# cgisky1980/Qwen3-TTS-Rust

Measured on AMD Instinct MI355X. Metric: audio_sec_per_s, higher is better.
Workload: dtype bf16

## Files before the change

include/q3tts.h:

```cpp
#ifndef Q3TTS_H
#define Q3TTS_H

#include <stdint.h>

#ifdef __cplusplus
extern "C" {
#endif

#define Q3TTS_OK 0
#define Q3TTS_ERR_INVALID (-1)
#define Q3TTS_ERR_DEVICE (-2)
#define Q3TTS_ERR_OOM (-3)
#define Q3TTS_ERR_IO (-4)
#define Q3TTS_ERR_STATE (-5)
#define Q3TTS_ERR_UNSUPPORTED (-6)

#define Q3TTS_MAX_UPSAMPLE 4
#define Q3TTS_MAX_DEC_BLOCKS 8


typedef struct q3tts_model_config {
    int32_t t_n_layer, t_d_model, t_n_head, t_n_kv_head, t_head_dim, t_d_ffn, t_vocab;
    float t_rope_theta;
    int32_t t_mrope_sections[4];
// ... 164 lines not shown
int32_t q3tts_node_size(const q3tts_node* n);
q3tts_engine* q3tts_node_engine(q3tts_node* n, int32_t rank);
int32_t q3tts_node_shard(int32_t n_total, int32_t world, int32_t rank, int32_t* idx, int32_t cap);

typedef struct q3tts_timings {
    float prefill_ms, decode_ms, vocoder_ms, total_ms;
    float frame_step_ms;
    float probe_kernel_ms;
    int64_t frame_steps;
    int64_t algo_bytes_per_step;
    int64_t algo_flops_per_step;
    float mean_live_slots;
    float mean_rows;
    int64_t probe_count;
    float probe_empty_ms;
    float mean_ctx_tokens;
} q3tts_timings;
int q3tts_get_timings(const q3tts_engine* e, q3tts_timings* out);

int32_t q3tts_mel_frames(int64_t n_samples);
int q3tts_mel(q3tts_engine* e, const float* audio, int64_t n_samples, float* out, int32_t cap_frames, int32_t* n_frames);

typedef struct q3tts_clone_config {
    int32_t mel_dim;
    int32_t se_channels[5];
    int32_t se_kernels[5];
    int32_t se_dilations[5];
    int32_t se_attn_channels;
    int32_t se_res2net_scale;
    int32_t se_se_channels;
    int32_t se_dim;
    int32_t ae_filters;
    int32_t ae_kernel, ae_res_kernel, ae_last_kernel;
    int32_t ae_n_ratios; int32_t ae_ratios[4];
    int32_t ae_hidden;
    int32_t ae_n_layer, ae_n_head, ae_head_dim, ae_d_ffn, ae_window;
    float ae_rope_theta, ae_ln_eps, ae_layer_scale;
    int32_t ae_down_stride;
    int32_t ae_vq_dim;
    int32_t ae_n_codebooks, ae_codebook_size;
} q3tts_clone_config;
void q3tts_clone_default_config(q3tts_clone_config* cfg);
int q3tts_clone_init(q3tts_engine* e, const q3tts_clone_config* cfg);
int32_t q3tts_clone_audio_frames(const q3tts_engine* e, int64_t n_samples);
int q3tts_clone_audio_encode(q3tts_engine* e, const float* audio, int64_t n_samples, int64_t* codes, int32_t cap_frames,
                             int32_t* n_frames);
int q3tts_clone_speaker_encode(q3tts_engine* e, const float* audio, int64_t n_samples, float* spk_emb);
int q3tts_k_speaker_from_mel(q3tts_engine* e, const float* mel, int32_t n_frames, float* spk_emb);
int q3tts_k_audio_latent(q3tts_engine* e, const float* audio, int64_t n_samples, float* latent, int32_t cap_frames,
                         int32_t* n_frames);

typedef struct q3tts_tokenizer q3tts_tokenizer;
int q3tts_tokenizer_load(const char* tokenizer_json_path, q3tts_tokenizer** out, char* err, int32_t err_cap);
void q3tts_tokenizer_free(q3tts_tokenizer* t);
int32_t q3tts_tokenizer_vocab_size(const q3tts_tokenizer* t);
int q3tts_tokenizer_encode(const q3tts_tokenizer* t, const char* utf8, int64_t n_bytes, uint32_t* ids, int32_t cap,
                           int32_t* n_ids, char* err, int32_t err_cap);
int q3tts_tokenizer_decode(const q3tts_tokenizer* t, const uint32_t* ids, int32_t n, char* out, int64_t cap, int64_t* n_bytes,
                           char* err, int32_t err_cap);

int q3tts_k_gemm_exact(int32_t device, const float* x, int32_t B, int32_t K, const uint16_t* w_bf16, int32_t N,
                       const float* norm_w , float eps, const float* bias ,
                       int32_t epilogue , float* y, uint64_t* argmax_keys,
                       int32_t iters, float* mean_kernel_ms);
int q3tts_k_attention(int32_t device, const float* qkv , int32_t n_rows, int32_t pos0,
                      int32_t n_head, int32_t n_kv_head, int32_t head_dim, const float* q_norm_w, const float* k_norm_w,
                      float eps, float rope_theta, const int32_t* mrope_sections, float* out );
int q3tts_k_attention_decode(int32_t device, const float* qkv, int32_t n_slots, const int32_t* lens, int32_t n_ctx, int32_t n_head,
                             int32_t n_kv_head, int32_t head_dim, const float* q_norm_w, const float* k_norm_w, float eps, float rope_theta,
                             const int32_t* mrope_sections, int32_t policy, float* out_f32, uint16_t* out_bf16);
int q3tts_k_attention_runs(int32_t device, const float* qkv, int32_t n_runs, const int32_t* run_n, const int32_t* run_pos0, int32_t n_ctx,
                           int32_t n_head, int32_t n_kv_head, int32_t head_dim, const float* q_norm_w, const float* k_norm_w, float eps,
                           float rope_theta, const int32_t* mrope_sections, int32_t policy, int32_t out_form, void* out, float* out_scale,
                           uint16_t* k_cache, uint16_t* v_cache);
int q3tts_k_attention_decode_ex(int32_t device, const float* qkv, int32_t n_slots, const int32_t* lens, int32_t n_ctx, int32_t n_head,
                                int32_t n_kv_head, int32_t head_dim, const float* q_norm_w, const float* k_norm_w, float eps,
                                float rope_theta, const int32_t* mrope_sections, int32_t policy, int32_t row_indexed, int32_t out_form,
                                void* out, float* out_scale, uint16_t* k_cache, uint16_t* v_cache);
int q3tts_k_attention_pair(int32_t device, const float* qkv, int32_t n_slots, int32_t n_ctx, int32_t n_head, int32_t n_kv_head,
                           int32_t head_dim, const float* q_norm_w, const float* k_norm_w, float eps, float rope_theta,
                           const int32_t* mrope_sections, int32_t out_form, void* out, float* out_scale, uint16_t* k_cache, uint16_t* v_cache);
int q3tts_k_attend_pick(int32_t fused, int32_t gqa_ratio, int32_t n_ctx, int32_t n_seg, int32_t seg_max_n, int32_t seg_max_t,
                        int32_t n_kv_head, int32_t* kernel);
int q3tts_k_sample(int32_t device, const float* logits, int32_t n, int32_t ld, int32_t limit, float temperature,
                   int32_t top_k, float top_p, const float* r_uniform, int32_t* out_ids);
int q3tts_k_talker_prefill(q3tts_engine* e, const float* embd, int32_t n_tok, float* hidden_out, float* logits_out);
int q3tts_k_talker_prefill_prefix(q3tts_engine* e, const q3tts_prefix* prefix, const float* embd, int32_t n_tok, float* hidden_out,
                                  float* logits_out);
int q3tts_k_vocoder(q3tts_engine* e, const int32_t* codes, int32_t n_frames, int32_t chunk_frames, float* pcm_out,
                    int32_t* n_samples_out);
int q3tts_k_vocoder_latent(q3tts_engine* e, const int32_t* codes, int32_t n_frames, int32_t chunk_frames, float* out);
typedef struct q3tts_voc_tap {
    char name[32];
    int32_t dtype, layout, hist_rows, rows, channels, reserved;
    uint64_t offset;
} q3tts_voc_tap;
int q3tts_k_vocoder_taps(q3tts_engine* e, const int32_t* codes, int32_t n_frames, int32_t chunk_frames, int32_t tap_call, void* buf,
                         uint64_t buf_bytes, q3tts_voc_tap* recs, int32_t rec_cap, int32_t* n_recs);
int q3tts_k_vocoder_bench(q3tts_engine* e, int32_t n_slots, int32_t chunks, float* ms_per_chunk);
int q3tts_k_gguf_read(const char* path, const char* tensor, float* out, int64_t cap, int64_t* nelem, int64_t* dims4, int32_t* ggml_type);
int q3tts_k_gguf_meta(const char* path, const char* key, int32_t* value_type, int32_t* elem_type, int64_t* count, double* values,
                      int64_t values_cap, char* str, int64_t str_cap, int64_t* str_bytes);
int q3tts_k_probe(q3tts_engine* e, int32_t enable);
int q3tts_k_mfma_bf16(int32_t device, const uint16_t* a, const uint16_t* b, const float* c, float* d, int32_t n_cases, int32_t chain);
int q3tts_k_bgemm(int32_t device, const uint16_t* xb, int32_t B, int32_t K, const uint16_t* w_bf16, int32_t N, const float* ssp, int32_t ntiles,
                  int32_t d_norm, float eps, int32_t epilogue, const float* nw_next, float* y, uint16_t* yb, float* ssp_out, uint64_t* keys,
                  int32_t iters, float* mean_kernel_ms);
int q3tts_k_bgemm_policy(int32_t big);
int q3tts_k_attend_policy(int32_t decode, int32_t prefill);
int q3tts_k_pred_variant(q3tts_engine* e, int32_t force);
int q3tts_k_text_ready(int32_t n_text, int32_t closed, int32_t n_frames);
int q3tts_k_bgemm_pick(int32_t B, int32_t K, int32_t N, int32_t epilogue, int32_t w_once, int32_t q8, int32_t* out5);
int q3tts_k_bgemm_q8(int32_t device, const uint16_t* xb, int32_t B, int32_t K, const int8_t* q, const uint16_t* d_f16, int32_t N, const float* ssp,
                     int32_t ntiles, int32_t d_norm, float eps, int32_t epilogue, const float* nw_next, float* y, uint16_t* yb, float* ssp_out,
                     uint64_t* keys, int32_t iters, float* mean_kernel_ms);
int q3tts_k_bgemm_q8a8(int32_t device, const int8_t* aq, const float* ad, int32_t B, int32_t K, const int8_t* q, const uint16_t* d_f16, int32_t N,
                       const float* ssp, int32_t ntiles, int32_t d_norm, float eps, int32_t epilogue, const float* nw_next, float* y, int8_t* yq,
                       float* yd, float* ssp_out, int32_t iters, float* mean_kernel_ms);
int q3tts_k_bgemm_q8a8_argmax(int32_t device, const int8_t* aq, const float* ad, int32_t B, int32_t K, const int8_t* q, const uint16_t* d_f16, int32_t N,
                              const float* ssp, int32_t ntiles, int32_t d_norm, float eps, int32_t* ids_out);
int q3tts_k_bgemm_voc(int32_t device, const uint16_t* xb, int32_t B, int32_t K, const uint16_t* w_bf16, int32_t N, int32_t epilogue, const float* bias,
                      int32_t bias_n, const float* col_scale, int32_t seg_rows, int32_t gap_rows, float* y, uint16_t* yb, int32_t want_yb);
int q3tts_k_project(int32_t device, const float* x, int32_t rows, int32_t n_in, const float* w, const float* bias, int32_t n_out, const float* nw,
                    float* y, uint16_t* xb, float* ssp);
int q3tts_k_norm_inputs(int32_t device, const float* x, int32_t rows, int32_t d, const float* nw, uint16_t* xb, float* ssp);
int q3tts_k_alloc_upload(q3tts_engine* e, int64_t bytes, int64_t* mismatches);
int q3tts_k_pcm_pack(int32_t device, const float* src, int32_t rows, int64_t stride, const int32_t* ent_row, const int32_t* ent_first,
                     const int32_t* ent_count, const int64_t* ent_dst, int32_t n_ent, int32_t format, void* out, int64_t out_n);
int q3tts_k_resample_table(int32_t rate_in, int32_t rate_out, int32_t* L, int32_t* M, int32_t* H, float* tab, int64_t cap, int64_t* n);
int q3tts_k_pcm_resample(int32_t device, const float* src, int32_t rows, int64_t stride, const int32_t* row_len, const int32_t* row_final,
                         const int32_t* ent_row, const int32_t* ent_first, const int32_t* ent_count, const int64_t* ent_dst, int32_t n_ent,
                         int32_t rate_in, int32_t rate_out, int32_t format, void* out, int64_t out_n, int32_t iters, float* mean_ms);
int q3tts_k_rng_f32(uint64_t seed, int32_t n, float* out);

#ifdef __cplusplus
}
#endif
#endif
```

qwen3-tts-rust_amd/csrc/q3_attend.hip:

```cpp
#include "q3_kernels.h"

__device__ __forceinline__ uint2 pack_bf16x4(float a, float b, float c, float d) {
    return make_uint2((uint32_t)q3_bf16(a) | ((uint32_t)q3_bf16(b) << 16), (uint32_t)q3_bf16(c) | ((uint32_t)q3_bf16(d) << 16));
}
__device__ __forceinline__ uint16_t* k_cache_elem(uint16_t* khead, int pos, int lane) {
    const int blk = pos >> 6, kl = pos & 63, c = lane >> 1, e0 = 4 * (lane & 1);
    return khead + ((size_t)(blk * (Q3_ATT_HD >> 3) + c) * 64 + kl) * 8 + e0;
}
__device__ __forceinline__ float prep_rinv(const float4 x4, float eps, int hd) {
    float acc = 0.0f;
    acc = fmaf(x4.x, x4.x, acc); acc = fmaf(x4.y, x4.y, acc); acc = fmaf(x4.z, x4.z, acc); acc = fmaf(x4.w, x4.w, acc);
    acc = wave_sum(acc);
    return 1.0f / sqrtf(acc / (float)hd + eps);
}
__device__ __forceinline__ void prep_norm(const float4 x4, float rinv, const float4 w4, float y[4]) {
    y[0] = (x4.x * rinv) * w4.x; y[1] = (x4.y * rinv) * w4.y; y[2] = (x4.z * rinv) * w4.z; y[3] = (x4.w * rinv) * w4.w;
}
__device__ __forceinline__ void prep_rope(const float y[4], const float4 c4, const float4 s4, int hl, int lane, float o[4]) {
    const float cc[4] = {c4.x, c4.y, c4.z, c4.w}, ss[4] = {s4.x, s4.y, s4.z, s4.w};
#pragma unroll
    for (int e = 0; e < 4; ++e) {
        const float other = __shfl_xor(y[e], hl);
        o[e] = (lane < hl) ? fmaf(-other, ss[e], y[e] * cc[e])
                           : fmaf(other, ss[e], y[e] * cc[e]);
// ... 312 lines not shown
#pragma unroll
        for (int u = 0; u < 4; ++u) vv[tr][u] = *(const uint4*)(vb + (size_t)min(64 * tr + 4 * sw + kg + 16 * u, T - 1) * hd + dl * 8);
    ml0 = wave_max(ml0); ml1 = wave_max(ml1);
    if (lane == 0) { mw[sw] = ml0; mw[4 + sw] = ml1; }
    Q3_LDS_BARRIER();
    const float m0 = fmaxf(fmaxf(mw[0], mw[1]), fmaxf(mw[2], mw[3])), m1 = fmaxf(fmaxf(mw[4], mw[5]), fmaxf(mw[6], mw[7]));
    float ls0 = 0.0f, ls1 = 0.0f;
    for (int blk = sw; blk * 64 < T; blk += 4) {
        const int t = blk * 64 + lane;
        if (t < T) {
            const float e0 = q3_expf(p0[t] - m0), e1 = q3_expf(p1[t] - m1);
            p0[t] = e0; p1[t] = e1; ls0 += e0; ls1 += e1;
        }
    }
    ls0 = wave_sum(ls0); ls1 = wave_sum(ls1);
    if (lane == 0) { lw[sw] = ls0; lw[4 + sw] = ls1; }
    Q3_LDS_BARRIER();
    Q3_STAMP(a, 2);
    float o0[8], o1[8];
#pragma unroll
    for (int e = 0; e < 8; ++e) { o0[e] = 0.0f; o1[e] = 0.0f; }
    const uint4 vn = *(const uint4*)(vnew + 4 * dl);
#pragma unroll
    for (int tr = 0; tr < 4; ++tr) {
        const int t0 = 64 * tr + 4 * sw + kg;
        if (64 * tr >= T) break;
#pragma unroll
        for (int u = 0; u < 4; ++u) {
            const int t = t0 + 16 * u;
            if (t < T) {
                const float pa = p0[t], pb = p1[t];
                const uint4 w = (t == pos) ? vn : vv[tr][u];
                att_pv8x2(pa, pb, w, o0, o1);
            }
        }
    }
    for (int t0 = 256 + 4 * sw + kg; t0 < T; t0 += 64) {
        uint4 vl[4];
#pragma unroll
        for (int u = 0; u < 4; ++u) vl[u] = *(const uint4*)(vb + (size_t)min(t0 + 16 * u, T - 1) * hd + dl * 8);
#pragma unroll
        for (int u = 0; u < 4; ++u) {
            const int t = t0 + 16 * u;
            if (t < T) {
                const float pa = p0[t], pb = p1[t];
                const uint4 w = (t == pos) ? vn : vl[u];
                att_pv8x2(pa, pb, w, o0, o1);
            }
        }
    }
#pragma unroll
    for (int e = 0; e < 8; ++e) {
        o0[e] = o0[e] + __shfl_xor(o0[e], 16); o0[e] = o0[e] + __shfl_xor(o0[e], 32);
        o1[e] = o1[e] + __shfl_xor(o1[e], 16); o1[e] = o1[e] + __shfl_xor(o1[e], 32);
    }
    if (kg == 0) {
        *(float4*)(ow + (0 * 4 + sw) * hd + dl * 8) = (float4){o0[0], o0[1], o0[2], o0[3]}; *(float4*)(ow + (0 * 4 + sw) * hd + dl * 8 + 4) = (float4){o0[4], o0[5], o0[6], o0[7]};
        *(float4*)(ow + (1 * 4 + sw) * hd + dl * 8) = (float4){o1[0], o1[1], o1[2], o1[3]}; *(float4*)(ow + (1 * 4 + sw) * hd + dl * 8 + 4) = (float4){o1[4], o1[5], o1[6], o1[7]};
    }
    Q3_LDS_BARRIER();
    Q3_STAMP(a, 3);
    if (tid < 128) {
        const int h2 = tid >> 6, d0 = 2 * (tid & 63);
        const float l = ((lw[h2 * 4] + lw[h2 * 4 + 1]) + lw[h2 * 4 + 2]) + lw[h2 * 4 + 3];
        float ov[2];
#pragma unroll
        for (int q = 0; q < 2; ++q) {
            const int d = d0 + q;
            const float r0 = ow[(h2 * 4 + 0) * hd + d], r1 = ow[(h2 * 4 + 1) * hd + d], r2 = ow[(h2 * 4 + 2) * hd + d], r3 = ow[(h2 * 4 + 3) * hd + d];
            ov[q] = (((r0 + r1) + r2) + r3) / l;
        }
        const int hq = g * 2 + h2;
        if (a.out_bf16 == 2) q3_q8_out2x16(ov[0], ov[1], row, hq * hd + d0, (a.Hq * hd) >> 6, a.out_rt16, (int8_t*)a.out, a.out_scale);
        else if (a.out_bf16) *(uint32_t*)((uint16_t*)a.out + q3_atile_off(row, hq * hd + d0, (a.Hq * hd) >> 5)) = (uint32_t)q3_bf16(ov[0]) | ((uint32_t)q3_bf16(ov[1]) << 16);
        else *(float2*)(a.out + (size_t)row * a.ldo + (size_t)hq * hd + d0) = make_float2(ov[0], ov[1]);
    }
#ifdef Q3_STAMPS
    Q3_STAMP(a, 4);
    asm volatile("s_waitcnt vmcnt(0)" ::: "memory");
    Q3_STAMP(a, 5);
#endif
}

template <int R>
__global__ __launch_bounds__((R + 1) * 64) void k_attend_small(Q3Attend a) {
    __shared__ __attribute__((aligned(16))) float qh[R][Q3_ATT_HD];
    __shared__ __attribute__((aligned(16))) uint32_t knew[64];
    __shared__ __attribute__((aligned(16))) uint32_t vnew[64];
    const int g = blockIdx.x, row = blockIdx.y, wv = threadIdx.x >> 6, lane = threadIdx.x & 63;
    Q3_STAMP(a, 0);
    int pos, slot;
    q3_row_map(row, a.row_pos, a.row_slot, a.slot_mod, a.pos_const, &pos, &slot);
    if (pos < 0) return;
    constexpr int hd = Q3_ATT_HD, half = hd >> 1, nl = hd >> 2;
    const int T = pos + 1;
    const Q3QkPrep& pr = a.prep;
    const size_t hb = ((size_t)slot * a.Hkv + g) * a.n_ctx;
    const uint16_t* kb = a.kc + hb * hd;
    const uint16_t* vb = a.vc + hb * hd;
    const float* rowp = a.qkv + (size_t)row * a.ld;
    const float* csp = pr.cs + (size_t)pos * half + 4 * (lane & 15);
    const float* snp = pr.sn + (size_t)pos * half + 4 * (lane & 15);
    if (wv == R) {
        const bool isk = lane < nl;
        const float4 x4 = isk ? ((const float4*)(rowp + (size_t)(a.Hq + g) * hd))[lane] : ((const float4*)(rowp + (size_t)(a.Hq + a.Hkv + g) * hd))[lane - nl];
        float4 w4 = (float4){0.f, 0.f, 0.f, 0.f}, c4 = (float4){1.f, 1.f, 1.f, 1.f}, s4 = (float4){0.f, 0.f, 0.f, 0.f};
        if (isk) { w4 = ((const float4*)pr.knw)[lane]; c4 = *(const float4*)csp; s4 = *(const float4*)snp; }
        const float4 v = isk ? x4 : (float4){0.f, 0.f, 0.f, 0.f};
        float o[4];
        prep_arith(v, w4, c4, s4, pr.eps, lane, o);
        if (isk) {
            const uint2 kk = pack_bf16x4(o[0], o[1], o[2], o[3]);
            *(uint2*)k_cache_elem(pr.kc + hb * hd, pos, lane) = kk;
            *(uint2*)(knew + 2 * lane) = kk;
        } else {
            const int j = lane - nl;
            const uint2 vk = pack_bf16x4(x4.x, x4.y, x4.z, x4.w);
            *(uint2*)(pr.vc + (hb + pos) * hd + 4 * j) = vk;
            *(uint2*)(vnew + 2 * j) = vk;
        }
        Q3_STAMP(a, 1);
        __syncthreads();
        return;
    }
    const int hq = g * R + wv;
    uint4 kv[16];
    uint32_t vv[16];
#pragma unroll
    for (int c = 0; c < 16; ++c) kv[c] = lane < pos ? ((const uint4*)kb)[c * 64 + lane] : make_uint4(0, 0, 0, 0);
#pragma unroll
    for (int u = 0; u < 16; ++u) vv[u] = u < pos ? *(const uint32_t*)(vb + (size_t)u * hd + 2 * lane) : 0u;
    float4 x4 = (float4){0.f, 0.f, 0.f, 0.f}, w4 = x4, c4 = (float4){1.f, 1.f, 1.f, 1.f}, s4 = x4;
    if (lane < nl) { x4 = ((const float4*)(rowp + (size_t)hq * hd))[lane]; w4 = ((const float4*)pr.qnw)[lane]; c4 = *(const float4*)csp; s4 = *(const float4*)snp; }
    {
        float y[4];
        prep_norm(x4, prep_rinv(x4, pr.eps, hd), w4, y);
        const float cc[4] = {c4.x, c4.y, c4.z, c4.w}, ss[4] = {s4.x, s4.y, s4.z, s4.w};
        float o[4];
#pragma unroll
        for (int e = 0; e < 4; ++e) {
            const float other = __shfl_xor(y[e], 16);
            o[e] = (lane < 16) ? fmaf(-other, ss[e], y[e] * cc[e]) : fmaf(other, ss[e], y[e] * cc[e]);
        }
        if (lane < nl) *(float4*)(qh[wv] + 4 * lane) = (float4){o[0], o[1], o[2], o[3]};
    }
    Q3_STAMP(a, 1);
    __syncthreads();
    Q3_STAMP(a, 2);
    if (lane == pos) {
#pragma unroll
        for (int c = 0; c < 16; ++c) kv[c] = *(const uint4*)(knew + 4 * c);
    }
    const float* q = qh[wv];
    float sc = 0.0f;
#pragma unroll
    for (int c = 0; c < 16; ++c)
        sc = att_dot8(*(const float4*)(q + c * 8), *(const float4*)(q + c * 8 + 4), kv[c], sc);
    sc = sc * (1.0f / sqrtf((float)hd));
    const float m = wave_max(lane < T ? sc : -INFINITY);
    const float e = lane < T ? q3_expf(sc - m) : 0.0f;
    float l = wave_sum(e);
    l = ((l + 0.0f) + 0.0f) + 0.0f;
#ifdef Q3_STAMPS
    asm volatile("" :: "v"(l)); Q3_STAMP(a, 3);
#endif
    float o0[16], o1[16];
#pragma unroll
    for (int u = 0; u < 16; ++u) { o0[u] = 0.0f; o1[u] = 0.0f; }
    const uint32_t vn = vnew[lane];
#pragma unroll
    for (int c = 0; c < 4; ++c) {
        if (16 * c >= T) break;
#pragma unroll
        for (int u = 0; u < 16; ++u) {
            const int t = 16 * c + u;
            if (t >= T) break;
            uint32_t w;
            if (t == pos) w = vn;
            else if (c == 0) w = vv[u];
            else w = *(const uint32_t*)(vb + (size_t)t * hd + 2 * lane);
            const float pt = __uint_as_float(__builtin_amdgcn_readlane(__float_as_uint(e), t));
            o0[u] = fmaf(pt, q3_u2f(w << 16), o0[u]);
            o1[u] = fmaf(pt, q3_u2f(w & 0xffff0000u), o1[u]);
        }
    }
    float r0[4], r1[4];
#pragma unroll
    for (int w = 0; w < 4; ++w) {
        r0[w] = (o0[4 * w] + o0[4 * w + 1]) + (o0[4 * w + 2] + o0[4 * w + 3]);
        r1[w] = (o1[4 * w] + o1[4 * w + 1]) + (o1[4 * w + 2] + o1[4 * w + 3]);
    }
    const float ov0 = (((r0[0] + r0[1]) + r0[2]) + r0[3]) / l, ov1 = (((r1[0] + r1[1]) + r1[2]) + r1[3]) / l;
    const int d0 = 2 * lane;
    att_out2(a, row, hq, d0, ov0, ov1);
#ifdef Q3_STAMPS
    Q3_STAMP(a, 4);
    asm volatile("s_waitcnt vmcnt(0)" ::: "memory");
    Q3_STAMP(a, 5);
#endif
}

__global__ __launch_bounds__(256) void k_attend_pair(Q3Attend a) {
    __shared__ __attribute__((aligned(16))) float kh[2][128], vh[2][128], qh[2][2][128], ps[2][2][64];
    const int g = blockIdx.x, b = blockIdx.y, wave = threadIdx.x >> 6, lane = threadIdx.x & 63;
    const int rr = wave >> 1, hh = wave & 1, R = 2, hd = 128;
    const int row = rr * a.slot_mod + b, slot = b, pos = rr;
    const Q3QkPrep& pr = a.prep;
    const size_t hb = ((size_t)slot * a.Hkv + g) * a.n_ctx;
    const float* rowp = a.qkv + (size_t)row * a.ld;
    const int half = hd >> 1, nl = hd >> 2;
    float qo[4], o4[4];
    prep_head(rowp + (size_t)(g * R + hh) * hd, pr.qnw, pr.eps, pr.cs + (size_t)pos * half, pr.sn + (size_t)pos * half, hd, lane, qo);
    if (lane < nl) *(float4*)(qh[rr][hh] + 4 * lane) = (float4){qo[0], qo[1], qo[2], qo[3]};
    if (hh == 0) {
        prep_head(rowp + (size_t)(a.Hq + g) * hd, pr.knw, pr.eps, pr.cs + (size_t)pos * half, pr.sn + (size_t)pos * half, hd, lane, o4);
        if (lane < nl) {
// ... 144 lines not shown
                const float ov = ((rsw[0][e] + rsw[1][e]) + rsw[2][e]) + rsw[3][e];
                const int d = dl * 8 + e, col = (g * 2 + hh) * hd + d;
                if (a.out_bf16) ((uint16_t*)a.out)[q3_atile_off(row, col, (a.Hq * hd) >> 5)] = q3_bf16(ov / l);
                else a.out[(size_t)row * a.ldo + col] = ov / l;
            }
        }
        asm volatile("s_waitcnt lgkmcnt(0)" ::: "memory");
    }
}

static int g_att_decode = 0, g_att_prefill = 0;
static std::once_flag g_att_once;
static void att_policy_init() {
    std::call_once(g_att_once, []() {
        const char* ev = getenv("Q3TTS_ATT_OLD"); g_att_decode = (ev && atoi(ev)) ? 1 : 0;
        ev = getenv("Q3TTS_ATT_PREFILL_OLD"); g_att_prefill = (ev && atoi(ev)) ? 1 : 0;
    });
}
void q3_attend_policy(int decode, int prefill) { att_policy_init(); g_att_decode = decode; g_att_prefill = prefill; }
void q3_attend_policy_get(int* decode, int* prefill) { att_policy_init(); *decode = g_att_decode; *prefill = g_att_prefill; }

static hipError_t att_allow_lds(const void* kernel, size_t lds) { return hipFuncSetAttribute(kernel, hipFuncAttributeMaxDynamicSharedMemorySize, (int)lds); }

int q3_attend_pick(const Q3Attend& a) {
    att_policy_init();
    if (a.hd != Q3_ATT_HD || a.Hkv <= 0 || a.Hq % a.Hkv) return Q3_ATT_REFUSED;
    const int R = a.Hq / a.Hkv;
    if ((R != 1 && R != 2 && R != 4) || (a.fused && R == 1) || (a.fused == 2 && R != 2)) return Q3_ATT_REFUSED;
    if (a.fused == 2) return Q3_ATT_PAIR;
    if (a.fused && a.n_ctx <= 64 && R == 2) return Q3_ATT_SMALL2;
    if (a.fused && R == 2 && g_att_decode == 0) return Q3_ATT_GQA2;
    if (!a.fused && R == 2 && a.seg && a.seg_max_n <= 128 && a.seg_max_t <= 256 && g_att_prefill != 1 &&
        (a.n_seg * a.Hkv >= 128 || g_att_prefill == 2)) return Q3_ATT_PREFILL;
    if (a.fused) return R == 2 ? Q3_ATT_F2 : Q3_ATT_F4;
    return R == 1 ? Q3_ATT_N1 : (R == 2 ? Q3_ATT_N2 : Q3_ATT_N4);
}

int q3_launch_attend(const Q3Attend& a, hipStream_t s) {
    const int pick = q3_attend_pick(a);
    if (pick == Q3_ATT_REFUSED) return 1;
    const int R = a.Hq / a.Hkv;
    const dim3 grid(a.Hkv, a.rows);
    if (pick == Q3_ATT_PAIR) {
        hipLaunchKernelGGL(k_attend_pair, dim3(a.Hkv, a.slot_mod), dim3(256), 0, s, a);
        return 0;
    }
    if (pick == Q3_ATT_SMALL2) {
        hipLaunchKernelGGL((k_attend_small<2>), grid, dim3(192), 0, s, a);
        return 0;
    }
    if (pick == Q3_ATT_GQA2) {
        const size_t lds2 = ((size_t)2 * a.n_ctx + 2 * Q3_ATT_HD + 8 * Q3_ATT_HD + 16 + 128) * sizeof(float);
        static Q3PerDevice pd2;
        if (lds2 > 65536 && !pd2.ensure(lds2, [&]() { return att_allow_lds((const void*)k_attend_gqa2, lds2); })) return 1;
        hipLaunchKernelGGL(k_attend_gqa2, grid, dim3(256), lds2, s, a);
        return 0;
    }
    if (pick == Q3_ATT_PREFILL) {
        const int nblk = (a.seg_max_t + 63) / 64;
        const int pw = a.seg_max_t > 128 ? (a.seg_max_t + 63) & ~63 : 128;
        const size_t lds3 = (size_t)nblk * 16384 + (size_t)a.seg_max_t * 256 + (size_t)8 * (pw + 128) * sizeof(float);
        static Q3PerDevice pd3;
        if (lds3 > 65536 && !pd3.ensure(lds3, [&]() { return att_allow_lds((const void*)k_attend_prefill, lds3); })) return 1;
        hipLaunchKernelGGL(k_attend_prefill, dim3(a.Hkv, a.n_seg), dim3(512), lds3, s, a);
        return 0;
    }
    const size_t lds = att_lds(R, a.n_ctx).bytes;
    static Q3PerDevice pd;
    if (lds > 65536 && !pd.ensure(lds, [&]() {
            hipError_t e = hipSuccess;
            for (const void* k : {(const void*)k_attend<2, true>, (const void*)k_attend<4, true>, (const void*)k_attend<1, false>,
                                  (const void*)k_attend<2, false>, (const void*)k_attend<4, false>})
                if (e == hipSuccess) e = att_allow_lds(k, lds);
            return e;
        })) return 1;
    if (pick == Q3_ATT_F2) hipLaunchKernelGGL((k_attend<2, true>), grid, dim3(512), lds, s, a);
    else if (pick == Q3_ATT_F4) hipLaunchKernelGGL((k_attend<4, true>), grid, dim3(1024), lds, s, a);
    else if (pick == Q3_ATT_N1) hipLaunchKernelGGL((k_attend<1, false>), grid, dim3(256), lds, s, a);
    else if (pick == Q3_ATT_N2) hipLaunchKernelGGL((k_attend<2, false>), grid, dim3(512), lds, s, a);
    else hipLaunchKernelGGL((k_attend<4, false>), grid, dim3(1024), lds, s, a);
    return 0;
}

__global__ __launch_bounds__(256) void k_kv_prefix(Q3KvPrefix a) {
    const int j = blockIdx.y, isv = blockIdx.x & 1, lg = blockIdx.x >> 1, l = lg / a.Hkv, g = lg - l * a.Hkv;
    const int P = a.P[j], np = (P + 63) & ~63;
    const size_t src = ((size_t)l * a.Hkv + g) * np * a.hd;
    const size_t dst = (size_t)l * a.layer_stride + ((size_t)a.slot[j] * a.Hkv + g) * a.n_ctx * a.hd;
    const int n16 = (isv ? P : np) * (a.hd >> 3);
    const uint4* sp = (const uint4*)((isv ? a.pv[j] : a.pk[j]) + src);
    uint4* dp = (uint4*)((isv ? a.vc : a.kc) + dst);
    for (int i = threadIdx.x; i < n16; i += 256) dp[i] = sp[i];
}
void q3_launch_kv_prefix(const Q3KvPrefix& a, hipStream_t s) {
    if (a.n <= 0) return;
    hipLaunchKernelGGL(k_kv_prefix, dim3(a.L * 2 * a.Hkv, a.n), dim3(256), 0, s, a);
}
```

qwen3-tts-rust_amd/csrc/q3_engine.h:

```cpp
#pragma once
#include <algorithm>
#include <cstddef>
#include <atomic>
#include <mutex>
#include <string>
#include <vector>

#include "../../include/q3tts.h"
#include "q3_kernels.h"

static_assert(sizeof(q3tts_request) == 80 && offsetof(q3tts_request, text_stream) == 12 && offsetof(q3tts_request, prompt) == 16 &&
              offsetof(q3tts_request, text_open) == 44 && offsetof(q3tts_request, seed) == 48 && offsetof(q3tts_request, prefix) == 72, "q3tts_request layout");

struct Q3Voc;
struct Q3Mel;
struct Q3Clone;

struct Q3Tfm {
    int L = 0, d = 0, Hq = 0, Hkv = 0, hd = 0, F = 0, nq = 0, nkv = 0, nqkv = 0, head_n = 0;
    std::vector<float*> attn_norm, ffn_norm, qn, kn;
    std::vector<uint4*> wqkv, wo, wgu, wd;
    float* out_norm = nullptr;
    uint4* head = nullptr;
    std::vector<uint16_t*> sqkv, so, sgu, sd; uint16_t* shead = nullptr; bool q8 = false;
    bool a8 = false;
    uint16_t *kc = nullptr, *vc = nullptr;
    size_t layer_stride = 0;
    int n_ctx = 0, n_slots = 0;
    float *cs = nullptr, *sn = nullptr;
    size_t weight_bytes = 0;
};

struct Q3Scratch {
    float* qkv = nullptr;
    uint16_t *att = nullptr, *h = nullptr;
    float *asc_att = nullptr, *asc_h = nullptr; int rt16 = 0;
    int rows = 0;
};

struct Q3Rows {
    float* x = nullptr;
    uint16_t* xb = nullptr;
    float* ssp = nullptr;
    float* ascale = nullptr; int rt16 = 0;
};

struct Q3Lane {
    int nb = 0;
    hipStream_t stream = nullptr;
    Q3Rows T, P;
    float *logits = nullptr, *logits_tmp = nullptr, *fb = nullptr;
    unsigned long long* keys = nullptr;
    int *row_pos_t = nullptr, *slot_id = nullptr, *perm = nullptr;
    Q3Scratch sc;
    float* plogits = nullptr;
    std::vector<hipGraph_t> graphs;
    std::vector<hipGraphExec_t> execs;
    std::vector<hipGraph_t> graphs_s;
    std::vector<hipGraphExec_t> execs_s;
    std::vector<hipGraph_t> graphs_t[2];
    std::vector<hipGraphExec_t> execs_t[2];
    hipEvent_t ev_begin = nullptr, ev_end = nullptr;
};

struct q3tts_engine {
    q3tts_engine_config cfg;
    std::string err;
    hipStream_t stream = nullptr, vstream = nullptr;
    std::vector<void*> allocs;
    Q3Tfm T, P;
    float* text = nullptr;
    std::vector<float*> codec;
    const float** codec_dev = nullptr;
    std::vector<float*> pproj;
    float* proj_w = nullptr;
    float* proj_b = nullptr;
    float* tts_pad = nullptr;
    float* marker_row = nullptr;
    int B = 0;
    std::vector<int> buckets; int cur_bucket = -1;
    std::vector<int> row_of_slot, slot_of_row;
    Q3Slot* slots = nullptr;
    Q3Slot* slots_host = nullptr;
    int* codes = nullptr;
    float* rng = nullptr;
    Q3Lane lane;
    Q3Scratch sc_pre;
    Q3Rows pf;
    int *pf_pos = nullptr, *pf_slot = nullptr;
    int* pf_seg = nullptr;
    Q3PromptRow* prow_dev = nullptr; int prow_cap = 0;
    float* spk_dev = nullptr; int* refcodes_dev = nullptr;
    float temperature = 0.7f; int top_k = 40; float top_p = 0.9f; int has_seed = 0; uint64_t seed = 0;
    int max_steps = 512;
    float p_temperature = 0.0f; int p_top_k = 0; float p_top_p = 1.0f; float rep_penalty = 1.0f;
    int pred_force = 0, pred_variant = 0;
    int streams_open = 0;
    int* ts_ids = nullptr; int* ts_cnt = nullptr; int2* ts_cur = nullptr;
    std::vector<char> ts_slot; int ts_variant = 0, ts_used = 0;
    float* prng = nullptr;
    uint32_t* seen = nullptr; int seen_words = 0;
    hipEvent_t ev0 = nullptr, ev1 = nullptr, ev2 = nullptr, ev3 = nullptr;
    std::vector<hipEvent_t> fin_ev;
    q3tts_timings tm{};
    Q3Voc* voc = nullptr;
    Q3Mel* mel = nullptr;
    Q3Clone* clone = nullptr;
    int probe = 0, probe_kind = 0;
    std::vector<hipEvent_t> probe_ev;
    int probe_i = 0;
    double probe_ms = 0, probe_empty_ms = 0; long long probe_cnt = 0, probe_empty_cnt = 0, row_steps = 0;
    int dev_pcm_on = 0; float* dev_pcm = nullptr; int dev_pcm_n = 0; size_t dev_pcm_stride = 0;
    int out_rate = 0; Q3Resamp rs_out{}; std::vector<Q3Resamp> rs_cache;
    float* rs_stage = nullptr; size_t rs_stage_stride = 0, rs_stage_cap = 0;
    double hp_launch = 0, hp_sync = 0;
    float *park_logits = nullptr, *park_x = nullptr;
    float* first_chunk_host = nullptr;
    std::atomic<q3tts_session*> session{nullptr};
    std::mutex err_mu;
};

struct q3tts_prefix {
    q3tts_engine* e = nullptr;
    int P = 0, np = 0;
    uint16_t *k = nullptr, *v = nullptr;
};

int q3_set_err(q3tts_engine* e, int code, const std::string& msg);
int q3_refuse_in_session(q3tts_engine* e);
#define Q3_NOT_IN_SESSION(e) do { if ((e) && (e)->session.load()) return q3_refuse_in_session(e); } while (0)
#define Q3_HIP(e, call)                                                                                         \
    do {                                                                                                        \
        hipError_t err__ = (call);                                                                              \
        if (err__ != hipSuccess)                                                                                \
            return q3_set_err((e), Q3TTS_ERR_DEVICE, std::string(#call) + ": " + hipGetErrorString(err__));     \
    } while (0)

int q3_dev_alloc_zeroed(q3tts_engine* e, void** p, size_t bytes);

template <class T>
int q3_dalloc(q3tts_engine* e, T** p, size_t n) {
    void* q = nullptr;
    const int rc = q3_dev_alloc_zeroed(e, &q, n * sizeof(T) + 64);
    if (rc != Q3TTS_OK) return rc;
    e->allocs.push_back(q);
    *p = (T*)q;
    return Q3TTS_OK;
}

class Q3Gguf;
struct Q3TfmShape {
    int grp;
    int L, d, Hq, Hkv, hd, F, head_n;
    float theta; const int* sections;
    int n_ctx, n_slots;
};
int q3_tfm_init(q3tts_engine* e, Q3Tfm& t, const Q3TfmShape& sh, const Q3Gguf* g, const char* file, int q8mode);
int q3_assets_init(q3tts_engine* e, const std::string& wdir);

struct Q3LayerRun {
    int rows;
    const int *row_pos, *row_slot;
    bool one_row_per_slot;
    hipEvent_t* probe;
    int slot_mod, pos_const;
    const int* seg; int n_seg, seg_max_n, seg_max_t;
};
int q3_run_layers(q3tts_engine* e, Q3Tfm& t, const Q3Rows& r, const Q3LayerRun& a, Q3Scratch& sc, hipStream_t s);
int q3_record_frame(q3tts_engine* e, Q3Lane& L, hipStream_t s, int B);
int q3_capture_frames(q3tts_engine* e, std::vector<hipGraph_t>& graphs, std::vector<hipGraphExec_t>& execs);
Q3BGemm q3_gemm_head(const Q3Tfm& t, int q, int N, const Q3Rows& r, int row0, int rows, float eps, int once, float* y);
int q3_launch_gemm(q3tts_engine* e, const Q3Tfm& t, const Q3BGemm& g, hipStream_t s, hipEvent_t* probe = nullptr, int kind = -1);

void q3_rope_tables(int n_pos, int hd, float theta, const int* sections, std::vector<float>& cs, std::vector<float>& sn);

void q3_stdrng_f32(uint64_t seed, int n, float* out);

void q3_mel_destroy(q3tts_engine* e);
int q3_mel_run(q3tts_engine* e, const float* audio, int64_t n_samples, int32_t* n_frames, float** out_dev);
void q3_clone_destroy(q3tts_engine* e);
int q3_voc_create(q3tts_engine* e);
void q3_voc_destroy(q3tts_engine* e);
int q3_voc_reset(q3tts_engine* e, int slot);
int q3_voc_decode(q3tts_engine* e, int slot, int f0, int nf, int is_last, hipStream_t s);
int q3_voc_decode_batch(q3tts_engine* e, const int* slots, const int* real, int ns, int nf, hipStream_t s, int beside_decoder);
void q3_voc_mark_last(q3tts_engine* e, int slot);
float* q3_voc_pcm(q3tts_engine* e, int slot);
int q3_voc_samples(q3tts_engine* e, int slot);
int q3_voc_samples_per_frame(const q3tts_engine* e);
size_t q3_voc_pcm_stride(const q3tts_engine* e);

int q3_resample_get(q3tts_engine* e, int rate_in, int rate_out, Q3Resamp* out);
int q3_resample_slot(q3tts_engine* e, int b, long long first_out, int count, int n_valid, bool is_final, hipStream_t s);

enum { BOS_TOKEN = 151672, EOS_TOKEN = 151673 };

int q3_plan_rows(q3tts_engine* e, const std::vector<int>& live);
int q3_admit_many(q3tts_engine* e, const int* slots, const q3tts_request* const* reqs, int count, int* rc);
int q3_run_chunk(q3tts_engine* e, int CH);
int q3_text_rows_set(q3tts_engine* e, int b, const int32_t* T, int from, int n, int n_frames);
int q3_park_rows(q3tts_engine* e, int b, bool save);
void q3_text_trailing(const q3tts_request* r, std::vector<int32_t>& T);
int q3_pred_force_variant(q3tts_engine* e, int force);
int q3_voc_dispatch(q3tts_engine* e, const char* live, const char* want, int* voc_frames, bool more, bool* first);
double q3_now_ms();
```

qwen3-tts-rust_amd/csrc/q3_engine.hip:

```cpp
#include "q3_engine.h"
#include "q3_gguf.h"

#include <chrono>
#include <cmath>
#include <cstdio>
#include <cstdlib>
#include <cstring>

static thread_local std::string g_err;

int q3_set_err(q3tts_engine* e, int code, const std::string& msg) {
    if (e) { std::lock_guard<std::mutex> lk(e->err_mu); e->err = msg; }
    g_err = msg;
    return code;
}
extern "C" const char* q3tts_last_error(const q3tts_engine* e) {
    if (!e) return g_err.c_str();
    if (!e->session.load()) return e->err.c_str();
    static thread_local std::string copy;
    std::lock_guard<std::mutex> lk(const_cast<q3tts_engine*>(e)->err_mu);
    copy = e->err;
    return copy.c_str();
}
int q3_refuse_in_session(q3tts_engine* e) {
// ... 49 lines not shown
    if (c.talker_q8_0 == 2) REQ(m.t_vocab % 32 == 0 && ((m.t_n_head + 2 * m.t_n_kv_head) * m.t_head_dim) % 32 == 0 && m.t_d_ffn % 64 == 0);
    REQ(c.predictor_q8_0 >= 0 && c.predictor_q8_0 <= 2);
    if (c.predictor_q8_0 == 2) {
        REQ(m.p_d_model % 512 == 0); REQ(m.p_d_ffn % 512 == 0); REQ((m.p_n_head * m.p_head_dim) % 512 == 0);
        REQ(m.codebook_size % 32 == 0); REQ(((m.p_n_head + 2 * m.p_n_kv_head) * m.p_head_dim) % 32 == 0); REQ(m.p_d_ffn % 64 == 0);
    }
#undef REQ
    return Q3TTS_OK;
}

int q3_dev_alloc_zeroed(q3tts_engine* e, void** p, size_t bytes) {
    void* q = nullptr;
    hipError_t err = hipMalloc(&q, bytes);
    if (err != hipSuccess) return q3_set_err(e, Q3TTS_ERR_OOM, std::string("hipMalloc: ") + hipGetErrorString(err));
    err = hipMemsetAsync(q, 0, bytes, e->stream);
    if (err == hipSuccess) err = hipStreamSynchronize(e->stream);
    if (err != hipSuccess) { hipFree(q); return q3_set_err(e, Q3TTS_ERR_DEVICE, std::string("hipMemset: ") + hipGetErrorString(err)); }
    *p = q;
    return Q3TTS_OK;
}
#define TRY(x) do { int rc__ = (x); if (rc__ != Q3TTS_OK) return rc__; } while (0)

static int alloc_scratch(q3tts_engine* e, Q3Scratch& sc, int rows, int nqkv, int nq, int F) {
    sc.rows = rows;
    const size_t r16 = ((size_t)rows + 15) & ~(size_t)15;
    TRY(q3_dalloc(e, &sc.qkv, (size_t)rows * nqkv)); TRY(q3_dalloc(e, &sc.att, r16 * nq)); TRY(q3_dalloc(e, &sc.h, r16 * F));
    sc.rt16 = (int)(r16 / 16);
    if (e->T.a8 || e->P.a8) { TRY(q3_dalloc(e, &sc.asc_att, r16 * (nq / 32))); TRY(q3_dalloc(e, &sc.asc_h, r16 * (F / 32))); }
    return Q3TTS_OK;
}

static int alloc_rows(q3tts_engine* e, Q3Rows& r, size_t rows, int d, bool scales) {
    const size_t r16 = (rows + 15) & ~(size_t)15;
    TRY(q3_dalloc(e, &r.x, rows * d)); TRY(q3_dalloc(e, &r.xb, r16 * d)); TRY(q3_dalloc(e, &r.ssp, rows * (d / 16)));
    r.rt16 = (int)(r16 / 16);
    if (scales) TRY(q3_dalloc(e, &r.ascale, r16 * (d / 32)));
    return Q3TTS_OK;
}

extern "C" int q3tts_engine_create(const q3tts_engine_config* cfg, q3tts_engine** out) {
    if (!cfg || !out) return q3_set_err(nullptr, Q3TTS_ERR_INVALID, "null argument");
    std::string why;
    if (validate(*cfg, why) != Q3TTS_OK) return q3_set_err(nullptr, Q3TTS_ERR_INVALID, why);
    if (cfg->predictor_q8_0 == 1)
        return q3_set_err(nullptr, Q3TTS_ERR_UNSUPPORTED, "predictor_q8_0 = 1 (Q8_0 weights x bf16 activations) is not implemented for the Predictor: use 0 (bf16) or 2 (Q8_0 x Q8_0)");
    int ndev = 0;
    if (hipGetDeviceCount(&ndev) != hipSuccess || ndev <= 0)
        return q3_set_err(nullptr, Q3TTS_ERR_DEVICE, "no HIP device: libq3tts has no CPU fallback");
    if (cfg->device < 0 || cfg->device >= ndev) return q3_set_err(nullptr, Q3TTS_ERR_INVALID, "device ordinal out of range");
    q3tts_engine* e = new q3tts_engine();
    e->cfg = *cfg; e->cfg.weights_path = nullptr;
    e->max_steps = cfg->max_steps_cap < 512 ? cfg->max_steps_cap : 512;
    auto fail = [&](int rc) { std::string m = e->err; q3tts_engine_destroy(e); g_err = m; return rc; };
#define TRYC(x) do { int rc__ = (x); if (rc__ != Q3TTS_OK) return fail(rc__); } while (0)
#define HIPC(call) do { hipError_t er__ = (call); if (er__ != hipSuccess) { q3_set_err(e, Q3TTS_ERR_DEVICE, std::string(#call) + ": " + hipGetErrorString(er__)); return fail(Q3TTS_ERR_DEVICE); } } while (0)
    HIPC(hipSetDevice(cfg->device));
    q3_bgemm_prepare();
    if (cfg->talker_q8_0 == 2 || cfg->predictor_q8_0 == 2) q3_bgemm8_prepare();
    HIPC(hipStreamCreateWithFlags(&e->stream, hipStreamNonBlocking));
    if (getenv("Q3TTS_VOC_SERIAL") && atoi(getenv("Q3TTS_VOC_SERIAL"))) e->vstream = e->stream;
    else if (getenv("Q3TTS_VOC_CUMASK")) {
        uint32_t w = (uint32_t)strtoul(getenv("Q3TTS_VOC_CUMASK"), nullptr, 16), mask[8];
        for (auto& x : mask) x = w;
        HIPC(hipExtStreamCreateWithCUMask(&e->vstream, 8, mask));
    } else HIPC(hipStreamCreateWithFlags(&e->vstream, hipStreamNonBlocking));
    HIPC(hipEventCreate(&e->ev0)); HIPC(hipEventCreate(&e->ev1)); HIPC(hipEventCreate(&e->ev2)); HIPC(hipEventCreate(&e->ev3));
    e->fin_ev.resize(cfg->max_batch, nullptr);
    for (auto& ev : e->fin_ev) HIPC(hipEventCreateWithFlags(&ev, hipEventDisableTiming));
    const q3tts_model_config& m = e->cfg.model;
    const int B = cfg->max_batch;
    e->B = B;
    hipStream_t s = e->stream;
    const std::string wdir = cfg->weights_path ? cfg->weights_path : "";
    Q3Gguf gt, gp;
    std::string er;
    if (!wdir.empty() && (gt.open(wdir + "/qwen3_tts_talker.gguf", er) || gp.open(wdir + "/qwen3_tts_predictor.gguf", er))) { q3_set_err(e, Q3TTS_ERR_INVALID, er); return fail(Q3TTS_ERR_INVALID); }
    TRYC(q3_tfm_init(e, e->T, {.grp = Q3G_TALKER, .L = m.t_n_layer, .d = m.t_d_model, .Hq = m.t_n_head, .Hkv = m.t_n_kv_head, .hd = m.t_head_dim, .F = m.t_d_ffn,
                               .head_n = m.t_vocab, .theta = m.t_rope_theta, .sections = m.t_mrope_sections, .n_ctx = cfg->n_ctx, .n_slots = B},
                     wdir.empty() ? nullptr : &gt, "qwen3_tts_talker.gguf", cfg->talker_q8_0));
    TRYC(q3_tfm_init(e, e->P, {.grp = Q3G_PRED, .L = m.p_n_layer, .d = m.p_d_model, .Hq = m.p_n_head, .Hkv = m.p_n_kv_head, .hd = m.p_head_dim, .F = m.p_d_ffn,
                               .head_n = (m.n_codebooks - 1) * m.codebook_size, .theta = m.p_rope_theta, .sections = nullptr, .n_ctx = 64, .n_slots = B},
                     wdir.empty() ? nullptr : &gp, "qwen3_tts_predictor.gguf", cfg->predictor_q8_0));
    TRYC(q3_assets_init(e, wdir));
    TRYC(q3_dalloc(e, &e->slots, (size_t)B));
    HIPC(hipHostMalloc((void**)&e->slots_host, sizeof(Q3Slot) * 2 * B, hipHostMallocDefault));
    memset(e->slots_host, 0, sizeof(Q3Slot) * 2 * B);
    TRYC(q3_dalloc(e, &e->codes, (size_t)B * cfg->max_steps_cap * m.n_codebooks)); TRYC(q3_dalloc(e, &e->rng, (size_t)B * cfg->max_steps_cap));
    TRYC(q3_dalloc(e, &e->prng, (size_t)B * cfg->max_steps_cap * (m.n_codebooks - 1)));
    e->seen_words = (m.sample_limit + 31) / 32;
    TRYC(q3_dalloc(e, &e->seen, (size_t)B * e->seen_words));
    TRYC(q3_dalloc(e, &e->ts_ids, (size_t)B * cfg->max_steps_cap)); TRYC(q3_dalloc(e, &e->ts_cnt, (size_t)B)); TRYC(q3_dalloc(e, &e->ts_cur, (size_t)B));
    TRYC(q3_dalloc(e, &e->park_logits, (size_t)B * m.t_vocab)); TRYC(q3_dalloc(e, &e->park_x, (size_t)B * m.t_d_model));
    e->ts_slot.assign(B, 0);
    {
        const int nb = B;
        const int nqkv_max = std::max(e->T.nqkv, e->P.nqkv), nq_max = std::max(e->T.nq, e->P.nq), F_max = std::max(e->T.F, e->P.F);
        Q3Lane& L = e->lane;
        L.nb = nb;
        HIPC(hipStreamCreateWithFlags(&L.stream, hipStreamNonBlocking));
        HIPC(hipEventCreate(&L.ev_begin)); HIPC(hipEventCreate(&L.ev_end));
        TRYC(alloc_rows(e, L.T, (size_t)nb, m.t_d_model, e->T.a8)); TRYC(alloc_rows(e, L.P, (size_t)2 * nb, m.p_d_model, e->P.a8));
        TRYC(q3_dalloc(e, &L.logits, (size_t)nb * m.t_vocab)); TRYC(q3_dalloc(e, &L.logits_tmp, (size_t)nb * std::max(m.t_vocab, m.t_d_model)));
        TRYC(q3_dalloc(e, &L.fb, (size_t)nb * m.d_embed)); TRYC(q3_dalloc(e, &L.keys, (size_t)nb * (m.codebook_size / 16)));
        TRYC(q3_dalloc(e, &L.plogits, (size_t)nb * m.codebook_size));
        TRYC(q3_dalloc(e, &L.row_pos_t, (size_t)nb)); TRYC(q3_dalloc(e, &L.slot_id, (size_t)nb)); TRYC(q3_dalloc(e, &L.perm, (size_t)nb));
        std::vector<int> sid(nb), rp(nb, -1);
        for (int b = 0; b < nb; ++b) sid[b] = b;
        HIPC(hipMemcpyAsync(L.slot_id, sid.data(), nb * 4, hipMemcpyHostToDevice, s));
        HIPC(hipMemcpyAsync(L.row_pos_t, rp.data(), nb * 4, hipMemcpyHostToDevice, s));
        HIPC(hipStreamSynchronize(s));
        TRYC(alloc_scratch(e, L.sc, 2 * nb, nqkv_max, nq_max, F_max));
        for (int r = 1; r < nb && r < 16; r *= 2) e->buckets.push_back(r);
        for (int r = 16; r < nb; r += 16) e->buckets.push_back(r);
        e->buckets.push_back(nb);
        e->cur_bucket = (int)e->buckets.size() - 1;
        e->row_of_slot = sid; e->slot_of_row = sid;
    }
    TRYC(alloc_scratch(e, e->sc_pre, cfg->n_ctx, e->T.nqkv, e->T.nq, e->T.F));
    TRYC(alloc_rows(e, e->pf, (size_t)cfg->n_ctx, m.t_d_model, e->T.a8));
    TRYC(q3_dalloc(e, &e->pf_pos, (size_t)cfg->n_ctx)); TRYC(q3_dalloc(e, &e->pf_slot, (size_t)cfg->n_ctx)); TRYC(q3_dalloc(e, &e->pf_seg, (size_t)4 * cfg->max_batch));
    { std::vector<int> pp(cfg->n_ctx); for (int i = 0; i < cfg->n_ctx; ++i) pp[i] = i;
      HIPC(hipMemcpyAsync(e->pf_pos, pp.data(), pp.size() * 4, hipMemcpyHostToDevice, s)); HIPC(hipStreamSynchronize(s)); }
    e->prow_cap = cfg->n_ctx;
    TRYC(q3_dalloc(e, &e->prow_dev, (size_t)e->prow_cap)); TRYC(q3_dalloc(e, &e->spk_dev, (size_t)m.d_embed));
    TRYC(q3_dalloc(e, &e->refcodes_dev, (size_t)cfg->n_ctx * 16));
    {
        TRYC(q3_dalloc(e, &e->marker_row, (size_t)m.d_embed));
        const Q3PromptRow mr{1, m.tts_pad_id, 0, 0};
        HIPC(hipMemcpyAsync(e->prow_dev, &mr, sizeof(mr), hipMemcpyHostToDevice, s));
        HIPC(hipStreamSynchronize(s));
        q3_launch_prompt_rows(e->prow_dev, 1, e->text, m.text_vocab, e->codec_dev, m.codec0_rows, m.codecq_rows, m.n_codebooks, e->spk_dev, m.d_embed, e->marker_row, s);
        HIPC(hipStreamSynchronize(s));
    }
    if (cfg->with_vocoder) {
        TRYC(q3_voc_create(e));
        HIPC(hipHostMalloc((void**)&e->first_chunk_host, sizeof(float) * 4 * (size_t)q3_voc_samples_per_frame(e), hipHostMallocDefault));
    }
    HIPC(hipStreamSynchronize(s));
    if (!(getenv("Q3TTS_NO_GRAPH") && atoi(getenv("Q3TTS_NO_GRAPH")))) TRYC(q3_capture_frames(e, e->lane.graphs, e->lane.execs));
#undef TRYC
#undef HIPC
    *out = e;
    return Q3TTS_OK;
}

extern "C" void q3tts_engine_destroy(q3tts_engine* e) {
    if (!e) return;
    if (q3tts_session* ss = e->session.load()) q3tts_session_close(ss);
    hipSetDevice(e->cfg.device);
    if (e->stream) hipStreamSynchronize(e->stream);
    if (e->vstream) hipStreamSynchronize(e->vstream);
    if (e->voc) q3_voc_destroy(e);
    q3_mel_destroy(e);
    q3_clone_destroy(e);
    if (e->first_chunk_host) hipHostFree(e->first_chunk_host);
    {
        Q3Lane& L = e->lane;
        if (L.stream) hipStreamSynchronize(L.stream);
        for (auto ge : L.execs) if (ge) hipGraphExecDestroy(ge);
        for (auto gr : L.graphs) if (gr) hipGraphDestroy(gr);
        for (auto ge : L.execs_s) if (ge) hipGraphExecDestroy(ge);
        for (auto gr : L.graphs_s) if (gr) hipGraphDestroy(gr);
        for (int v = 0; v < 2; ++v) {
            for (auto ge : L.execs_t[v]) if (ge) hipGraphExecDestroy(ge);
            for (auto gr : L.graphs_t[v]) if (gr) hipGraphDestroy(gr);
        }
// ... 640 lines not shown
    e->probe_ms = 0; e->probe_cnt = 0; e->row_steps = 0; e->probe_empty_ms = 0; e->probe_empty_cnt = 0;
    hipStream_t s = e->stream;
    while (done < n) {
        bool admitted = false;
        {
            std::vector<int> as, ai; std::vector<const q3tts_request*> ar;
            for (int b = 0; b < B && next < n; ++b)
                if (run[b].req < 0) { TRY(drain(b)); as.push_back(b); ar.push_back(&reqs[next]); ai.push_back(next++); }
            {
                std::vector<int> live(as);
                for (int b = 0; b < B; ++b) if (run[b].req >= 0) live.push_back(b);
                TRY(plan_rows(e, live));
            }
            if (!as.empty()) {
                Q3_HIP(e, hipEventRecord(e->ev0, s));
                admitted = true;
                std::vector<int> rcs(as.size());
                TRY(admit_many(e, as.data(), ar.data(), (int)as.size(), rcs.data()));
                for (size_t i = 0; i < as.size(); ++i) {
                    if (rcs[i] != Q3TTS_OK) { outs[ai[i]].status = rcs[i]; ++done; }
                    else { run[as[i]] = SlotRun{}; run[as[i]].req = ai[i]; voc_frames[as[i]] = 0; }
                }
            }
        }
        if (admitted) { Q3_HIP(e, hipEventRecord(e->ev2, s)); }
        hp_lap(hp_admit);
        bool any = false;
        for (int b = 0; b < B; ++b) if (run[b].req >= 0) any = true;
        if (!any) break;
        float ms = 0;
        TRY(run_chunk(e, CH, &ms));
        hp_lap(hp_chunk);
        dec_ms += ms; steps += CH;
        if (admitted) { hipEventElapsedTime(&ms, e->ev0, e->ev2); pre_ms += ms; }
        for (int b = 0; b < B; ++b) if (run[b].req >= 0) { ctx_tokens += (long long)e->slots_host[b].cur_pos * CH; live_slot_steps += CH; }
        if (e->voc) {
            const double tv0 = now_ms();
            hipStream_t vs = e->vstream;
            for (int b = 0; b < B; ++b) { live[b] = run[b].req >= 0; want[b] = live[b] && reqs[run[b].req].want_pcm; }
            bool first = false;
            TRY(q3_voc_dispatch(e, live.data(), want.data(), voc_frames.data(), next < n, &first));
            if (first) {
                for (int b = 0; b < B; ++b)
                    if (run[b].req >= 0 && run[b].t_first == 0 && voc_frames[b] > 0) {
                        const int nsmp = std::min(voc_frames[b], 4) * spf;
                        Q3_HIP(e, hipMemcpyAsync(e->first_chunk_host, q3_voc_pcm(e, b), sizeof(float) * (size_t)nsmp, hipMemcpyDeviceToHost, vs));
                    }
                Q3_HIP(e, hipStreamSynchronize(vs));
                const double tn = now_ms();
                for (int b = 0; b < B; ++b) if (run[b].req >= 0 && run[b].t_first == 0 && voc_frames[b] > 0) run[b].t_first = tn;
            }
            voc_ms += now_ms() - tv0;
        }
        hp_lap(hp_voc);
        for (int j = 0; j < B; ++j)
            if (pending[j] >= 0 && hipEventQuery(e->fin_ev[j]) == hipSuccess) TRY(drain(j));
        for (int b = 0; b < B; ++b) {
            if (run[b].req < 0 || e->slots_host[b].active) continue;
            for (int j = 0; j < B; ++j)
                if (pending[j] >= 0 && hipEventQuery(e->fin_ev[j]) == hipSuccess) TRY(drain(j));
            TRY(finalize(e, b, &reqs[run[b].req], &outs[run[b].req], run[b], t0, true, e->fin_ev[b], run[b].req));
            pending[b] = run[b].req;
            run[b].req = -1; ++done;
            e->ts_slot[b] = 0;
        }
        hp_lap(hp_fin);
    }
    for (int b = 0; b < B; ++b) TRY(drain(b));
    hp_lap(hp_tail);
    if (host_prof) {
        fprintf(stderr, "q3tts_generate_batch host wall (ms): admit + plan %.1f | chunks (launch + wait) %.1f = launch %.1f + wait %.1f, device events %.1f over %lld steps | vocoder issue %.1f | finalize %.1f | tail (last results) %.1f | total %.1f\n",
                hp_admit, hp_chunk, e->hp_launch, e->hp_sync, dec_ms, steps, hp_voc, hp_fin, hp_tail, now_ms() - t0);
        e->hp_launch = e->hp_sync = 0;
    }
    e->tm.prefill_ms = (float)pre_ms; e->tm.decode_ms = (float)dec_ms; e->tm.vocoder_ms = (float)voc_ms;
    e->tm.total_ms = (float)(now_ms() - t0); e->tm.frame_steps = steps; e->tm.frame_step_ms = steps ? (float)(dec_ms / steps) : 0.0f;
    {
        const q3tts_model_config& m = e->cfg.model;
        const long long wt = (long long)e->T.weight_bytes;
        const double bpw_p = e->P.q8 ? 1.0625 : 2.0;
        const long long wp_layers = (long long)e->P.weight_bytes - (long long)(bpw_p * (double)((size_t)e->P.head_n * m.p_d_model));
        const long long head1 = (long long)(bpw_p * (double)((size_t)m.codebook_size * m.p_d_model)), pj = 2ll * m.p_d_model * m.d_embed;
        const long long kv_per_tok = 2ll * m.t_n_layer * 2 * m.t_n_kv_head * m.t_head_dim;
        const long long fixed = wt + (m.n_codebooks - 1) * (wp_layers + head1) + pj;
        e->tm.algo_bytes_per_step = fixed + (steps ? kv_per_tok * (ctx_tokens / steps) : 0);
        e->tm.mean_live_slots = steps ? (float)((double)live_slot_steps / (double)steps) : 0.0f;
        e->tm.algo_flops_per_step = (long long)((double)fixed * (double)e->tm.mean_live_slots);
        e->tm.mean_rows = steps ? (float)((double)e->row_steps / (double)steps) : 0.0f;
        e->tm.mean_ctx_tokens = steps ? (float)((double)ctx_tokens / (double)steps) : 0.0f;
        e->tm.probe_kernel_ms = e->probe_cnt ? (float)(e->probe_ms / (double)e->probe_cnt) : 0.0f;
        e->tm.probe_count = e->probe_cnt;
        e->tm.probe_empty_ms = e->probe_empty_cnt ? (float)(e->probe_empty_ms / (double)e->probe_empty_cnt) : 0.0f;
    }
    return Q3TTS_OK;
}

int q3_plan_rows(q3tts_engine* e, const std::vector<int>& live) { return plan_rows(e, live); }
int q3_admit_many(q3tts_engine* e, const int* slots, const q3tts_request* const* reqs, int count, int* rc) { return admit_many(e, slots, reqs, count, rc); }
int q3_run_chunk(q3tts_engine* e, int CH) { return run_chunk(e, CH, nullptr); }
double q3_now_ms() { return now_ms(); }

extern "C" int q3tts_generate(q3tts_engine* e, const q3tts_request* req, q3tts_result* out) {
    int rc = q3tts_generate_batch(e, req, 1, out);
    if (rc != Q3TTS_OK) return rc;
    return out->status;
}

extern "C" void q3tts_result_free(q3tts_result* r) {
    if (!r) return;
    free(r->codes);
    pin_free(r->pcm);
    r->codes = nullptr; r->pcm = nullptr;
}

extern "C" int q3tts_get_timings(const q3tts_engine* e, q3tts_timings* out) {
    if (!e || !out) return Q3TTS_ERR_INVALID;
    *out = e->tm;
    return Q3TTS_OK;
}

struct q3tts_stream {
    q3tts_engine* e; q3tts_request req; int voc_frames = 0; bool finished = false; bool final_sent = false;
    std::vector<float> chunk; double t0 = 0, t_first = 0;
    long long delivered = 0;
};

static int stream_emit(q3tts_stream* st, int before, int after, bool fin, const float** chunk, int32_t* n_samples) {
    q3tts_engine* e = st->e;
    hipStream_t s = e->stream;
    const float* from = q3_voc_pcm(e, 0) + before;
    int c = after - before;
    if (e->out_rate) {
        const Q3Resamp& r = e->rs_out;
        c = (int)((fin ? q3_resample_N(after, r.L, r.M) : q3_resample_D(after, r.L, r.M, r.H)) - st->delivered);
        TRY(q3_resample_slot(e, 0, st->delivered, c, after, fin, s));
        from = e->rs_stage;
        st->delivered += std::max(c, 0);
    }
    st->chunk.resize((size_t)std::max(1, c));
    if (c > 0) Q3_HIP(e, hipMemcpyAsync(st->chunk.data(), from, sizeof(float) * (size_t)c, hipMemcpyDeviceToHost, s));
    Q3_HIP(e, hipStreamSynchronize(s));
    *chunk = st->chunk.data(); *n_samples = std::max(c, 0);
    return Q3TTS_OK;
}

extern "C" int q3tts_stream_begin(q3tts_engine* e, const q3tts_request* req, q3tts_stream** out) {
    if (!e || !req || !out) return q3_set_err(e, Q3TTS_ERR_INVALID, "null argument");
    Q3_NOT_IN_SESSION(e);
    if (!e->voc) return q3_set_err(e, Q3TTS_ERR_STATE, "streaming needs with_vocoder = 1");
    if (req->text_open == 1) return q3_set_err(e, Q3TTS_ERR_INVALID, "text_open = 1 is for sessions (q3tts_session_append_text): a stream takes closed text and never waits");
    Q3_HIP(e, hipSetDevice(e->cfg.device));
    std::fill(e->ts_slot.begin(), e->ts_slot.end(), 0);
    q3tts_stream* st = new q3tts_stream();
    st->e = e; st->req = *req; st->t0 = now_ms();
    int rc = plan_rows(e, std::vector<int>{0});
    if (rc == Q3TTS_OK) rc = admit(e, 0, req);
    if (rc != Q3TTS_OK) { delete st; return rc; }
    ++e->streams_open;
    *out = st;
    return Q3TTS_OK;
}

extern "C" int q3tts_stream_poll(q3tts_stream* st, const float** chunk, int32_t* n_samples, int32_t* is_final) {
    if (!st || !chunk || !n_samples || !is_final) return q3_set_err(nullptr, Q3TTS_ERR_INVALID, "null argument");
    q3tts_engine* e = st->e;
    *chunk = nullptr; *n_samples = 0; *is_final = 0;
    if (st->final_sent) { *is_final = 1; return Q3TTS_OK; }
    hipStream_t s = e->stream;
    const int spf = q3_voc_samples_per_frame(e);
// ... 55 lines not shown
```

qwen3-tts-rust_amd/csrc/q3_hooks.hip:

```cpp
#include "q3_engine.h"

#include <cstdio>
#include <cstring>

#define TRY(x) do { int rc__ = (x); if (rc__ != Q3TTS_OK) return rc__; } while (0)
#define HK(call) do { hipError_t er__ = (call); if (er__ != hipSuccess) return q3_set_err(nullptr, Q3TTS_ERR_DEVICE, std::string(#call) + ": " + hipGetErrorString(er__)); } while (0)

struct DevBuf {
    void* p = nullptr;
    ~DevBuf() { if (p) hipFree(p); }
    template <class T> operator T*() const { return (T*)p; }
    int put(const void* host, size_t bytes) {
        if (hipMalloc(&p, bytes + 64) != hipSuccess || hipMemset(p, 0, bytes + 64) != hipSuccess) return q3_set_err(nullptr, Q3TTS_ERR_OOM, "hipMalloc");
        if (host) HK(hipMemcpy(p, host, bytes, hipMemcpyHostToDevice));
        return Q3TTS_OK;
    }
    int alloc(size_t bytes) { return put(nullptr, bytes); }
    int get(void* host, size_t bytes) const { HK(hipMemcpy(host, p, bytes, hipMemcpyDeviceToHost)); return Q3TTS_OK; }
};

template <class F>
static int time_launches(int iters, F launch, float* mean_ms) {
    if (iters <= 0 || !mean_ms) return Q3TTS_OK;
    hipEvent_t a, b; HK(hipEventCreate(&a)); HK(hipEventCreate(&b));
// ... 286 lines not shown
        if (q3_launch_qk_prep(qp, nullptr)) return q3_set_err(nullptr, Q3TTS_ERR_INVALID, "attention runs hook: the q/k prep launch was refused");
    }
    Q3QkPrep qp = h.prep(drun, (int)n_run, eps); qp.row_pos = drp; qp.row_slot = drs;
    if (q3_launch_qk_prep(qp, nullptr)) return q3_set_err(nullptr, Q3TTS_ERR_INVALID, "attention runs hook: the q/k prep launch was refused");
    Q3Attend at = h.attend(drun, (int)n_run); at.row_pos = drp; at.row_slot = drs;
    at.seg = dseg; at.n_seg = n_runs; at.seg_max_n = seg_max_n; at.seg_max_t = seg_max_t;
    TRY(att_hook_launch("attention runs hook", at, -1, policy));
    TRY(h.read_out(out, out_scale));
    return h.read_cache(k_cache, v_cache);
}

extern "C" int q3tts_k_attention_decode_ex(int32_t device, const float* qkv, int32_t n_slots, const int32_t* lens, int32_t n_ctx, int32_t Hq, int32_t Hkv,
                                           int32_t hd, const float* qnw, const float* knw, float eps, float theta, const int32_t* sections, int32_t policy,
                                           int32_t row_indexed, int32_t out_form, void* out, float* out_scale, uint16_t* k_cache, uint16_t* v_cache) {
    if (const char* why = AttHook::check(qkv, n_slots, n_ctx, Hq, Hkv, hd, qnw, knw, out_form, out, out_scale))
        return q3_set_err(nullptr, Q3TTS_ERR_INVALID, std::string("attention decode_ex hook: ") + why);
    if (!lens || Hq / Hkv < 2 || policy < -1 || policy > 1 || row_indexed < 0 || row_indexed > 1)
        return q3_set_err(nullptr, Q3TTS_ERR_INVALID, "attention decode_ex hook: lens, a GQA ratio of 2 or 4, decode policy -1 .. 1, row_indexed 0 / 1");
    long long total = 0;
    for (int s = 0; s < n_slots; ++s) {
        if (lens[s] < 1 || lens[s] > n_ctx) return q3_set_err(nullptr, Q3TTS_ERR_INVALID, "attention decode_ex hook: a length outside 1 .. n_ctx");
        if (row_indexed && lens[s] != lens[0]) return q3_set_err(nullptr, Q3TTS_ERR_INVALID, "attention decode_ex hook: row-indexed addressing needs equal lengths");
        total += lens[s];
    }
    HK(hipSetDevice(device));
    AttHook h;
    TRY(h.init(n_slots, n_ctx, Hq, Hkv, qnw, knw, theta, sections, out_form, n_slots));
    const int ld = h.ld, npre = (int)(total - n_slots);
    std::vector<float> pre((size_t)std::max(npre, 1) * ld), last((size_t)n_slots * ld);
    std::vector<int> pp, ps, dp(n_slots), ds(n_slots);
    {
        size_t src = 0, ip = 0;
        for (int s = 0; s < n_slots; ++s) {
            for (int r = 0; r < lens[s] - 1; ++r, ++src, ++ip) { memcpy(&pre[ip * ld], qkv + src * ld, (size_t)ld * 4); pp.push_back(r); ps.push_back(s); }
            memcpy(&last[(size_t)s * ld], qkv + src * ld, (size_t)ld * 4); ++src;
            dp[s] = lens[s] - 1; ds[s] = s;
        }
    }
    DevBuf dpre, dlast, dpp, dps, ddp, dds;
    TRY(dpre.put(pre.data(), pre.size() * 4)); TRY(dlast.put(last.data(), last.size() * 4));
    TRY(dpp.put(pp.data(), pp.size() * 4)); TRY(dps.put(ps.data(), ps.size() * 4)); TRY(ddp.put(dp.data(), n_slots * 4)); TRY(dds.put(ds.data(), n_slots * 4));
    if (npre) {
        Q3QkPrep qp = h.prep(dpre, npre, eps); qp.row_pos = dpp; qp.row_slot = dps;
        if (q3_launch_qk_prep(qp, nullptr)) return q3_set_err(nullptr, Q3TTS_ERR_INVALID, "attention decode_ex hook: the q/k prep launch was refused");
    }
    Q3QkPrep dq = h.prep(dlast, n_slots, eps);
    Q3Attend at = h.attend(dlast, n_slots);
    if (row_indexed) { dq.slot_mod = at.slot_mod = n_slots; dq.pos_const = at.pos_const = lens[0] - 1; }
    else { dq.row_pos = at.row_pos = ddp; dq.row_slot = at.row_slot = dds; }
    at.fused = 1; at.prep = dq;
    TRY(att_hook_launch("attention decode_ex hook", at, policy, -1));
    TRY(h.read_out(out, out_scale));
    return h.read_cache(k_cache, v_cache);
}

extern "C" int q3tts_k_attention_pair(int32_t device, const float* qkv, int32_t n_slots, int32_t n_ctx, int32_t Hq, int32_t Hkv, int32_t hd, const float* qnw,
                                      const float* knw, float eps, float theta, const int32_t* sections, int32_t out_form, void* out, float* out_scale,
                                      uint16_t* k_cache, uint16_t* v_cache) {
    if (const char* why = AttHook::check(qkv, n_slots, n_ctx, Hq, Hkv, hd, qnw, knw, out_form, out, out_scale))
        return q3_set_err(nullptr, Q3TTS_ERR_INVALID, std::string("attention pair hook: ") + why);
    if (Hq / Hkv != 2) return q3_set_err(nullptr, Q3TTS_ERR_INVALID, "attention pair hook: the GQA ratio must be 2");
    HK(hipSetDevice(device));
    AttHook h;
    TRY(h.init(n_slots, n_ctx, Hq, Hkv, qnw, knw, theta, sections, out_form, 2 * n_slots));
    DevBuf drows;
    TRY(drows.put(qkv, (size_t)2 * n_slots * h.ld * 4));
    Q3QkPrep qp = h.prep(drows, 2 * n_slots, eps); qp.slot_mod = n_slots; qp.pos_const = 0;
    Q3Attend at = h.attend(drows, 2 * n_slots); at.slot_mod = n_slots; at.pos_const = 0;
    at.fused = 2; at.prep = qp;
    TRY(att_hook_launch("attention pair hook", at, -1, -1));
    TRY(h.read_out(out, out_scale));
    return h.read_cache(k_cache, v_cache);
}

extern "C" int q3tts_k_attend_pick(int32_t fused, int32_t gqa_ratio, int32_t n_ctx, int32_t n_seg, int32_t seg_max_n, int32_t seg_max_t, int32_t n_kv_head,
                                   int32_t* kernel) {
    if (!kernel || fused < 0 || fused > 2 || gqa_ratio <= 0 || gqa_ratio > 64 || n_ctx <= 0 || n_seg < 0 || seg_max_n < 0 || seg_max_t < 0 || n_kv_head <= 0 ||
        n_kv_head > 4096)
        return q3_set_err(nullptr, Q3TTS_ERR_INVALID, "attend pick: bad shape");
    Q3Attend a{}; a.hd = Q3_ATT_HD; a.Hkv = n_kv_head; a.Hq = n_kv_head * gqa_ratio; a.fused = fused; a.n_ctx = n_ctx;
    if (n_seg > 0) { a.seg = (const int*)16; a.n_seg = n_seg; a.seg_max_n = seg_max_n; a.seg_max_t = seg_max_t; }
    *kernel = q3_attend_pick(a);
    return Q3TTS_OK;
}

extern "C" int q3tts_k_sample(int32_t device, const float* logits, int32_t n, int32_t ld, int32_t limit, float temperature, int32_t top_k,
                              float top_p, const float* r, int32_t* out) {
    if (!logits || !out || n <= 0 || limit <= 0 || limit > 4096 || limit > ld) return q3_set_err(nullptr, Q3TTS_ERR_INVALID, "sample hook: bad shape");
    HK(hipSetDevice(device));
    DevBuf dl, dr, dout;
    TRY(dl.put(logits, (size_t)n * ld * 4)); TRY(dr.put(r, (size_t)n * 4)); TRY(dout.alloc((size_t)n * 4));
    q3_launch_sample_rows(dl, n, ld, limit, temperature, top_k, top_p, r ? (const float*)dr.p : nullptr, dout, nullptr);
    HK(hipDeviceSynchronize());
    return dout.get(out, (size_t)n * 4);
}

static int bgemm_hook(const char* name, int device, const uint16_t* xb, int B, int K, const void* w, bool q8, int N, const float* ssp, int ntiles, int d_norm,
                      float eps, int epi, const float* nw_next, float* y, uint16_t* yb, float* ssp_out, uint64_t* keys, int iters, float* mean_ms) {
    HK(hipSetDevice(device));
    const int F = N / 2, nt = N / 16;
    DevBuf dx, dw, dwt, dsc, ds, dn, dy, dyb, dso, dk;
    { const std::vector<uint16_t> xt = atile_host(xb, B, K); TRY(dx.put(xt.data(), xt.size() * 2)); }
    TRY(dw.put(w, q8 ? (size_t)N * (K / 32) * 34 : (size_t)N * K * 2)); TRY(dwt.alloc(q8 ? (size_t)N * K : (size_t)N * K * 2));
    if (q8) TRY(dsc.alloc((size_t)N * (K / 32) * 2));
    TRY(ds.put(ntiles > 0 ? ssp : nullptr, (size_t)B * std::max(ntiles, 1) * 4)); TRY(dn.put(nw_next, (size_t)N * 4));
    TRY(dy.put(epi == Q3_EPI_RESID ? y : nullptr, (size_t)B * N * 4)); TRY(dyb.alloc(pad16(B) * N * 2)); TRY(dso.alloc((size_t)B * nt * 4)); TRY(dk.alloc((size_t)B * nt * 8));
    tile_weight(dw, dwt, q8 ? &dsc : nullptr, N, K, epi == Q3_EPI_SWIGLU);
    Q3BGemm g{}; g.a = dx; g.a_row0 = 0; g.B = B; g.w = dwt; g.K = K; g.N = N;
    if (q8) g.wscale = dsc;
    if (ssp) g.ssp = ds;
    g.ld_ssp = ntiles; g.ntiles = ntiles; g.d_norm = d_norm; g.eps = eps; g.epi = epi;
    g.y = dy; g.ldy = N; g.yb = dyb;
    if (nw_next) g.nw_next = dn;
    g.ssp_out = dso; g.ld_ssp_out = nt; g.keys = dk; g.key_stride = nt;
    if (q3_launch_bgemm(g, nullptr)) return q3_set_err(nullptr, Q3TTS_ERR_INVALID, std::string(name) + ": shape");
    HK(hipDeviceSynchronize());
    if (epi == Q3_EPI_STORE || epi == Q3_EPI_RESID) TRY(dy.get(y, (size_t)B * N * 4));
    if (epi == Q3_EPI_SWIGLU) TRY(untile_host(dyb, B, F, yb));
    if (epi == Q3_EPI_RESID && nw_next) { TRY(untile_host(dyb, B, N, yb)); TRY(dso.get(ssp_out, (size_t)B * nt * 4)); }
    if (epi == Q3_EPI_ARGMAX) {
        std::vector<uint64_t> parts((size_t)B * nt);
        TRY(dk.get(parts.data(), parts.size() * 8));
        for (int b = 0; b < B; ++b) { uint64_t m = 0; for (int t = 0; t < nt; ++t) m = std::max(m, parts[(size_t)b * nt + t]); keys[b] = m; }
    }
    if (epi == Q3_EPI_RESID) { g.epi = Q3_EPI_STORE; g.nw_next = nullptr; }
    return time_launches(iters, [&] { q3_launch_bgemm(g, nullptr); }, mean_ms);
}

extern "C" int q3tts_k_bgemm(int32_t device, const uint16_t* xb, int32_t B, int32_t K, const uint16_t* w, int32_t N, const float* ssp, int32_t ntiles,
                             int32_t d_norm, float eps, int32_t epi, const float* nw_next, float* y, uint16_t* yb, float* ssp_out, uint64_t* keys,
                             int32_t iters, float* mean_ms) {
    if (!xb || !w || B <= 0 || K % 256 || K < 256 || N % 16 || epi < 0 || epi > 3) return q3_set_err(nullptr, Q3TTS_ERR_INVALID, "bgemm hook: K % 256 == 0, N % 16 == 0");
    if (epi == Q3_EPI_SWIGLU && (N % 64 || !yb)) return q3_set_err(nullptr, Q3TTS_ERR_INVALID, "bgemm hook: swiglu needs N % 64 == 0 and yb");
    if (epi == Q3_EPI_RESID && nw_next && N % 32) return q3_set_err(nullptr, Q3TTS_ERR_INVALID, "bgemm hook: norm outputs need N % 32 == 0");
    if ((epi == Q3_EPI_STORE || epi == Q3_EPI_RESID) && !y) return q3_set_err(nullptr, Q3TTS_ERR_INVALID, "bgemm hook: y missing");
    if (epi == Q3_EPI_ARGMAX && !keys) return q3_set_err(nullptr, Q3TTS_ERR_INVALID, "bgemm hook: keys missing");
    if (epi == Q3_EPI_RESID && nw_next && (!yb || !ssp_out)) return q3_set_err(nullptr, Q3TTS_ERR_INVALID, "bgemm hook: norm outputs missing");
    return bgemm_hook("bgemm", device, xb, B, K, w, false, N, ssp, ntiles, d_norm, eps, epi, nw_next, y, yb, ssp_out, keys, iters, mean_ms);
}

extern "C" int q3tts_k_bgemm_q8(int32_t device, const uint16_t* xb, int32_t B, int32_t K, const int8_t* q, const uint16_t* d_f16, int32_t N, const float* ssp,
                                int32_t ntiles, int32_t d_norm, float eps, int32_t epi, const float* nw_next, float* y, uint16_t* yb, float* ssp_out,
                                uint64_t* keys, int32_t iters, float* mean_ms) {
    if (!xb || !q || !d_f16 || B <= 0 || K % 512 || K < 512 || N % 16 || epi < 0 || epi > 3) return q3_set_err(nullptr, Q3TTS_ERR_INVALID, "bgemm_q8 hook: K % 512 == 0, N % 16 == 0");
    if (epi == Q3_EPI_SWIGLU && (N % 64 || !yb)) return q3_set_err(nullptr, Q3TTS_ERR_INVALID, "bgemm_q8 hook: swiglu needs N % 64 == 0 and yb");
    if (epi == Q3_EPI_RESID && nw_next && (N % 32 || !yb || !ssp_out)) return q3_set_err(nullptr, Q3TTS_ERR_INVALID, "bgemm_q8 hook: norm outputs");
    if ((epi == Q3_EPI_STORE || epi == Q3_EPI_RESID) && !y) return q3_set_err(nullptr, Q3TTS_ERR_INVALID, "bgemm_q8 hook: y missing");
    if (epi == Q3_EPI_ARGMAX && !keys) return q3_set_err(nullptr, Q3TTS_ERR_INVALID, "bgemm_q8 hook: keys missing");
    const std::vector<uint8_t> blocks = pack_q8_0(q, d_f16, N, K);
    return bgemm_hook("bgemm_q8", device, xb, B, K, blocks.data(), true, N, ssp, ntiles, d_norm, eps, epi, nw_next, y, yb, ssp_out, keys, iters, mean_ms);
}

extern "C" int q3tts_k_bgemm_q8a8(int32_t device, const int8_t* aq, const float* ad, int32_t B, int32_t K, const int8_t* q, const uint16_t* d_f16, int32_t N,
                                  const float* ssp, int32_t ntiles, int32_t d_norm, float eps, int32_t epi, const float* nw_next, float* y, int8_t* yq, float* yd,
                                  float* ssp_out, int32_t iters, float* mean_ms) {
    if (!aq || !ad || !q || !d_f16 || B <= 0 || K % 512 || K < 512 || N % 32 || epi < 0 || epi > 2) return q3_set_err(nullptr, Q3TTS_ERR_INVALID, "bgemm_q8a8 hook: K % 512 == 0, N % 32 == 0, epilogue 0..2");
    if (epi == Q3_EPI_SWIGLU && (N % 128 || !yq || !yd)) return q3_set_err(nullptr, Q3TTS_ERR_INVALID, "bgemm_q8a8 hook: swiglu needs N % 128 == 0, yq, yd");
    if (epi == Q3_EPI_RESID && (N % 64 || !nw_next || !yq || !yd || !ssp_out || !y)) return q3_set_err(nullptr, Q3TTS_ERR_INVALID, "bgemm_q8a8 hook: residual needs N % 64 == 0, nw_next, y, yq, yd, ssp_out");
    if (epi == Q3_EPI_STORE && !y) return q3_set_err(nullptr, Q3TTS_ERR_INVALID, "bgemm_q8a8 hook: y missing");
    HK(hipSetDevice(device));
    const int F = N / 2, kb = K / 32, Nout = epi == Q3_EPI_SWIGLU ? F : N;
    const size_t B16 = pad16(B); const int rt16 = (int)(B16 / 16);
    const std::vector<uint8_t> blocks = pack_q8_0(q, d_f16, N, K);
    std::vector<int8_t> at(B16 * K, 0); std::vector<float> ast((size_t)kb * B16, 0.0f);
    for (int r = 0; r < B; ++r) {
        for (int k = 0; k < K; ++k) at[q3_q8_off(r, k, K >> 6)] = aq[(size_t)r * K + k];
// ... 340 lines not shown
```

qwen3-tts-rust_amd/csrc/q3_kernels.h:

```cpp
#pragma once
#include "q3_common.h"

enum { Q3_EPI_STORE = 0, Q3_EPI_RESID = 1, Q3_EPI_SWIGLU = 2, Q3_EPI_ARGMAX = 3, Q3_EPI_GELU = 4 };

#ifdef Q3_STAMPS
#define Q3_STAMP_FIELD unsigned long long* dbg;
#define Q3_STAMP(p, i) do { if ((p).dbg && threadIdx.x == 0) (p).dbg[((size_t)blockIdx.x + (size_t)gridDim.x * blockIdx.y) * 8 + (i)] = __builtin_amdgcn_s_memrealtime(); } while (0)
#else
#define Q3_STAMP_FIELD
#define Q3_STAMP(p, i) do { } while (0)
#endif

#include <mutex>
#include <type_traits>
#include <vector>
struct Q3PerDevice {
    std::mutex mu; size_t have[64] = {0};
    template <class F> bool ensure(size_t want, F set_attr) {
        int dev = 0; if (hipGetDevice(&dev) != hipSuccess) dev = 0;
        std::lock_guard<std::mutex> lk(mu);
        if (have[dev & 63] >= want) return true;
        if constexpr (std::is_void_v<decltype(set_attr())>) set_attr();
        else if (set_attr() != hipSuccess) return false;
        have[dev & 63] = want;
// ... 87 lines not shown
    sq = sq + __shfl_xor(sq, 1); sq = sq + __shfl_xor(sq, 2); sq = sq + __shfl_xor(sq, 4); sq = sq + __shfl_xor(sq, 8);
    if (tile_leader) *ssp_tile = sq;
}
#endif

#ifdef __HIPCC__
__device__ __forceinline__ void q3_q8_out32(float v, int row, int k, int kpairs, int rt16, int8_t* q, float* sc) {
    float amax = fabsf(v);
#pragma unroll
    for (int m = 1; m <= 16; m <<= 1) amax = fmaxf(amax, __shfl_xor(amax, m));
    const float d = amax / 127.0f, id = d != 0.0f ? 1.0f / d : 0.0f;
    q[q3_q8_off(row, k, kpairs)] = (int8_t)(int)roundf(v * id);
    if ((k & 31) == 0) sc[q3_q8_scale_idx(row, k >> 5, rt16)] = q3_q8_sig11(d);
}
__device__ __forceinline__ void q3_norm_out_q8(float v, float nwv, int row, int k, int kpairs, int rt16, int8_t* q, float* sc, float* ssp_tile, bool tile_leader) {
    q3_q8_out32(v * nwv, row, k, kpairs, rt16, q, sc);
    float sq = v * v;
    sq = sq + __shfl_xor(sq, 1); sq = sq + __shfl_xor(sq, 2); sq = sq + __shfl_xor(sq, 4); sq = sq + __shfl_xor(sq, 8);
    if (tile_leader) *ssp_tile = sq;
}
__device__ __forceinline__ void q3_q8_out2x16(float v0, float v1, int row, int k0, int kpairs, int rt16, int8_t* q, float* sc) {
    float amax = fmaxf(fabsf(v0), fabsf(v1));
#pragma unroll
    for (int m = 1; m <= 8; m <<= 1) amax = fmaxf(amax, __shfl_xor(amax, m));
    const float d = amax / 127.0f, id = d != 0.0f ? 1.0f / d : 0.0f;
    q[q3_q8_off(row, k0, kpairs)] = (int8_t)(int)roundf(v0 * id);
    q[q3_q8_off(row, k0 + 1, kpairs)] = (int8_t)(int)roundf(v1 * id);
    if ((k0 & 31) == 0) sc[q3_q8_scale_idx(row, k0 >> 5, rt16)] = q3_q8_sig11(d);
}
__device__ __forceinline__ void q3_q8_out8x4(const float* v, int row, int k0, int kpairs, int rt16, int8_t* q, float* sc, bool store) {
    float amax = 0.0f;
#pragma unroll
    for (int i = 0; i < 8; ++i) amax = fmaxf(amax, fabsf(v[i]));
    amax = fmaxf(amax, __shfl_xor(amax, 1)); amax = fmaxf(amax, __shfl_xor(amax, 2));
    const float d = amax / 127.0f, id = d != 0.0f ? 1.0f / d : 0.0f;
    if (store) {
#pragma unroll
        for (int i = 0; i < 8; ++i) q[q3_q8_off(row, k0 + i, kpairs)] = (int8_t)(int)roundf(v[i] * id);
        if ((k0 & 31) == 0) sc[q3_q8_scale_idx(row, k0 >> 5, rt16)] = q3_q8_sig11(d);
    }
}
#endif

struct Q3Fill {
    uint4* dst; int N, K;
    int mode;
    int row0, rows;
    uint32_t tid_a, tid_b;
    const uint16_t* src_a; const uint16_t* src_b;
    uint64_t seed; float scale;
    uint16_t* dst_scale; const uint8_t* src8_a; const uint8_t* src8_b;
};
void q3_launch_fill_tiled(const Q3Fill& f, hipStream_t s);
void q3_launch_fill_tiled_q8(const Q3Fill& f, hipStream_t s);
void q3_launch_fill_f32(float* dst, size_t n, uint64_t seed, uint32_t tid, float base, float scale, int round_bf16, hipStream_t s);

constexpr int Q3_ATT_HD = 128;
struct Q3QkPrep {
    float* qkv; int ld; int rows;
    int Hq, Hkv, hd;
    const float* qnw; const float* knw; float eps;
    const float* cs; const float* sn;
    uint16_t* kc; uint16_t* vc; int n_ctx;
    const int* row_pos; const int* row_slot;
    int slot_mod, pos_const;
};
int q3_launch_qk_prep(const Q3QkPrep& a, hipStream_t s);

struct Q3Attend {
    const float* qkv; int ld; int rows;
    float* out; int ldo;
    int out_bf16;
    float* out_scale; int out_rt16;
    int Hq, Hkv, hd;
    const uint16_t* kc; const uint16_t* vc; int n_ctx;
    const int* row_pos; const int* row_slot;
    int slot_mod, pos_const;
    int fused;
    Q3QkPrep prep;
    const int* seg; int n_seg; int seg_max_n; int seg_max_t;
    Q3_STAMP_FIELD
};
int q3_launch_attend(const Q3Attend& a, hipStream_t s);
enum { Q3_ATT_REFUSED = -1, Q3_ATT_N1 = 0, Q3_ATT_N2 = 1, Q3_ATT_N4 = 2,
       Q3_ATT_F2 = 3, Q3_ATT_F4 = 4,
       Q3_ATT_GQA2 = 5, Q3_ATT_SMALL2 = 6, Q3_ATT_PAIR = 7, Q3_ATT_PREFILL = 8 };
int q3_attend_pick(const Q3Attend& a);
#define Q3_KVP_MAX 64
struct Q3KvPrefix {
    uint16_t* kc; uint16_t* vc; size_t layer_stride; int n_ctx;
    int L, Hkv, hd, n;
    const uint16_t* pk[Q3_KVP_MAX]; const uint16_t* pv[Q3_KVP_MAX]; int P[Q3_KVP_MAX]; int slot[Q3_KVP_MAX];
};
void q3_launch_kv_prefix(const Q3KvPrefix& a, hipStream_t s);
void q3_attend_policy(int decode, int prefill);
void q3_attend_policy_get(int* decode, int* prefill);

struct Q3Sample {
    float* logits; int ld; int limit; int eos;
    Q3Slot* slots; int B;
    const int* row_slot;
    const float* rng;
    int* codes; int max_steps_cap; int ncb;
    uint32_t* seen; int seen_words;
};
void q3_launch_sample(const Q3Sample& a, hipStream_t s);
void q3_launch_sample_rows(const float* logits, int n, int ld, int limit, float temperature, int top_k, float top_p,
                           const float* r, int* out, hipStream_t s);

struct Q3PredInput {
    const float* xT; const float* out_norm; float eps; int d;
    const float* codec0; int codec0_rows;
    const float* pproj0; const float* proj_b; int dp;
    const Q3Slot* slots; const int* row_slot; float* X; float* px; float* fb; int B;
    const float* nw; uint16_t* xb; float* ssp;
    float* xscale; int x_rt16;
};
void q3_launch_pred_input(const Q3PredInput& a, hipStream_t s);
int q3_launch_sample_input(const Q3Sample& a, const Q3PredInput& p, const Q3Project& pj, hipStream_t s);

struct Q3PredNext {
    const unsigned long long* keys; int n_key_parts; int q; int ncb;
    const float* codec_q; int rows_q; int d;
    Q3Slot* slots; const int* row_slot; int B;
    int* codes; int max_steps_cap;
    float* fb; const float* tts_pad; float* xT; int* row_pos_t;
    const float* pproj_q; const float* proj_b; int dp; float* px;
    const float* nw; uint16_t* xb; float* ssp;
    float* xscale; int x_rt16;
    const float* plogits; int cbs; const float* prng; int prng_stride;
    Q3_STAMP_FIELD
};
int q3_launch_pred_next(const Q3PredNext& a, hipStream_t s, bool sample = false);
int q3_pred_next_prepare();
struct Q3TextRows {
    const float* text; int text_vocab;
    const int* ids; const int* cnt; int2* cur; int cap;
};
int q3_launch_pred_last_text(const Q3PredNext& a, const Q3TextRows& t, hipStream_t s, bool sample);

struct Q3PromptRow { int32_t kindA, idA, kindB, idB; };
void q3_launch_prompt_rows(const Q3PromptRow* rows, int n, const float* text, int text_vocab, const float* const* codec,
                           int codec0_rows, int codecq_rows, int ncb, const float* spk, int d, float* out, hipStream_t s);
void q3_launch_prompt_ref_frames(const int* codes, int n_frames, const float* marker, const float* const* codec,
                                 int codec0_rows, int codecq_rows, int ncb, int d, float* out, hipStream_t s);

void q3_launch_copy_rows(float* dst, int ldd, const float* src, int lds, int rows, int cols, hipStream_t s);

void q3_launch_gather_rows(float* dst, const float* src, const int* perm, int rows, int cols, hipStream_t s);
void q3_launch_rmsnorm_rows(const float* x, int ldx, const float* w, float eps, int d, int rows, float* out, int ldo, hipStream_t s);

#define Q3_PCM_MAX_ENT 64
struct Q3PcmEnt { int32_t row, first, count, pad; long long dst_off; };
struct Q3PcmPack { Q3PcmEnt e[Q3_PCM_MAX_ENT]; };
void q3_launch_pcm_pack(const float* src, size_t stride, const Q3PcmPack& ents, int n_ent, int max_count, int i16, void* dst, hipStream_t s);
__device__ __forceinline__ void q3_pcm_put(float* d, float v) { *d = v; }
__device__ __forceinline__ void q3_pcm_put(int16_t* d, float v) {
    v = v * 32767.0f;
    v = fminf(fmaxf(v, -32768.0f), 32767.0f);
    *d = (int16_t)(int)truncf(v);
}

#define Q3_RESAMPLE_MAX_COEF 32768
#define Q3_RESAMPLE_LDS_BYTES 65536
struct Q3Resamp { int32_t rate_in, rate_out, L, M, H, T; const float* tab; };
struct Q3PcmSrc { int32_t len[Q3_PCM_MAX_ENT]; unsigned long long final_mask; };
int q3_resample_plan(int rate_in, int rate_out, int* L, int* M, int* H, int* T);
int q3_resample_table(int rate_in, int rate_out, int* L, int* M, int* H, std::vector<float>& tab);
std::vector<float> q3_resample_device_layout(const std::vector<float>& tab, int L, int M, int T);
long long q3_resample_N(long long n, int L, int M);
long long q3_resample_D(long long n, int L, int M, int H);
int q3_launch_pcm_resample(const float* src, size_t stride, const Q3PcmPack& ents, const Q3PcmSrc& rows, int n_ent, int max_count, const Q3Resamp& rs,
                           int i16, void* dst, hipStream_t s);
```

qwen3-tts-rust_amd/csrc/q3_kernels.hip:

```cpp
#include "q3_kernels.h"


__global__ void k_fill_tiled(Q3Fill f, int nb0, int nb_count) {
    const size_t gid = (size_t)blockIdx.x * blockDim.x + threadIdx.x;
    const int kblocks = f.K >> 5;
    const size_t total = (size_t)nb_count * kblocks * 64;
    if (gid >= total) return;
    const int lane = (int)(gid & 63);
    const size_t t = gid >> 6;
    const int kb = (int)(t % kblocks), nb = nb0 + (int)(t / kblocks);
    const int n = nb * 16 + (lane & 15), k0 = kb * 32 + (lane >> 4) * 4;
    uint32_t tid; int lr; const uint16_t* src;
    if (f.mode == 0) { tid = f.tid_a; lr = n - f.row0; src = f.src_a; }
    else {
        const int tile = n >> 4, c = n & 15;
        if (c < 8) { tid = f.tid_a; lr = tile * 8 + c; src = f.src_a; }
        else { tid = f.tid_b; lr = tile * 8 + c - 8; src = f.src_b; }
    }
    uint16_t h[8];
#pragma unroll
    for (int e = 0; e < 8; ++e) {
        const size_t idx = (size_t)lr * f.K + k0 + (e >> 2) * 16 + (e & 3);
        h[e] = src ? src[idx] : q3_bf16(q3_synth(f.seed, tid, idx, f.scale));
    }
// ... 468 lines not shown
    const float* e = a.codec_q + (size_t)(ok ? code : 0) * d;
    const int frame = sl->n_frames;
    if (tid == 0) a.codes[((size_t)slot * a.max_steps_cap + frame) * a.ncb + a.q] = code;
    constexpr int NI = 8, NP = 4;
    const float* pr = ok ? a.pproj_q + (size_t)code * a.dp : a.proj_b;
    const bool trow = cur.x != 0;
    float pv[NP], wv[NP];
    if (!last) {
#pragma unroll
        for (int u = 0; u < NP; ++u) { const int i = min(tid + u * 256, a.dp - 1); pv[u] = pr[i]; wv[u] = a.nw[i]; }
    }
    for (int i0 = 0; i0 < d; i0 += NI * 256) {
        float ev[NI], fv[NI], tp[NI], nv[NI];
#pragma unroll
        for (int u = 0; u < NI; ++u) {
            const int i = min(i0 + tid + u * 256, d - 1);
            ev[u] = ok ? e[i] : 0.0f; fv[u] = a.fb[(size_t)b * d + i];
            if (last) {
                if constexpr (TEXT) tp[u] = trow ? text_elem(text_rows(tx...).text, text_rows(tx...).text_vocab, cur.y, i, d) : a.tts_pad[i];
                else tp[u] = a.tts_pad[i];
                nv[u] = a.nw[i];
            }
        }
#pragma unroll
        for (int u = 0; u < NI; ++u) {
            const int i = i0 + tid + u * 256;
            if (i >= d) continue;
            float f = fv[u] + ev[u];
            if (!last) a.fb[(size_t)b * d + i] = f;
            else {
                f = f + tp[u]; a.xT[(size_t)b * d + i] = f;
                if (a.xscale) q3_norm_out_q8(f, nv[u], b, i, d >> 6, a.x_rt16, (int8_t*)a.xb, a.xscale, a.ssp + (size_t)b * (d >> 4) + (i >> 4), (i & 15) == 0);
                else q3_norm_out(f, nv[u], a.xb + q3_atile_off(b, i, d >> 5), a.ssp + (size_t)b * (d >> 4) + (i >> 4), (i & 15) == 0);
            }
        }
    }
    if (!last) {
#pragma unroll
        for (int u = 0; u < NP; ++u) {
            const int i = tid + u * 256;
            if (i < a.dp) {
                a.px[(size_t)b * a.dp + i] = pv[u];
                if (a.xscale) q3_norm_out_q8(pv[u], wv[u], b, i, a.dp >> 6, a.x_rt16, (int8_t*)a.xb, a.xscale, a.ssp + (size_t)b * (a.dp >> 4) + (i >> 4), (i & 15) == 0);
                else q3_norm_out(pv[u], wv[u], a.xb + q3_atile_off(b, i, a.dp >> 5), a.ssp + (size_t)b * (a.dp >> 4) + (i >> 4), (i & 15) == 0);
            }
        }
        for (int i = tid + NP * 256; i < a.dp; i += 256) {
            const float v = pr[i];
            a.px[(size_t)b * a.dp + i] = v;
            if (a.xscale) q3_norm_out_q8(v, a.nw[i], b, i, a.dp >> 6, a.x_rt16, (int8_t*)a.xb, a.xscale, a.ssp + (size_t)b * (a.dp >> 4) + (i >> 4), (i & 15) == 0);
            else q3_norm_out(v, a.nw[i], a.xb + q3_atile_off(b, i, a.dp >> 5), a.ssp + (size_t)b * (a.dp >> 4) + (i >> 4), (i & 15) == 0);
        }
    }
    if (last) {
        __syncthreads();
        if (tid == 0) {
            a.row_pos_t[b] = sl->cur_pos; sl->cur_pos = sl->cur_pos + 1; sl->n_frames = frame + 1;
            if constexpr (TEXT) {
                const Q3TextRows& t = text_rows(tx...);
                t.cur[slot] = frame + 1 < tcnt ? make_int2(1, t.ids[(size_t)slot * t.cap + frame + 1]) : make_int2(0, 0);
            }
        }
    }
}
int q3_pred_next_prepare() {
    static std::mutex mu;
    static bool done[64] = {false};
    int dev = 0; if (hipGetDevice(&dev) != hipSuccess) dev = 0;
    std::lock_guard<std::mutex> lk(mu);
    if (done[dev & 63]) return 0;
    if (hipFuncSetAttribute((const void*)k_pred_next<true>, hipFuncAttributeMaxDynamicSharedMemorySize, SAMP_MAX * (int)sizeof(float)) != hipSuccess ||
        hipFuncSetAttribute((const void*)k_pred_next<true, Q3TextRows>, hipFuncAttributeMaxDynamicSharedMemorySize, SAMP_MAX * (int)sizeof(float)) != hipSuccess) {
        (void)hipGetLastError();
        return -1;
    }
    done[dev & 63] = true;
    return 0;
}
int q3_launch_pred_next(const Q3PredNext& a, hipStream_t s, bool sample) {
    if (!sample) { hipLaunchKernelGGL(k_pred_next<false>, dim3(a.B), dim3(256), 0, s, a); return 0; }
    if (a.cbs < 1 || a.cbs > SAMP_MAX || !a.plogits || !a.prng || a.q < 1) return -1;
    hipLaunchKernelGGL(k_pred_next<true>, dim3(a.B), dim3(256), (size_t)a.cbs * sizeof(float), s, a);
    return 0;
}
int q3_launch_pred_last_text(const Q3PredNext& a, const Q3TextRows& t, hipStream_t s, bool sample) {
    if (a.q != a.ncb - 1 || !t.ids || !t.cnt || !t.cur || t.cap < 1 || (t.text_vocab > 0 && !t.text)) return -1;
    if (!sample) { hipLaunchKernelGGL((k_pred_next<false, Q3TextRows>), dim3(a.B), dim3(256), 0, s, a, t); return 0; }
    if (a.cbs < 1 || a.cbs > SAMP_MAX || !a.plogits || !a.prng || a.q < 1) return -1;
    hipLaunchKernelGGL((k_pred_next<true, Q3TextRows>), dim3(a.B), dim3(256), (size_t)a.cbs * sizeof(float), s, a, t);
    return 0;
}

__device__ __forceinline__ float prompt_elem(int kind, int id, int i, const float* text, int text_vocab,
                                             const float* const* codec, int codec0_rows, int codecq_rows, int ncb,
                                             const float* spk, int d) {
    if (kind == 1) return text_elem(text, text_vocab, id, i, d);
    if (kind >= 2) {
        const int q = kind - 2;
        const int rows = q == 0 ? codec0_rows : codecq_rows;
        if (id < 0) id = 0;
        if (q < ncb && id < rows) return codec[q][(size_t)id * d + i];
        return 0.0f;
    }
    if (kind == -1) return spk[i];
    return 0.0f;
}
__global__ void k_prompt_rows(const Q3PromptRow* rows, const float* text, int text_vocab, const float* const* codec,
                              int codec0_rows, int codecq_rows, int ncb, const float* spk, int d, float* out) {
    const Q3PromptRow r = rows[blockIdx.x];
    for (int i = threadIdx.x; i < d; i += blockDim.x) {
        const float a = prompt_elem(r.kindA, r.idA, i, text, text_vocab, codec, codec0_rows, codecq_rows, ncb, spk, d);
        float v = a;
        if (r.kindB != 0) v = a + prompt_elem(r.kindB, r.idB, i, text, text_vocab, codec, codec0_rows, codecq_rows, ncb, spk, d);
        out[(size_t)blockIdx.x * d + i] = v;
    }
}
void q3_launch_prompt_rows(const Q3PromptRow* rows, int n, const float* text, int text_vocab, const float* const* codec,
                           int codec0_rows, int codecq_rows, int ncb, const float* spk, int d, float* out, hipStream_t s) {
    hipLaunchKernelGGL(k_prompt_rows, dim3(n), dim3(256), 0, s, rows, text, text_vocab, codec, codec0_rows, codecq_rows, ncb, spk, d, out);
}
__global__ void k_prompt_ref_frames(const int* codes, const float* marker, const float* const* codec, int codec0_rows,
                                    int codecq_rows, int ncb, int d, float* out) {
    const int f = blockIdx.x;
    for (int i = threadIdx.x; i < d; i += blockDim.x) {
        float sum = 0.0f;
        for (int q = 0; q < 16; ++q)
            sum += prompt_elem(2 + q, codes[f * 16 + q], i, nullptr, 0, codec, codec0_rows, codecq_rows, ncb, nullptr, d);
        out[(size_t)f * d + i] = marker[i] + sum;
    }
}
void q3_launch_prompt_ref_frames(const int* codes, int n_frames, const float* marker, const float* const* codec,
                                 int codec0_rows, int codecq_rows, int ncb, int d, float* out, hipStream_t s) {
    hipLaunchKernelGGL(k_prompt_ref_frames, dim3(n_frames), dim3(256), 0, s, codes, marker, codec, codec0_rows, codecq_rows, ncb, d, out);
}

__global__ void k_copy_rows(float* dst, int ldd, const float* src, int lds, int cols) {
    const int r = blockIdx.x;
    for (int i = threadIdx.x; i < cols; i += blockDim.x) dst[(size_t)r * ldd + i] = src[(size_t)r * lds + i];
}
__global__ void k_gather_rows(float* dst, const float* src, const int* perm, int cols) {
    const int r = blockIdx.y;
    const float* sp = src + (size_t)perm[r] * cols;
    for (int i = blockIdx.x * blockDim.x + threadIdx.x; i < cols; i += gridDim.x * blockDim.x) dst[(size_t)r * cols + i] = sp[i];
}
void q3_launch_gather_rows(float* dst, const float* src, const int* perm, int rows, int cols, hipStream_t s) {
    hipLaunchKernelGGL(k_gather_rows, dim3((cols + 255) / 256, rows), dim3(256), 0, s, dst, src, perm, cols);
}
void q3_launch_copy_rows(float* dst, int ldd, const float* src, int lds, int rows, int cols, hipStream_t s) {
    hipLaunchKernelGGL(k_copy_rows, dim3(rows), dim3(256), 0, s, dst, ldd, src, lds, cols);
}

template <int CPL>
__global__ __launch_bounds__(256) void k_rmsnorm_rows(const float* x, int ldx, const float* w, float eps, int d, int rows, float* out, int ldo) {
    const int r = blockIdx.x * 4 + (threadIdx.x >> 6), lane = threadIdx.x & 63;
    if (r >= rows) return;
    const float4* xr = (const float4*)(x + (size_t)r * ldx);
    float4* orow = (float4*)(out + (size_t)r * ldo);
    const float4* w4 = (const float4*)w;
    if constexpr (CPL > 0) {
        float4 v[CPL], g[CPL];
#pragma unroll
        for (int i = 0; i < CPL; ++i) { v[i] = xr[lane + 64 * i]; g[i] = w4[lane + 64 * i]; }
        float acc = 0.0f;
#pragma unroll
        for (int i = 0; i < CPL; ++i) { acc = fmaf(v[i].x, v[i].x, acc); acc = fmaf(v[i].y, v[i].y, acc); acc = fmaf(v[i].z, v[i].z, acc); acc = fmaf(v[i].w, v[i].w, acc); }
        acc = wave_sum(acc);
// ... 52 lines not shown
```

qwen3-tts-rust_amd/csrc/q3_layers.hip:

```cpp
#include "q3_engine.h"

static Q3BGemm gemm_w(const uint4* w, const uint16_t* wscale, int K, int N, int rows, int once) {
    Q3BGemm g{}; g.w_once = once; g.B = rows; g.w = w; g.wscale = wscale; g.K = K; g.N = N;
    return g;
}
static void a_rows(Q3BGemm& g, const Q3Tfm& t, const Q3Rows& r, float eps) {
    g.a = r.xb; g.ssp = r.ssp; g.ld_ssp = t.d / 16; g.ntiles = t.d / 16; g.d_norm = t.d; g.eps = eps;
    if (t.a8) { g.ascale = r.ascale; g.a_rt16 = r.rt16; }
}
static void a_scratch(Q3BGemm& g, const Q3Tfm& t, const Q3Scratch& sc, const uint16_t* a, const float* ascale) {
    g.a = a;
    if (t.a8) { g.ascale = ascale; g.a_rt16 = sc.rt16; }
}
static void y_rows(Q3BGemm& g, const Q3Tfm& t, const Q3Rows& r, const float* nw_next) {
    g.epi = Q3_EPI_RESID; g.y = r.x; g.ldy = t.d; g.yb = r.xb; g.nw_next = nw_next; g.ssp_out = r.ssp; g.ld_ssp_out = t.d / 16;
    if (t.a8) { g.yscale = r.ascale; g.y_rt16 = r.rt16; }
}
static Q3BGemm gemm_qkv(const Q3Tfm& t, int l, const Q3Rows& r, const Q3Scratch& sc, int rows, float eps, int once) {
    Q3BGemm g = gemm_w(t.wqkv[l], t.q8 ? t.sqkv[l] : nullptr, t.d, t.nqkv, rows, once);
    a_rows(g, t, r, eps);
    g.epi = Q3_EPI_STORE; g.y = sc.qkv; g.ldy = t.nqkv;
    return g;
}
static Q3BGemm gemm_o(const Q3Tfm& t, int l, const Q3Rows& r, const Q3Scratch& sc, int rows, int once) {
    Q3BGemm g = gemm_w(t.wo[l], t.q8 ? t.so[l] : nullptr, t.nq, t.d, rows, once);
    a_scratch(g, t, sc, sc.att, sc.asc_att);
    y_rows(g, t, r, t.ffn_norm[l]);
    return g;
}
static Q3BGemm gemm_gate_up(const Q3Tfm& t, int l, const Q3Rows& r, const Q3Scratch& sc, int rows, float eps, int once) {
    Q3BGemm g = gemm_w(t.wgu[l], t.q8 ? t.sgu[l] : nullptr, t.d, 2 * t.F, rows, once);
    a_rows(g, t, r, eps);
    g.epi = Q3_EPI_SWIGLU; g.yb = sc.h;
    if (t.a8) { g.yscale = sc.asc_h; g.y_rt16 = sc.rt16; }
    return g;
}
static Q3BGemm gemm_down(const Q3Tfm& t, int l, const Q3Rows& r, const Q3Scratch& sc, int rows, int once) {
    Q3BGemm g = gemm_w(t.wd[l], t.q8 ? t.sd[l] : nullptr, t.F, t.d, rows, once);
    a_scratch(g, t, sc, sc.h, sc.asc_h);
    y_rows(g, t, r, l + 1 < t.L ? t.attn_norm[l + 1] : t.out_norm);
    return g;
}
Q3BGemm q3_gemm_head(const Q3Tfm& t, int q, int N, const Q3Rows& r, int row0, int rows, float eps, int once, float* y) {
    const size_t tile_stride = (size_t)(N / 16) * (t.d / (t.q8 ? 64 : 32)) * 64, scale_stride = (size_t)N * (t.d / 32);
    Q3BGemm g = gemm_w(t.head + tile_stride * q, t.q8 ? t.shead + scale_stride * q : nullptr, t.d, N, rows, once);
    a_rows(g, t, r, eps);
    g.a_row0 = row0; g.ssp += (size_t)row0 * (t.d / 16);
    if (y) { g.epi = Q3_EPI_STORE; g.y = y; g.ldy = N; }
    return g;
}
template <class F>
static int probed(q3tts_engine* e, hipEvent_t* probe, int kind, hipStream_t s, F launch) {
    const bool on = probe && kind == e->probe_kind;
    if (on) hipEventRecord(probe[0], s);
    const int refused = launch() ? 1 : 0;
    if (on) hipEventRecord(probe[1], s);
    return refused;
}
int q3_launch_gemm(q3tts_engine* e, const Q3Tfm& t, const Q3BGemm& g, hipStream_t s, hipEvent_t* probe, int kind) {
    return probed(e, probe, kind, s, [&] { return (t.a8 ? q3_launch_bgemm8(g, s) : q3_launch_bgemm(g, s)) != 0; });
}

int q3_run_layers(q3tts_engine* e, Q3Tfm& t, const Q3Rows& r, const Q3LayerRun& a, Q3Scratch& sc, hipStream_t s) {
    const float eps = e->cfg.model.rms_eps;
    int bad = 0;
    const int once = &t == &e->T ? 1 : 0;
    for (int l = 0; l < t.L; ++l) {
        hipEvent_t* pe = l == 0 ? a.probe : nullptr;
        bad += q3_launch_gemm(e, t, gemm_qkv(t, l, r, sc, a.rows, eps, once), s, pe, 1);
        Q3QkPrep qp{}; qp.qkv = sc.qkv; qp.ld = t.nqkv; qp.rows = a.rows; qp.Hq = t.Hq; qp.Hkv = t.Hkv; qp.hd = t.hd;
        qp.qnw = t.qn[l]; qp.knw = t.kn[l]; qp.eps = eps; qp.cs = t.cs; qp.sn = t.sn;
        qp.kc = t.kc + l * t.layer_stride; qp.vc = t.vc + l * t.layer_stride; qp.n_ctx = t.n_ctx; qp.row_pos = a.row_pos; qp.row_slot = a.row_slot;
        qp.slot_mod = a.slot_mod; qp.pos_const = a.pos_const;
        const bool fused = a.one_row_per_slot && t.Hq / t.Hkv >= 2;
        const bool pair = !a.one_row_per_slot && a.slot_mod > 0 && a.rows == 2 * a.slot_mod && a.pos_const == 0 && t.Hq / t.Hkv == 2 && t.hd == 128;
        if (!fused && !pair) bad += q3_launch_qk_prep(qp, s) ? 1 : 0;
        Q3Attend at{}; at.qkv = sc.qkv; at.ld = t.nqkv; at.rows = a.rows; at.out = (float*)sc.att; at.ldo = t.nq; at.Hq = t.Hq; at.Hkv = t.Hkv; at.hd = t.hd;
        at.kc = qp.kc; at.vc = qp.vc; at.n_ctx = t.n_ctx; at.row_pos = a.row_pos; at.row_slot = a.row_slot;
        at.fused = pair ? 2 : (fused ? 1 : 0); at.prep = qp; at.out_bf16 = 1; at.slot_mod = a.slot_mod; at.pos_const = a.pos_const;
        if (t.a8) { at.out_bf16 = 2; at.out_scale = sc.asc_att; at.out_rt16 = sc.rt16; }
        if (!fused && !pair && a.n_seg > 0) { at.seg = a.seg; at.n_seg = a.n_seg; at.seg_max_n = a.seg_max_n; at.seg_max_t = a.seg_max_t; }
        bad += probed(e, pe, 2, s, [&] { return q3_launch_attend(at, s) != 0; });
        bad += q3_launch_gemm(e, t, gemm_o(t, l, r, sc, a.rows, once), s, pe, 3);
        bad += q3_launch_gemm(e, t, gemm_gate_up(t, l, r, sc, a.rows, eps, once), s, pe, 0);
        bad += q3_launch_gemm(e, t, gemm_down(t, l, r, sc, a.rows, once), s, pe, 4);
    }
    return bad;
}

int q3_record_frame(q3tts_engine* e, Q3Lane& L, hipStream_t s, int B) {
    int bad = 0;
    const q3tts_model_config& m = e->cfg.model;
    const int ncb = m.n_codebooks, cbs = m.codebook_size, dp = m.p_d_model, de = m.d_embed, cap = e->cfg.max_steps_cap;
    const float eps = m.rms_eps;
    Q3Slot* slots = e->slots;
    int* codes = e->codes;
    Q3Sample sa{}; sa.logits = L.logits; sa.ld = m.t_vocab; sa.limit = m.sample_limit; sa.eos = m.eos_code; sa.slots = slots; sa.B = B; sa.row_slot = L.slot_id;
    sa.rng = e->rng; sa.codes = codes; sa.max_steps_cap = cap; sa.ncb = ncb; sa.seen = e->seen; sa.seen_words = e->seen_words;
    const bool smp = e->pred_variant != 0;
    Q3PredInput pi{}; pi.xT = L.T.x; pi.out_norm = e->T.out_norm; pi.eps = eps; pi.d = de; pi.codec0 = e->codec[0]; pi.codec0_rows = m.codec0_rows;
    pi.slots = slots; pi.row_slot = L.slot_id; pi.X = nullptr; pi.fb = L.fb; pi.B = B; pi.pproj0 = e->pproj[0]; pi.proj_b = e->proj_b; pi.dp = dp; pi.px = L.P.x;
    pi.nw = e->P.attn_norm[0]; pi.xb = L.P.xb; pi.ssp = L.P.ssp;
    if (e->P.a8) { pi.xscale = L.P.ascale; pi.x_rt16 = L.P.rt16; }
    {
        Q3Project pj{}; pj.x = L.T.x; pj.ldx = de; pj.rows = B; pj.w = e->proj_w; pj.bias = e->proj_b; pj.n_in = de; pj.n_out = dp; pj.y = L.P.x; pj.ldy = dp;
        pj.nw = e->P.attn_norm[0]; pj.xb = L.P.xb; pj.ssp = L.P.ssp; pj.ld_ssp = dp / 16;
        pj.norm_w = e->T.out_norm; pj.eps = eps;
        if (e->P.a8) { pj.xscale = L.P.ascale; pj.x_rt16 = L.P.rt16; }
        bad += q3_launch_sample_input(sa, pi, pj, s) != 0;
    }
    auto pred_next = [&](int q) {
        Q3PredNext pn{}; pn.keys = L.keys; pn.n_key_parts = cbs / 16; pn.q = q; pn.ncb = ncb; pn.codec_q = e->codec[q]; pn.rows_q = m.codecq_rows; pn.d = de;
        pn.slots = slots; pn.row_slot = L.slot_id; pn.B = B; pn.codes = codes; pn.max_steps_cap = cap; pn.fb = L.fb;
        pn.tts_pad = e->tts_pad; pn.xT = L.T.x; pn.row_pos_t = L.row_pos_t; pn.pproj_q = e->pproj[q]; pn.proj_b = e->proj_b; pn.dp = dp; pn.px = L.P.x;
        const bool last = q == ncb - 1;
        pn.nw = last ? e->T.attn_norm[0] : e->P.attn_norm[0]; pn.xb = last ? L.T.xb : L.P.xb; pn.ssp = last ? L.T.ssp : L.P.ssp;
        if (last ? e->T.a8 : e->P.a8) { pn.xscale = last ? L.T.ascale : L.P.ascale; pn.x_rt16 = last ? L.T.rt16 : L.P.rt16; }
        if (smp) { pn.plogits = L.plogits; pn.cbs = cbs; pn.prng = e->prng; pn.prng_stride = cap * (ncb - 1); }
        if (last && e->ts_variant) {
            const Q3TextRows tr{e->text, m.text_vocab, e->ts_ids, e->ts_cnt, e->ts_cur, cap};
            bad += q3_launch_pred_last_text(pn, tr, s, smp) != 0;
        } else bad += q3_launch_pred_next(pn, s, smp) != 0;
    };
    for (int q = 0; q < ncb - 1; ++q) {
        const int rows = q == 0 ? 2 * B : B;
        if (q > 0) pred_next(q);
        hipEvent_t* pe = nullptr;
        if (e->probe == 1 && q == 1 && B == L.nb && e->probe_i + 2 <= 8) { pe = &e->probe_ev[e->probe_i]; e->probe_i += 2; }
        bad += q3_run_layers(e, e->P, L.P, {.rows = rows, .one_row_per_slot = q > 0, .probe = pe, .slot_mod = B, .pos_const = q == 0 ? 0 : q + 1}, L.sc, s);
        Q3BGemm g = q3_gemm_head(e->P, q, cbs, L.P, q == 0 ? B : 0, B, eps, 0, smp ? L.plogits : nullptr);
        if (!smp) { g.epi = Q3_EPI_ARGMAX; g.keys = L.keys; g.key_stride = cbs / 16; }
        bad += q3_launch_gemm(e, e->P, g, s);
    }
    pred_next(ncb - 1);
    hipEvent_t* pt = nullptr;
    if (e->probe == 2 && B == L.nb && e->probe_i + 2 <= 8) { pt = &e->probe_ev[e->probe_i]; e->probe_i += 2; }
    bad += q3_run_layers(e, e->T, L.T, {.rows = B, .row_pos = L.row_pos_t, .row_slot = L.slot_id, .one_row_per_slot = true, .probe = pt}, L.sc, s);
    bad += q3_launch_gemm(e, e->T, q3_gemm_head(e->T, 0, m.t_vocab, L.T, 0, B, eps, 1, L.logits), s);
    return bad;
}

int q3_capture_frames(q3tts_engine* e, std::vector<hipGraph_t>& graphs, std::vector<hipGraphExec_t>& execs) {
    Q3Lane& L = e->lane;
    graphs.resize(e->buckets.size(), nullptr); execs.resize(e->buckets.size(), nullptr);
    for (size_t bi = 0; bi < e->buckets.size(); ++bi) {
        Q3_HIP(e, hipStreamBeginCapture(L.stream, hipStreamCaptureModeThreadLocal));
        const int refused = q3_record_frame(e, L, L.stream, e->buckets[bi]);
        Q3_HIP(e, hipStreamEndCapture(L.stream, &graphs[bi]));
        if (refused) return q3_set_err(e, Q3TTS_ERR_INVALID, "frame step: " + std::to_string(refused) + " kernel launch(es) refused for this model shape");
        Q3_HIP(e, hipGraphInstantiate(&execs[bi], graphs[bi], nullptr, nullptr, 0));
        Q3_HIP(e, hipStreamSynchronize(L.stream));
    }
    return Q3TTS_OK;
}
```

qwen3-tts-rust_amd/csrc/q3_weights.hip:

```cpp
#include "q3_engine.h"
#include "q3_gguf.h"

#include <cmath>
#include <cstdio>

#define TRY(x) do { int rc__ = (x); if (rc__ != Q3TTS_OK) return rc__; } while (0)

void q3_rope_tables(int n_pos, int hd, float theta, const int* sections, std::vector<float>& cs, std::vector<float>& sn) {
    const int half = hd / 2;
    int s3 = half;
    if (sections) s3 = sections[0] + sections[1] + sections[2];
    cs.resize((size_t)n_pos * half); sn.resize((size_t)n_pos * half);
    for (int p = 0; p < n_pos; ++p)
        for (int i = 0; i < half; ++i) {
            const double inv = pow((double)theta, -2.0 * (double)i / (double)hd);
            const double ang = (i < s3) ? (double)p * inv : 0.0;
            cs[(size_t)p * half + i] = (float)cos(ang);
            sn[(size_t)p * half + i] = (float)sin(ang);
        }
}

struct GgSrc {
    q3tts_engine* e; const Q3Gguf* g; const char* file;
    std::vector<uint16_t> host; uint16_t* dev[2] = {nullptr, nullptr}; size_t dev_cap[2] = {0, 0};
// ... 172 lines not shown
        Q3Gguf g;
        if (g.open(gpath, err)) return q3_set_err(e, Q3TTS_ERR_INVALID, err);
        auto fetch = [&](const std::string& name, uint64_t ne0, bool required, std::vector<float>& out, size_t* nrows) -> int {
            const Q3GgufTensor* t = g.find(name);
            if (!t) return required ? q3_set_err(e, Q3TTS_ERR_INVALID, gpath + ": " + name + " (tensor) missing") : Q3TTS_OK;
            if (t->dims[0] != ne0 || t->dims.size() > 2) return q3_set_err(e, Q3TTS_ERR_INVALID, gpath + ": tensor '" + name + "' has the wrong row length");
            out.resize(t->nelem);
            if (q3_gguf_to_f32(*t, out.data(), err)) return q3_set_err(e, Q3TTS_ERR_INVALID, gpath + ": " + err);
            if (nrows) *nrows = t->dims.size() > 1 ? (size_t)t->dims[1] : 1;
            return Q3TTS_OK;
        };
        size_t pr = 0;
        TRY(fetch("proj.weight", d, true, pw, &pr));
        if (pr != (size_t)m.p_d_model) return q3_set_err(e, Q3TTS_ERR_INVALID, gpath + ": proj.weight does not have p_d_model rows");
        TRY(fetch("proj.bias", (uint64_t)m.p_d_model, true, pb, nullptr));
        TRY(fetch("text_embd", d, false, tabs[0], &rows[0]));
        for (int q = 0; q < m.n_codebooks; ++q) TRY(fetch("codec_embd." + std::to_string(q), d, true, tabs[1 + q], &rows[1 + q]));
    } else {
        auto fetch = [&](const std::string& file, bool required, std::vector<float>& out, size_t* nrows, size_t row_len) -> int {
            const std::string path = dir + "/" + file;
            if (!file_exists(path)) return required ? q3_set_err(e, Q3TTS_ERR_INVALID, "neither qwen3_assets.gguf nor " + file + " in " + dir) : Q3TTS_OK;
            std::vector<size_t> shape;
            if (q3_npy_load_f32(path, out, shape, err)) return q3_set_err(e, Q3TTS_ERR_INVALID, err);
            if (out.size() % row_len) return q3_set_err(e, Q3TTS_ERR_INVALID, path + ": size is not a multiple of the row length");
            if (nrows) *nrows = out.size() / row_len;
            return Q3TTS_OK;
        };
        size_t pr = 0, br = 0;
        TRY(fetch("proj_weight.npy", true, pw, &pr, d));
        TRY(fetch("proj_bias.npy", true, pb, &br, 1));
        if (pr != (size_t)m.p_d_model || br != (size_t)m.p_d_model) return q3_set_err(e, Q3TTS_ERR_INVALID, dir + ": projection shape does not match p_d_model");
        TRY(fetch("text_embedding_projected.npy", false, tabs[0], &rows[0], d));
        for (int q = 0; q < m.n_codebooks; ++q) TRY(fetch("codec_embedding_" + std::to_string(q) + ".npy", true, tabs[1 + q], &rows[1 + q], d));
    }
    for (int q = 2; q < m.n_codebooks; ++q)
        if (rows[1 + q] != rows[2]) return q3_set_err(e, Q3TTS_ERR_INVALID, dir + ": codec tables 1.." + std::to_string(m.n_codebooks - 1) + " differ in size");
    m.text_vocab = (int32_t)rows[0]; m.codec0_rows = (int32_t)rows[1];
    if (m.n_codebooks > 1) m.codecq_rows = (int32_t)rows[2];
    if (rows[0]) TRY(upload_table(e, &e->text, tabs[0].data(), tabs[0].size()));
    for (int q = 0; q < m.n_codebooks; ++q) TRY(upload_table(e, &e->codec[q], tabs[1 + q].data(), tabs[1 + q].size()));
    TRY(upload_proj(e, pw.data(), pb.data()));
    if ((size_t)m.tts_pad_id < rows[0]) e->tts_pad = e->text + (size_t)m.tts_pad_id * d;
    else TRY(q3_dalloc(e, &e->tts_pad, d));
    return Q3TTS_OK;
}
static int fill_assets_synthetic(q3tts_engine* e) {
    const q3tts_model_config& m = e->cfg.model;
    const uint64_t seed = e->cfg.synth_seed;
    const float es = 0.05f / Q3_IH4_STD, ps = 0.02f / Q3_IH4_STD;
    hipStream_t s = e->stream;
    TRY(q3_dalloc(e, &e->text, (size_t)m.text_vocab * m.d_embed));
    q3_launch_fill_f32(e->text, (size_t)m.text_vocab * m.d_embed, seed, Q3_TID(Q3G_ASSET, 0, Q3WA_TEXT), 0.0f, es, 1, s);
    for (int q = 0; q < m.n_codebooks; ++q) {
        const size_t rows = q == 0 ? m.codec0_rows : m.codecq_rows;
        TRY(q3_dalloc(e, &e->codec[q], rows * m.d_embed));
        q3_launch_fill_f32(e->codec[q], rows * m.d_embed, seed, Q3_TID(Q3G_ASSET, 1 + q, 0), 0.0f, es, 1, s);
    }
    TRY(q3_dalloc(e, &e->proj_w, (size_t)m.p_d_model * m.d_embed));
    q3_launch_fill_f32(e->proj_w, (size_t)m.p_d_model * m.d_embed, seed, Q3_TID(Q3G_ASSET, 0, Q3WA_PROJ_W), 0.0f, ps, 1, s);
    TRY(q3_dalloc(e, &e->proj_b, (size_t)m.p_d_model));
    q3_launch_fill_f32(e->proj_b, m.p_d_model, seed, Q3_TID(Q3G_ASSET, 0, Q3WA_PROJ_B), 0.0f, ps, 0, s);
    e->tts_pad = e->text + (size_t)m.tts_pad_id * m.d_embed;
    return Q3TTS_OK;
}

int q3_assets_init(q3tts_engine* e, const std::string& wdir) {
    const q3tts_model_config& m = e->cfg.model;
    hipStream_t s = e->stream;
    e->codec.assign(m.n_codebooks, nullptr);
    TRY(wdir.empty() ? fill_assets_synthetic(e) : load_assets_files(e, wdir));
    TRY(q3_dalloc(e, &e->codec_dev, 16));
    Q3_HIP(e, hipMemcpyAsync((void*)e->codec_dev, e->codec.data(), sizeof(float*) * m.n_codebooks, hipMemcpyHostToDevice, s));
    e->pproj.assign(m.n_codebooks, nullptr);
    for (int q = 0; q < m.n_codebooks; ++q) {
        const int rows = q == 0 ? m.codec0_rows : m.codecq_rows;
        TRY(q3_dalloc(e, &e->pproj[q], (size_t)rows * m.p_d_model));
        Q3Project pj{}; pj.x = e->codec[q]; pj.ldx = m.d_embed; pj.rows = rows; pj.w = e->proj_w; pj.bias = e->proj_b; pj.n_in = m.d_embed; pj.n_out = m.p_d_model;
        pj.y = e->pproj[q]; pj.ldy = m.p_d_model;
        q3_launch_project(pj, s);
    }
    Q3_HIP(e, hipStreamSynchronize(s));
    return Q3TTS_OK;
}
```

qwen3-tts-rust_amd/q3tts/_abi.py:

```python
import ctypes as C
import os

HERE = os.path.dirname(os.path.abspath(__file__))
PKG_ROOT = os.path.dirname(HERE)
REPO_ROOT = os.path.dirname(PKG_ROOT)
LIB_PATH = os.path.join(PKG_ROOT, "csrc", "libq3tts.so")

Q3TTS_MAX_UPSAMPLE = 4
Q3TTS_MAX_DEC_BLOCKS = 8


class ModelConfig(C.Structure):
    _fields_ = [
        ("t_n_layer", C.c_int32), ("t_d_model", C.c_int32), ("t_n_head", C.c_int32), ("t_n_kv_head", C.c_int32),
        ("t_head_dim", C.c_int32), ("t_d_ffn", C.c_int32), ("t_vocab", C.c_int32),
        ("t_rope_theta", C.c_float),
        ("t_mrope_sections", C.c_int32 * 4),
        ("p_n_layer", C.c_int32), ("p_d_model", C.c_int32), ("p_n_head", C.c_int32), ("p_n_kv_head", C.c_int32),
        ("p_head_dim", C.c_int32), ("p_d_ffn", C.c_int32),
        ("p_rope_theta", C.c_float),
        ("n_codebooks", C.c_int32), ("codebook_size", C.c_int32),
        ("rms_eps", C.c_float),
        ("d_embed", C.c_int32), ("text_vocab", C.c_int32), ("codec0_rows", C.c_int32), ("codecq_rows", C.c_int32),
        ("sample_limit", C.c_int32), ("eos_code", C.c_int32), ("tts_pad_id", C.c_int32),
# ... 45 lines not shown
        ("use_engine_sampler", C.c_int32),
        ("temperature", C.c_float), ("top_k", C.c_int32), ("top_p", C.c_float), ("has_seed", C.c_int32),
        ("text_open", C.c_int32),
        ("seed", C.c_uint64),
        ("max_steps", C.c_int32), ("min_frames", C.c_int32), ("force_eos_at", C.c_int32), ("want_pcm", C.c_int32),
        ("prefix", C.c_void_p),
    ]


class Result(C.Structure):
    _fields_ = [
        ("status", C.c_int32), ("n_frames", C.c_int32), ("hit_eos", C.c_int32),
        ("codes", C.POINTER(C.c_int32)), ("pcm", C.POINTER(C.c_float)),
        ("n_samples", C.c_int32), ("sample_rate", C.c_int32),
        ("first_chunk_ms", C.c_float), ("total_ms", C.c_float),
    ]


class VocTap(C.Structure):
    _fields_ = [
        ("name", C.c_char * 32), ("dtype", C.c_int32), ("layout", C.c_int32), ("hist_rows", C.c_int32), ("rows", C.c_int32),
        ("channels", C.c_int32), ("reserved", C.c_int32), ("offset", C.c_uint64),
    ]


class SessionEvent(C.Structure):
    _fields_ = [
        ("id", C.c_uint64), ("kind", C.c_int32), ("status", C.c_int32), ("pcm", C.c_void_p), ("n_samples", C.c_int32),
        ("is_final", C.c_int32), ("result", Result),
    ]


EV_NONE, EV_CHUNK, EV_DONE, EV_FAILED, EV_CANCELLED = 0, 1, 2, 3, 4
PCM_F32, PCM_I16 = 0, 1
SESSION_RING_DEPTH = 4


class Timings(C.Structure):
    _fields_ = [
        ("prefill_ms", C.c_float), ("decode_ms", C.c_float), ("vocoder_ms", C.c_float), ("total_ms", C.c_float),
        ("frame_step_ms", C.c_float), ("probe_kernel_ms", C.c_float),
        ("frame_steps", C.c_int64), ("algo_bytes_per_step", C.c_int64), ("algo_flops_per_step", C.c_int64),
        ("mean_live_slots", C.c_float), ("mean_rows", C.c_float), ("probe_count", C.c_int64), ("probe_empty_ms", C.c_float),
        ("mean_ctx_tokens", C.c_float),
    ]


class NodeTimings(C.Structure):
    _fields_ = [("generate_ms", C.c_float), ("gather_ms", C.c_float), ("total_ms", C.c_float), ("gathered_bytes", C.c_int64), ("n_devices", C.c_int32)]


class CloneConfig(C.Structure):
    _fields_ = [
        ("mel_dim", C.c_int32),
        ("se_channels", C.c_int32 * 5), ("se_kernels", C.c_int32 * 5), ("se_dilations", C.c_int32 * 5),
        ("se_attn_channels", C.c_int32), ("se_res2net_scale", C.c_int32), ("se_se_channels", C.c_int32), ("se_dim", C.c_int32),
        ("ae_filters", C.c_int32), ("ae_kernel", C.c_int32), ("ae_res_kernel", C.c_int32), ("ae_last_kernel", C.c_int32),
        ("ae_n_ratios", C.c_int32), ("ae_ratios", C.c_int32 * 4),
        ("ae_hidden", C.c_int32), ("ae_n_layer", C.c_int32), ("ae_n_head", C.c_int32), ("ae_head_dim", C.c_int32),
        ("ae_d_ffn", C.c_int32), ("ae_window", C.c_int32),
        ("ae_rope_theta", C.c_float), ("ae_ln_eps", C.c_float), ("ae_layer_scale", C.c_float),
        ("ae_down_stride", C.c_int32), ("ae_vq_dim", C.c_int32), ("ae_n_codebooks", C.c_int32), ("ae_codebook_size", C.c_int32),
    ]


SYMBOLS = [
    "q3tts_default_config", "q3tts_engine_create", "q3tts_engine_destroy", "q3tts_last_error", "q3tts_set_sampler",
    "q3tts_set_max_steps", "q3tts_build_prompt", "q3tts_free", "q3tts_generate", "q3tts_generate_batch",
    "q3tts_result_free", "q3tts_stream_begin", "q3tts_stream_poll", "q3tts_stream_end",
    "q3tts_get_timings", "q3tts_k_gemm_exact", "q3tts_k_attention", "q3tts_k_attention_decode", "q3tts_k_sample", "q3tts_k_talker_prefill",
    "q3tts_k_vocoder", "q3tts_k_vocoder_latent", "q3tts_k_vocoder_taps", "q3tts_k_vocoder_bench", "q3tts_set_device_pcm", "q3tts_get_device_pcm", "q3tts_k_rng_f32", "q3tts_k_probe", "q3tts_k_gguf_read", "q3tts_mel_frames", "q3tts_mel",
    "q3tts_clone_default_config", "q3tts_clone_init", "q3tts_clone_audio_frames", "q3tts_clone_audio_encode",
    "q3tts_clone_speaker_encode", "q3tts_k_speaker_from_mel", "q3tts_k_audio_latent",
    "q3tts_node_create", "q3tts_node_destroy", "q3tts_node_generate_batch", "q3tts_node_get_timings", "q3tts_node_last_error", "q3tts_node_size", "q3tts_node_engine", "q3tts_node_shard", "q3tts_k_bgemm_q8", "q3tts_k_bgemm_q8a8_argmax", "q3tts_k_bgemm_q8a8", "q3tts_k_alloc_upload", "q3tts_k_bgemm_policy", "q3tts_k_attend_policy", "q3tts_k_bgemm_pick", "q3tts_k_mfma_bf16", "q3tts_k_bgemm", "q3tts_k_bgemm_voc", "q3tts_k_project", "q3tts_k_norm_inputs", "q3tts_tokenizer_load", "q3tts_tokenizer_free", "q3tts_tokenizer_vocab_size", "q3tts_tokenizer_encode", "q3tts_tokenizer_decode",
    "q3tts_session_create", "q3tts_session_submit", "q3tts_session_cancel", "q3tts_session_next", "q3tts_session_close",
    "q3tts_session_last_error", "q3tts_k_pcm_pack",
    "q3tts_prefix_create", "q3tts_prefix_rows", "q3tts_prefix_destroy", "q3tts_k_talker_prefill_prefix",
    "q3tts_config_from_model_dir", "q3tts_k_gguf_meta",
    "q3tts_set_predictor_sampler", "q3tts_get_predictor_sampler", "q3tts_set_repetition_penalty", "q3tts_get_repetition_penalty",
    "q3tts_k_pred_variant",
    "q3tts_set_output_rate", "q3tts_get_output_rate", "q3tts_resample", "q3tts_k_resample_table", "q3tts_k_pcm_resample",
    "q3tts_session_append_text", "q3tts_k_text_ready",
    "q3tts_k_attention_runs", "q3tts_k_attention_decode_ex", "q3tts_k_attention_pair", "q3tts_k_attend_pick",
]


class Q3Error(RuntimeError):
    pass


_lib = None


def load_library(path=None):
    global _lib
    if _lib is not None and path is None:
        return _lib
    p = path or os.environ.get("Q3TTS_LIB") or LIB_PATH
    if not os.path.exists(p):
        raise Q3Error(
            f"{p} not found: build the HIP extension first (python -c 'import __graft_entry__ as g; g.build()'). "
            "There is no CPU fallback for the product path.")
    lib = C.CDLL(p)
    f32p, i32p, u32p = C.POINTER(C.c_float), C.POINTER(C.c_int32), C.POINTER(C.c_uint32)
    vp = C.c_void_p
    lib.q3tts_default_config.argtypes = [C.POINTER(EngineConfig)]
    lib.q3tts_default_config.restype = None
    lib.q3tts_engine_create.argtypes = [C.POINTER(EngineConfig), C.POINTER(vp)]
    lib.q3tts_engine_destroy.argtypes = [vp]
    lib.q3tts_engine_destroy.restype = None
    lib.q3tts_last_error.argtypes = [vp]
    lib.q3tts_last_error.restype = C.c_char_p
    lib.q3tts_set_sampler.argtypes = [vp, C.c_float, C.c_int32, C.c_float, C.c_int32, C.c_uint64]
    lib.q3tts_set_max_steps.argtypes = [vp, C.c_int32]
    lib.q3tts_set_predictor_sampler.argtypes = [vp, C.c_float, C.c_int32, C.c_float]
    lib.q3tts_get_predictor_sampler.argtypes = [vp, f32p, i32p, f32p]
    lib.q3tts_set_repetition_penalty.argtypes = [vp, C.c_float]
    lib.q3tts_get_repetition_penalty.argtypes = [vp, f32p]
    lib.q3tts_k_pred_variant.argtypes = [vp, C.c_int32]
    lib.q3tts_build_prompt.argtypes = [vp, C.POINTER(PromptDesc), C.POINTER(f32p), i32p]
    lib.q3tts_free.argtypes = [vp]
    lib.q3tts_free.restype = None
    lib.q3tts_generate.argtypes = [vp, C.POINTER(Request), C.POINTER(Result)]
    lib.q3tts_generate_batch.argtypes = [vp, C.POINTER(Request), C.c_int32, C.POINTER(Result)]
    lib.q3tts_result_free.argtypes = [C.POINTER(Result)]
    lib.q3tts_result_free.restype = None
    lib.q3tts_session_create.argtypes = [vp, C.c_int32, C.POINTER(vp)]
    lib.q3tts_session_submit.argtypes = [vp, C.POINTER(Request), C.POINTER(C.c_uint64)]
    lib.q3tts_session_cancel.argtypes = [vp, C.c_uint64]
    lib.q3tts_session_next.argtypes = [vp, C.c_int32, C.POINTER(SessionEvent)]
    lib.q3tts_session_close.argtypes = [vp]
    lib.q3tts_session_last_error.argtypes = [vp]
    lib.q3tts_session_last_error.restype = C.c_char_p
    lib.q3tts_session_append_text.argtypes = [vp, C.c_uint64, u32p, C.c_int32, C.c_int32]
    lib.q3tts_k_text_ready.argtypes = [C.c_int32, C.c_int32, C.c_int32]
    lib.q3tts_k_pcm_pack.argtypes = [C.c_int32, f32p, C.c_int32, C.c_int64, i32p, i32p, i32p, C.POINTER(C.c_int64), C.c_int32, C.c_int32, vp,
                                     C.c_int64]
    lib.q3tts_set_output_rate.argtypes = [vp, C.c_int32]
    lib.q3tts_get_output_rate.argtypes = [vp, i32p]
    lib.q3tts_resample.argtypes = [vp, f32p, C.c_int64, C.c_int32, C.c_int32, f32p, C.c_int64, C.POINTER(C.c_int64)]
    lib.q3tts_k_resample_table.argtypes = [C.c_int32, C.c_int32, i32p, i32p, i32p, f32p, C.c_int64, C.POINTER(C.c_int64)]
    lib.q3tts_k_pcm_resample.argtypes = [C.c_int32, f32p, C.c_int32, C.c_int64, i32p, i32p, i32p, i32p, i32p, C.POINTER(C.c_int64), C.c_int32,
                                         C.c_int32, C.c_int32, C.c_int32, vp, C.c_int64, C.c_int32, f32p]
    lib.q3tts_stream_begin.argtypes = [vp, C.POINTER(Request), C.POINTER(vp)]
    lib.q3tts_stream_poll.argtypes = [vp, C.POINTER(f32p), i32p, i32p]
    lib.q3tts_stream_end.argtypes = [vp, C.POINTER(Result)]
    lib.q3tts_get_timings.argtypes = [vp, C.POINTER(Timings)]
    lib.q3tts_k_gemm_exact.argtypes = [C.c_int32, f32p, C.c_int32, C.c_int32, C.POINTER(C.c_uint16), C.c_int32, f32p,
                                       C.c_float, f32p, C.c_int32, f32p, C.POINTER(C.c_uint64), C.c_int32, f32p]
    lib.q3tts_k_attention.argtypes = [C.c_int32, f32p, C.c_int32, C.c_int32, C.c_int32, C.c_int32, C.c_int32, f32p, f32p,
                                      C.c_float, C.c_float, i32p, f32p]
    lib.q3tts_k_attention_decode.argtypes = [C.c_int32, f32p, C.c_int32, i32p, C.c_int32, C.c_int32, C.c_int32, C.c_int32, f32p, f32p,
                                             C.c_float, C.c_float, i32p, C.c_int32, f32p, C.POINTER(C.c_uint16)]
    lib.q3tts_k_attention_runs.argtypes = [C.c_int32, f32p, C.c_int32, i32p, i32p, C.c_int32, C.c_int32, C.c_int32, C.c_int32, f32p, f32p, C.c_float,
                                           C.c_float, i32p, C.c_int32, C.c_int32, C.c_void_p, C.c_void_p, C.c_void_p, C.c_void_p]
    lib.q3tts_k_attention_decode_ex.argtypes = [C.c_int32, f32p, C.c_int32, i32p, C.c_int32, C.c_int32, C.c_int32, C.c_int32, f32p, f32p, C.c_float,
                                                C.c_float, i32p, C.c_int32, C.c_int32, C.c_int32, C.c_void_p, C.c_void_p, C.c_void_p, C.c_void_p]
    lib.q3tts_k_attention_pair.argtypes = [C.c_int32, f32p, C.c_int32, C.c_int32, C.c_int32, C.c_int32, C.c_int32, f32p, f32p, C.c_float, C.c_float,
                                           i32p, C.c_int32, C.c_void_p, C.c_void_p, C.c_void_p, C.c_void_p]
    lib.q3tts_k_attend_pick.argtypes = [C.c_int32, C.c_int32, C.c_int32, C.c_int32, C.c_int32, C.c_int32, C.c_int32, i32p]
    lib.q3tts_k_sample.argtypes = [C.c_int32, f32p, C.c_int32, C.c_int32, C.c_int32, C.c_float, C.c_int32, C.c_float,
                                   f32p, i32p]
    lib.q3tts_k_talker_prefill.argtypes = [vp, f32p, C.c_int32, f32p, f32p]
    lib.q3tts_k_talker_prefill_prefix.argtypes = [vp, vp, f32p, C.c_int32, f32p, f32p]
    lib.q3tts_prefix_create.argtypes = [vp, C.POINTER(PromptDesc), f32p, C.c_int32, C.POINTER(vp)]
    lib.q3tts_prefix_rows.argtypes = [vp]
    lib.q3tts_prefix_rows.restype = C.c_int32
    lib.q3tts_prefix_destroy.argtypes = [vp]
    lib.q3tts_k_vocoder.argtypes = [vp, i32p, C.c_int32, C.c_int32, f32p, i32p]
    lib.q3tts_k_vocoder_latent.argtypes = [vp, i32p, C.c_int32, C.c_int32, f32p]
    lib.q3tts_k_vocoder_taps.argtypes = [vp, i32p, C.c_int32, C.c_int32, C.c_int32, C.c_void_p, C.c_uint64, C.POINTER(VocTap), C.c_int32, i32p]
    lib.q3tts_k_vocoder_bench.argtypes = [vp, C.c_int32, C.c_int32, f32p]
    lib.q3tts_set_device_pcm.argtypes = [vp, C.c_int32]
    lib.q3tts_get_device_pcm.argtypes = [vp, C.POINTER(f32p), C.POINTER(C.c_int64), i32p]
    lib.q3tts_k_rng_f32.argtypes = [C.c_uint64, C.c_int32, f32p]
    lib.q3tts_k_probe.argtypes = [C.c_void_p, C.c_int32]
    lib.q3tts_mel_frames.argtypes = [C.c_int64]
    lib.q3tts_mel_frames.restype = C.c_int32
    lib.q3tts_mel.argtypes = [C.c_void_p, f32p, C.c_int64, f32p, C.c_int32, C.POINTER(C.c_int32)]
    lib.q3tts_k_gguf_read.argtypes = [C.c_char_p, C.c_char_p, f32p, C.c_int64, C.POINTER(C.c_int64), C.POINTER(C.c_int64), C.POINTER(C.c_int32)]
    lib.q3tts_k_gguf_meta.argtypes = [C.c_char_p, C.c_char_p, i32p, i32p, C.POINTER(C.c_int64), C.POINTER(C.c_double), C.c_int64, C.c_char_p, C.c_int64,
                                      C.POINTER(C.c_int64)]
    lib.q3tts_config_from_model_dir.argtypes = [C.c_char_p, C.c_char_p, C.POINTER(EngineConfig), C.c_char_p, C.c_int32, C.c_char_p, C.c_int32]
    lib.q3tts_clone_default_config.argtypes = [C.POINTER(CloneConfig)]
    lib.q3tts_clone_default_config.restype = None
    lib.q3tts_clone_init.argtypes = [vp, C.POINTER(CloneConfig)]
    lib.q3tts_clone_audio_frames.argtypes = [vp, C.c_int64]
    lib.q3tts_clone_audio_frames.restype = C.c_int32
    lib.q3tts_clone_audio_encode.argtypes = [vp, f32p, C.c_int64, C.POINTER(C.c_int64), C.c_int32, i32p]
    lib.q3tts_clone_speaker_encode.argtypes = [vp, f32p, C.c_int64, f32p]
    lib.q3tts_k_speaker_from_mel.argtypes = [vp, f32p, C.c_int32, f32p]
    lib.q3tts_k_audio_latent.argtypes = [vp, f32p, C.c_int64, f32p, C.c_int32, i32p]
    lib.q3tts_k_mfma_bf16.argtypes = [C.c_int32, C.c_void_p, C.c_void_p, C.c_void_p, C.c_void_p, C.c_int32, C.c_int32]
    lib.q3tts_k_bgemm.argtypes = [C.c_int32, C.c_void_p, C.c_int32, C.c_int32, C.c_void_p, C.c_int32, C.c_void_p, C.c_int32, C.c_int32, C.c_float,
                                  C.c_int32, C.c_void_p, C.c_void_p, C.c_void_p, C.c_void_p, C.c_void_p, C.c_int32, f32p]
    lib.q3tts_k_project.argtypes = [C.c_int32, C.c_void_p, C.c_int32, C.c_int32, C.c_void_p, C.c_void_p, C.c_int32, C.c_void_p, C.c_void_p, C.c_void_p, C.c_void_p]
    lib.q3tts_k_norm_inputs.argtypes = [C.c_int32, C.c_void_p, C.c_int32, C.c_int32, C.c_void_p, C.c_void_p, C.c_void_p]
    lib.q3tts_k_bgemm_voc.argtypes = [C.c_int32, C.c_void_p, C.c_int32, C.c_int32, C.c_void_p, C.c_int32, C.c_int32, C.c_void_p, C.c_int32, C.c_void_p,
                                      C.c_int32, C.c_int32, C.c_void_p, C.c_void_p, C.c_int32]
    lib.q3tts_node_create.argtypes = [C.POINTER(EngineConfig), i32p, C.c_int32, C.POINTER(vp)]
    lib.q3tts_node_destroy.argtypes = [vp]
    lib.q3tts_node_destroy.restype = None
    lib.q3tts_node_generate_batch.argtypes = [vp, C.POINTER(Request), C.c_int32, C.POINTER(Result), C.POINTER(C.POINTER(C.c_int16))]
    lib.q3tts_node_get_timings.argtypes = [vp, C.POINTER(NodeTimings)]
    lib.q3tts_node_last_error.argtypes = [vp]
    lib.q3tts_node_last_error.restype = C.c_char_p
    lib.q3tts_node_size.argtypes = [vp]
    lib.q3tts_node_size.restype = C.c_int32
    lib.q3tts_node_engine.argtypes = [vp, C.c_int32]
    lib.q3tts_node_engine.restype = vp
    lib.q3tts_node_shard.argtypes = [C.c_int32, C.c_int32, C.c_int32, i32p, C.c_int32]
    lib.q3tts_node_shard.restype = C.c_int32
    lib.q3tts_k_bgemm_q8.argtypes = [C.c_int32, C.c_void_p, C.c_int32, C.c_int32, C.c_void_p, C.c_void_p, C.c_int32, C.c_void_p, C.c_int32, C.c_int32, C.c_float,
                                     C.c_int32, C.c_void_p, C.c_void_p, C.c_void_p, C.c_void_p, C.c_void_p, C.c_int32, f32p]
    lib.q3tts_k_bgemm_q8a8_argmax.argtypes = [C.c_int32, C.c_void_p, C.c_void_p, C.c_int32, C.c_int32, C.c_void_p, C.c_void_p, C.c_int32, C.c_void_p, C.c_int32, C.c_int32, C.c_float, C.c_void_p]
    lib.q3tts_k_bgemm_q8a8_argmax.restype = C.c_int
    lib.q3tts_k_bgemm_q8a8.argtypes = [C.c_int32, C.c_void_p, C.c_void_p, C.c_int32, C.c_int32, C.c_void_p, C.c_void_p, C.c_int32, C.c_void_p, C.c_int32, C.c_int32, C.c_float,
                                       C.c_int32, C.c_void_p, C.c_void_p, C.c_void_p, C.c_void_p, C.c_void_p, C.c_int32, f32p]
    lib.q3tts_k_bgemm_policy.argtypes = [C.c_int32]
    lib.q3tts_k_attend_policy.argtypes = [C.c_int32, C.c_int32]
    lib.q3tts_k_bgemm_pick.argtypes = [C.c_int32, C.c_int32, C.c_int32, C.c_int32, C.c_int32, C.c_int32, i32p]
    lib.q3tts_k_alloc_upload.argtypes = [vp, C.c_int64, C.POINTER(C.c_int64)]
    lib.q3tts_tokenizer_load.argtypes = [C.c_char_p, C.POINTER(vp), C.c_char_p, C.c_int32]
    lib.q3tts_tokenizer_free.argtypes = [vp]
    lib.q3tts_tokenizer_free.restype = None
    lib.q3tts_tokenizer_vocab_size.argtypes = [vp]
    lib.q3tts_tokenizer_vocab_size.restype = C.c_int32
    lib.q3tts_tokenizer_encode.argtypes = [vp, C.c_char_p, C.c_int64, u32p, C.c_int32, i32p, C.c_char_p, C.c_int32]
    lib.q3tts_tokenizer_decode.argtypes = [vp, u32p, C.c_int32, C.c_char_p, C.c_int64, C.POINTER(C.c_int64), C.c_char_p, C.c_int32]
    if path is None:
        _lib = lib
    return lib


def default_config():
    cfg = EngineConfig()
    load_library().q3tts_default_config(C.byref(cfg))
    return cfg


def copy_config(cfg):
    c = EngineConfig.from_buffer_copy(cfg)
    c._source = cfg
# ... 96 lines not shown
```

qwen3-tts-rust_amd/q3tts/native.py:

```python
import ctypes as C
import math
import os
import weakref

import numpy as np

from . import _abi

f32p, i32p, u32p = C.POINTER(C.c_float), C.POINTER(C.c_int32), C.POINTER(C.c_uint32)


def _ptr(a, typ):
    return a.ctypes.data_as(typ)


_LANG_DEFAULT = object()


def make_prompt_desc(text_ids, spk_emb=None, lang_id=_LANG_DEFAULT, spk_id=-1, instruct_ids=None, ref_codes=None,
                     ref_text_ids=None, part="whole"):
    if part not in ("whole", "voice", "text"):
        raise ValueError(f"part must be 'whole', 'voice' or 'text', not {part!r}")
    if part == "voice" and text_ids is not None and len(text_ids) > 0:
        raise ValueError("a voice-only desc has no text: text_ids must be None or empty")
# ... 14 lines not shown
    t = np.ascontiguousarray([] if text_ids is None else text_ids, dtype=np.uint32)
    keep.append(t)
    d.text_ids, d.n_text = _ptr(t, u32p), len(t)
    if instruct_ids is not None:
        ins = np.ascontiguousarray(instruct_ids, dtype=np.uint32)
        keep.append(ins)
        d.instruct_ids, d.n_instruct = _ptr(ins, u32p), len(ins)
    d.lang_id, d.spk_id = (-1 if lang_id is None else lang_id), spk_id
    if spk_emb is not None:
        s = np.ascontiguousarray(spk_emb, dtype=np.float32)
        keep.append(s)
        d.spk_emb = _ptr(s, f32p)
    if ref_codes is not None:
        rc = np.ascontiguousarray(ref_codes, dtype=np.int32)
        keep.append(rc)
        d.ref_codes, d.n_ref_frames = _ptr(rc, i32p), rc.size // 16
        rt = np.ascontiguousarray(ref_text_ids if ref_text_ids is not None else [], dtype=np.uint32)
        keep.append(rt)
        d.ref_text_ids, d.n_ref_text = _ptr(rt, u32p), len(rt)
    return d, keep


class GenResult:
    def __init__(self, status, codes, pcm, hit_eos, first_chunk_ms, total_ms, sample_rate):
        self.status, self.codes, self.pcm, self.hit_eos = status, codes, pcm, hit_eos
        self.first_chunk_ms, self.total_ms, self.sample_rate = first_chunk_ms, total_ms, sample_rate

    @property
    def n_frames(self):
        return self.codes.shape[0]


class NativeEngine:

    def __init__(self, cfg):
        self.lib = _abi.load_library()
        self.cfg = cfg
        self.h = C.c_void_p()
        self._prefixes = weakref.WeakSet()
        rc = self.lib.q3tts_engine_create(C.byref(cfg), C.byref(self.h))
        if rc != 0:
            raise _abi.Q3Error(f"q3tts_engine_create failed ({rc}): {self.lib.q3tts_last_error(None).decode()}")

    def close(self):
        if getattr(self, "h", None):
            for x in list(getattr(self, "_prefixes", ())):
                x.close()
            self.lib.q3tts_engine_destroy(self.h)
            self.h = None

    def __del__(self):
        self.close()

    def _check(self, rc, what):
        if rc != 0:
            raise _abi.Q3Error(f"{what} failed ({rc}): {self.lib.q3tts_last_error(self.h).decode()}")

    def set_sampler(self, temperature, top_k, top_p, seed=None):
        self._check(self.lib.q3tts_set_sampler(self.h, temperature, top_k, top_p, 0 if seed is None else 1, seed or 0),
                    "q3tts_set_sampler")

    def set_max_steps(self, n):
        self._check(self.lib.q3tts_set_max_steps(self.h, n), "q3tts_set_max_steps")

    def set_predictor_sampler(self, temperature, top_k, top_p):
        self._check(self.lib.q3tts_set_predictor_sampler(self.h, temperature, top_k, top_p), "q3tts_set_predictor_sampler")

    def predictor_sampler(self):
        t, k, p = C.c_float(), C.c_int32(), C.c_float()
        self._check(self.lib.q3tts_get_predictor_sampler(self.h, C.byref(t), C.byref(k), C.byref(p)), "q3tts_get_predictor_sampler")
        return t.value, k.value, p.value

    def set_repetition_penalty(self, p):
        self._check(self.lib.q3tts_set_repetition_penalty(self.h, p), "q3tts_set_repetition_penalty")

    def repetition_penalty(self):
        p = C.c_float()
        self._check(self.lib.q3tts_get_repetition_penalty(self.h, C.byref(p)), "q3tts_get_repetition_penalty")
        return p.value

    def k_pred_variant(self, force):
        self._check(self.lib.q3tts_k_pred_variant(self.h, int(force)), "q3tts_k_pred_variant")

    def build_prompt(self, desc):
        out, n = f32p(), C.c_int32()
        self._check(self.lib.q3tts_build_prompt(self.h, C.byref(desc), C.byref(out), C.byref(n)), "q3tts_build_prompt")
        d = self.cfg.model.d_embed
        arr = np.ctypeslib.as_array(out, shape=(n.value, d)).copy()
        self.lib.q3tts_free(out)
        return arr

    def create_prefix(self, desc=None, embd=None):
        if (desc is None) == (embd is None):
            raise ValueError("create_prefix: give exactly one of desc or embd")
        h = C.c_void_p()
        if desc is not None:
            self._check(self.lib.q3tts_prefix_create(self.h, C.byref(desc), None, 0, C.byref(h)), "q3tts_prefix_create")
        else:
            e = np.ascontiguousarray(embd, dtype=np.float32)
            self._check(self.lib.q3tts_prefix_create(self.h, None, _ptr(e, f32p), e.shape[0], C.byref(h)), "q3tts_prefix_create")
        x = NativePrefix(self, h)
        self._prefixes.add(x)
        return x

    @staticmethod
    def make_request(embd=None, desc=None, temperature=0.0, top_k=40, top_p=0.9, seed=None, max_steps=0, min_frames=0,
                     force_eos_at=-1, want_pcm=0, use_engine_sampler=0, prefix=None, text_stream=False, text_open=False):
        r = _abi.Request()
        keep = []
        if prefix is not None:
            if not prefix.h:
                raise _abi.Q3Error("the prefix is closed")
            keep.append(prefix)
            r.prefix = prefix.h
        if embd is not None:
            e = np.ascontiguousarray(embd, dtype=np.float32)
            keep.append(e)
            r.prompt_embd, r.n_tok = _ptr(e, f32p), e.shape[0]
        if desc is not None:
            keep.append(desc)
            r.prompt = C.pointer(desc)
        r.use_engine_sampler = use_engine_sampler
        r.temperature, r.top_k, r.top_p = temperature, top_k, top_p
        r.has_seed, r.seed = (0, 0) if seed is None else (1, seed)
        r.max_steps, r.min_frames, r.force_eos_at, r.want_pcm = max_steps, min_frames, force_eos_at, want_pcm
        r.text_stream, r.text_open = int(bool(text_stream)), int(bool(text_open))
        return r, keep

    def _unpack(self, res):
        ncb = self.cfg.model.n_codebooks
        codes = np.ctypeslib.as_array(res.codes, shape=(res.n_frames, ncb)).copy() if res.n_frames > 0 else \
            np.zeros((0, ncb), dtype=np.int32)
        pcm = None
        if res.pcm:
            pcm = np.ctypeslib.as_array(res.pcm, shape=(res.n_samples,)).copy() if res.n_samples > 0 else \
                np.zeros(0, dtype=np.float32)
        out = GenResult(res.status, codes, pcm, bool(res.hit_eos), res.first_chunk_ms, res.total_ms, res.sample_rate)
        out.n_samples = int(res.n_samples)
        self.lib.q3tts_result_free(C.byref(res))
        return out

    def generate(self, **kw):
        r, keep = self.make_request(**kw)
        res = _abi.Result()
        self._check(self.lib.q3tts_generate(self.h, C.byref(r), C.byref(res)), "q3tts_generate")
        return self._unpack(res)

    def generate_batch(self, requests):
        n = len(requests)
        arr = (_abi.Request * n)()
        keep = []
        for i, kw in enumerate(requests):
            r, k = self.make_request(**kw)
            arr[i] = r
            keep.append(k)
        res = (_abi.Result * n)()
        self._check(self.lib.q3tts_generate_batch(self.h, arr, n, res), "q3tts_generate_batch")
        return [self._unpack(res[i]) for i in range(n)]

    def set_device_pcm(self, enable=True):
        self._check(self.lib.q3tts_set_device_pcm(self.h, 1 if enable else 0), "q3tts_set_device_pcm")

    def device_pcm(self):
        base, stride, n = f32p(), C.c_int64(0), C.c_int32(0)
        self._check(self.lib.q3tts_get_device_pcm(self.h, C.byref(base), C.byref(stride), C.byref(n)), "q3tts_get_device_pcm")
        return (C.cast(base, C.c_void_p).value or 0), int(stride.value), int(n.value)
# ... 489 lines not shown

ATTEND_KERNELS = ("k_attend<1, false>", "k_attend<2, false>", "k_attend<4, false>", "k_attend<2, true>", "k_attend<4, true>", "k_attend_gqa2",
                  "k_attend_small<2>", "k_attend_pair", "k_attend_prefill")


def k_attend_pick(fused, gqa_ratio, n_ctx, n_kv_head, n_seg=0, seg_max_n=0, seg_max_t=0):
    lib = _abi.load_library()
    k = C.c_int32(-2)
    rc = lib.q3tts_k_attend_pick(fused, gqa_ratio, n_ctx, n_seg, seg_max_n, seg_max_t, n_kv_head, C.byref(k))
    if rc != 0:
        raise _abi.Q3Error(f"q3tts_k_attend_pick failed ({rc}): {lib.q3tts_last_error(None).decode()}")
    return None if k.value < 0 else ATTEND_KERNELS[k.value]


def _att_hook_out(rows, nq, out_form, n_slots, n_kv_head, n_ctx, head_dim, want_cache):
    out = np.zeros((rows, nq), dtype=(np.float32, np.uint16, np.int8)[out_form] if 0 <= out_form <= 2 else np.float32)
    sc = np.zeros((rows, nq // 32), dtype=np.float32) if out_form == 2 else None
    kc = np.zeros((n_slots, n_kv_head, n_ctx, head_dim), dtype=np.uint16) if want_cache else None
    vc = np.zeros((n_slots, n_kv_head, n_ctx, head_dim), dtype=np.uint16) if want_cache else None
    return out, sc, kc, vc


def _att_hook_ret(out, sc, kc, vc):
    return dict(out=out, scale=sc, k_cache=kc, v_cache=vc)


def _dp(a):
    return None if a is None else a.ctypes.data


def k_attention_runs(qkv, runs, n_ctx, n_head, n_kv_head, head_dim, q_norm_w, k_norm_w, eps, rope_theta, sections, policy=-1, out_form=0,
                     want_cache=True, device=0):
    lib = _abi.load_library()
    qkv = np.ascontiguousarray(qkv, dtype=np.float32)
    p0 = np.ascontiguousarray([r[0] for r in runs], dtype=np.int32)
    nn = np.ascontiguousarray([r[1] for r in runs], dtype=np.int32)
    assert qkv.shape[0] == int(p0.sum() + nn.sum())
    qn = np.ascontiguousarray(q_norm_w, dtype=np.float32)
    kn = np.ascontiguousarray(k_norm_w, dtype=np.float32)
    sec = None if sections is None else np.ascontiguousarray(sections, dtype=np.int32)
    out, sc, kc, vc = _att_hook_out(max(int(nn.sum()), 1), n_head * head_dim, out_form, len(runs), n_kv_head, n_ctx, head_dim, want_cache)
    rc = lib.q3tts_k_attention_runs(device, _ptr(qkv, f32p), len(runs), _ptr(nn, i32p), _ptr(p0, i32p), n_ctx, n_head, n_kv_head, head_dim,
                                    _ptr(qn, f32p), _ptr(kn, f32p), eps, rope_theta, None if sec is None else _ptr(sec, i32p), policy, out_form,
                                    _dp(out), _dp(sc), _dp(kc), _dp(vc))
    if rc != 0:
        raise _abi.Q3Error(f"q3tts_k_attention_runs failed ({rc}): {lib.q3tts_last_error(None).decode()}")
    return _att_hook_ret(out, sc, kc, vc)


def k_attention_decode_ex(qkv, lens, n_ctx, n_head, n_kv_head, head_dim, q_norm_w, k_norm_w, eps, rope_theta, sections, policy=-1,
                          row_indexed=False, out_form=0, want_cache=True, device=0):
    lib = _abi.load_library()
    qkv = np.ascontiguousarray(qkv, dtype=np.float32)
    ln = np.ascontiguousarray(lens, dtype=np.int32)
    assert qkv.shape[0] == int(ln.sum())
    qn = np.ascontiguousarray(q_norm_w, dtype=np.float32)
    kn = np.ascontiguousarray(k_norm_w, dtype=np.float32)
    sec = None if sections is None else np.ascontiguousarray(sections, dtype=np.int32)
    out, sc, kc, vc = _att_hook_out(max(ln.size, 1), n_head * head_dim, out_form, ln.size, n_kv_head, n_ctx, head_dim, want_cache)
    rc = lib.q3tts_k_attention_decode_ex(device, _ptr(qkv, f32p), ln.size, _ptr(ln, i32p), n_ctx, n_head, n_kv_head, head_dim, _ptr(qn, f32p),
                                         _ptr(kn, f32p), eps, rope_theta, None if sec is None else _ptr(sec, i32p), policy,
                                         1 if row_indexed else 0, out_form, _dp(out), _dp(sc), _dp(kc), _dp(vc))
    if rc != 0:
        raise _abi.Q3Error(f"q3tts_k_attention_decode_ex failed ({rc}): {lib.q3tts_last_error(None).decode()}")
    return _att_hook_ret(out, sc, kc, vc)


def k_attention_pair(qkv, n_slots, n_ctx, n_head, n_kv_head, head_dim, q_norm_w, k_norm_w, eps, rope_theta, sections, out_form=0,
                     want_cache=True, device=0):
    lib = _abi.load_library()
    qkv = np.ascontiguousarray(qkv, dtype=np.float32)
    assert qkv.shape[0] == 2 * n_slots
    qn = np.ascontiguousarray(q_norm_w, dtype=np.float32)
    kn = np.ascontiguousarray(k_norm_w, dtype=np.float32)
    sec = None if sections is None else np.ascontiguousarray(sections, dtype=np.int32)
    out, sc, kc, vc = _att_hook_out(max(2 * n_slots, 1), n_head * head_dim, out_form, n_slots, n_kv_head, n_ctx, head_dim, want_cache)
    rc = lib.q3tts_k_attention_pair(device, _ptr(qkv, f32p), n_slots, n_ctx, n_head, n_kv_head, head_dim, _ptr(qn, f32p), _ptr(kn, f32p), eps,
                                    rope_theta, None if sec is None else _ptr(sec, i32p), out_form, _dp(out), _dp(sc), _dp(kc), _dp(vc))
    if rc != 0:
        raise _abi.Q3Error(f"q3tts_k_attention_pair failed ({rc}): {lib.q3tts_last_error(None).decode()}")
    return _att_hook_ret(out, sc, kc, vc)


def k_sample(logits, limit, temperature, top_k, top_p, r=None, device=0):
    lib = _abi.load_library()
    lg = np.ascontiguousarray(logits, dtype=np.float32)
    n, ld = lg.shape
    out = np.zeros(n, dtype=np.int32)
    rr = None if r is None else np.ascontiguousarray(r, dtype=np.float32)
    rc = lib.q3tts_k_sample(device, _ptr(lg, f32p), n, ld, limit, temperature, top_k, top_p, None if rr is None else _ptr(rr, f32p),
                            _ptr(out, i32p))
    if rc != 0:
        raise _abi.Q3Error(f"q3tts_k_sample failed ({rc}): {lib.q3tts_last_error(None).decode()}")
    return out


def k_gguf_read(path, tensor=""):
    lib = _abi.load_library()
    n = C.c_int64(0); dims = (C.c_int64 * 4)(); ty = C.c_int32(0)
    rc = lib.q3tts_k_gguf_read(os.fsencode(path), tensor.encode(), None, 0, C.byref(n), dims, C.byref(ty))
    if rc != 0:
        raise _abi.Q3Error(f"q3tts_k_gguf_read: {lib.q3tts_last_error(None).decode()} (status {rc})")
    out = np.zeros(n.value, dtype=np.float32)
    rc = lib.q3tts_k_gguf_read(os.fsencode(path), tensor.encode(), _ptr(out, f32p), n.value, C.byref(n), dims, C.byref(ty))
    if rc != 0:
        raise _abi.Q3Error(f"q3tts_k_gguf_read: {lib.q3tts_last_error(None).decode()} (status {rc})")
    shape = [int(d) for d in dims if d]
    if not str(path).endswith(".npy"):
        shape = shape[::-1]
    return out.reshape(shape), int(ty.value)


GGUF_VALUE_TYPES = ("u8", "i8", "u16", "i16", "u32", "i32", "f32", "bool", "str", "array", "u64", "i64", "f64")


def k_gguf_meta(path, key):
    lib = _abi.load_library()
    vt, et, n, nb = C.c_int32(0), C.c_int32(0), C.c_int64(0), C.c_int64(0)
    rc = lib.q3tts_k_gguf_meta(os.fsencode(path), key.encode(), C.byref(vt), C.byref(et), C.byref(n), None, 0, None, 0, C.byref(nb))
    if rc != 0:
        raise _abi.Q3Error(f"q3tts_k_gguf_meta: {lib.q3tts_last_error(None).decode()} (status {rc})")
    vals = (C.c_double * max(1, n.value))(); buf = C.create_string_buffer(max(1, nb.value))
    rc = lib.q3tts_k_gguf_meta(os.fsencode(path), key.encode(), C.byref(vt), C.byref(et), C.byref(n), vals, n.value, buf, nb.value, C.byref(nb))
    if rc != 0:
        raise _abi.Q3Error(f"q3tts_k_gguf_meta: {lib.q3tts_last_error(None).decode()} (status {rc})")
    tname, ename = GGUF_VALUE_TYPES[vt.value], GGUF_VALUE_TYPES[et.value]
    raw = buf.raw[:nb.value]
    if tname == "str":
        return tname, ename, raw
    if tname != "array":
        return tname, ename, vals[0]
    if ename != "str":
        return tname, ename, list(vals[:n.value])
    out, pos = [], 0
    for _ in range(n.value):
        ln = int.from_bytes(raw[pos:pos + 8], "little")
        out.append(raw[pos + 8:pos + 8 + ln])
        pos += 8 + ln
    return tname, ename, out


def config_from_model_dir(model_dir, quant=None, base=None):
    lib = _abi.load_library()
    cfg = _abi.copy_config(base) if base is not None else _abi.default_config()
    md = os.fsencode(model_dir)
    buf = C.create_string_buffer(len(md) + 16)
    err = C.create_string_buffer(1024)
    q = None if quant is None else str(quant).encode()
    rc = lib.q3tts_config_from_model_dir(md, q, C.byref(cfg), buf, len(buf), err, len(err))
    if rc != 0:
        raise _abi.Q3Error(f"q3tts_config_from_model_dir failed ({rc}): {err.value.decode('utf-8', 'replace')}")
    cfg._path_buf = buf
    return cfg


def k_pcm_pack(src, entries, out_n, fmt=0, device=0):
    lib = _abi.load_library()
    src = np.ascontiguousarray(src, dtype=np.float32)
    rows, stride = src.shape
    e = np.asarray(entries, dtype=np.int64).reshape(-1, 4)
    er, ef, ec = (np.ascontiguousarray(e[:, i], dtype=np.int32) for i in range(3))
    ed = np.ascontiguousarray(e[:, 3], dtype=np.int64)
    out = np.zeros(max(int(out_n), 1), dtype=np.int16 if fmt else np.float32)
    rc = lib.q3tts_k_pcm_pack(device, _ptr(src, f32p), rows, stride, _ptr(er, i32p), _ptr(ef, i32p), _ptr(ec, i32p),
                              ed.ctypes.data_as(C.POINTER(C.c_int64)), len(e), fmt, out.ctypes.data, int(out_n))
    if rc != 0:
# ... 112 lines not shown
```

Measured before the change: 658.4.

## Precompute predictor layer-0 QKV table per codebook and gather it in attention

At init, the predictor's layer-0 QKV projection is computed for every possible codec code of each codebook and stored as a device table. During decode, the attention kernel reads the sampled code's argmax and gathers that table row in place of the layer-0 QKV GEMM input. The extra block in the same kernel also does the embedding accumulation and projection copy for the next step. This removes a per-step GEMM in exchange for a large device table (capped by an env var), more init work and a more complex kernel.

```diff
diff --git a/include/q3tts.h b/include/q3tts.h
--- a/include/q3tts.h
+++ b/include/q3tts.h
@@ -270,6 +270,24 @@
                            const int32_t* mrope_sections, int32_t out_form, void* out, float* out_scale, uint16_t* k_cache, uint16_t* v_cache);
 int q3tts_k_attend_pick(int32_t fused, int32_t gqa_ratio, int32_t n_ctx, int32_t n_seg, int32_t seg_max_n, int32_t seg_max_t,
                         int32_t n_kv_head, int32_t* kernel);
+int q3tts_k_pred_table_row(q3tts_engine* e, int32_t q, int32_t code, float* out);
+typedef struct q3tts_k_pred_step {
+    int32_t n_rows, q, n_codebooks, n_key_parts, rows_q, d_embed, d_proj, max_steps_cap;
+    const uint64_t* keys;
+    const int32_t* active;
+    const int32_t* n_frames;
+    const float* codec_q;
+    const float* pproj_q;
+    const float* proj_b;
+    float* fb;
+    float* px;
+    int32_t* codes;
+} q3tts_k_pred_step;
+int q3tts_k_pred_next(int32_t device, q3tts_k_pred_step* st, const float* norm_w, uint16_t* xb, float* ssp);
+int q3tts_k_attention_gather(int32_t device, q3tts_k_pred_step* st, const float* table, const float* qkv, int32_t len, int32_t n_ctx,
+                             int32_t n_head, int32_t n_kv_head, int32_t head_dim, const float* q_norm_w, const float* k_norm_w, float eps,
+                             float rope_theta, const int32_t* mrope_sections, int32_t out_form, void* out, float* out_scale,
+                             uint16_t* k_cache, uint16_t* v_cache);
 int q3tts_k_sample(int32_t device, const float* logits, int32_t n, int32_t ld, int32_t limit, float temperature,
                    int32_t top_k, float top_p, const float* r_uniform, int32_t* out_ids);
 int q3tts_k_talker_prefill(q3tts_engine* e, const float* embd, int32_t n_tok, float* hidden_out, float* logits_out);
diff --git a/qwen3-tts-rust_amd/csrc/q3_attend.hip b/qwen3-tts-rust_amd/csrc/q3_attend.hip
--- a/qwen3-tts-rust_amd/csrc/q3_attend.hip
+++ b/qwen3-tts-rust_amd/csrc/q3_attend.hip
@@ -418,12 +418,51 @@
 #endif
 }
 
-template <int R>
-__global__ __launch_bounds__((R + 1) * 64) void k_attend_small(Q3Attend a) {
+__device__ __forceinline__ const Q3AttGather& att_gather(const Q3AttGather& t) { return t; }
+__device__ __forceinline__ void att_keys_load(const Q3AttGather& t, int row, int lane, unsigned long long kk[2]) {
+    const unsigned long long* kr = t.keys + (size_t)row * t.n_key_parts;
+    kk[0] = kr[min(lane, t.n_key_parts - 1)];
+    kk[1] = kr[min(lane + 64, t.n_key_parts - 1)];
+}
+__device__ __forceinline__ int att_keys_code(const Q3AttGather& t, int row, int lane, const unsigned long long kk[2]) {
+    unsigned long long k = kk[1] > kk[0] ? kk[1] : kk[0];
+    for (int p = lane + 128; p < t.n_key_parts; p += 64) { const unsigned long long o = t.keys[(size_t)row * t.n_key_parts + p]; k = o > k ? o : k; }
+#pragma unroll
+    for (int m = 32; m >= 1; m >>= 1) { const unsigned long long o = __shfl_xor(k, m); k = o > k ? o : k; }
+    return __builtin_amdgcn_readfirstlane(q3_argmax_idx(k));
+}
+__device__ __forceinline__ bool att_code_ok(const Q3AttGather& t, int code) { return code >= 0 && code < t.tab_rows; }
+template <int NT>
+__device__ __forceinline__ void att_gather_book(const Q3AttGather& t, int b, int tid) {
+    unsigned long long kk[2];
+    att_keys_load(t, b, tid & 63, kk);
+    const int slot = t.row_slot[b];
+    const Q3Slot* sl = t.slots + slot;
+    const int active = sl->active, frame = sl->n_frames;
+    const int code = att_keys_code(t, b, tid & 63, kk);
+    if (!active) return;
+    const bool ok = att_code_ok(t, code);
+    if (tid == 0) t.codes[((size_t)slot * t.max_steps_cap + frame) * t.ncb + t.q] = code;
+    const float4* e = (const float4*)(t.codec_q + (size_t)(ok ? code : 0) * t.d);
+    const float4* pr = (const float4*)(ok ? t.pproj_q + (size_t)code * t.dp : t.proj_b);
+    float4* fb = (float4*)(t.fb + (size_t)b * t.d);
+    float4* px = (float4*)(t.px + (size_t)b * t.dp);
+    for (int i = tid; i < (t.d >> 2); i += NT) {
+        const float4 f = fb[i], ev = ok ? e[i] : (float4){0.f, 0.f, 0.f, 0.f};
+        fb[i] = (float4){f.x + ev.x, f.y + ev.y, f.z + ev.z, f.w + ev.w};
+    }
+    for (int i = tid; i < (t.dp >> 2); i += NT) px[i] = pr[i];
+}
+template <int R, class... TX>
+__global__ __launch_bounds__((R + 1) * 64) void k_attend_small(Q3Attend a, TX... tx) {
+    constexpr bool GATHER = sizeof...(TX) != 0;
     __shared__ __attribute__((aligned(16))) float qh[R][Q3_ATT_HD];
     __shared__ __attribute__((aligned(16))) uint32_t knew[64];
     __shared__ __attribute__((aligned(16))) uint32_t vnew[64];
     const int g = blockIdx.x, row = blockIdx.y, wv = threadIdx.x >> 6, lane = threadIdx.x & 63;
+    if constexpr (GATHER) {
+        if (g == a.Hkv) { att_gather_book<(R + 1) * 64>(att_gather(tx...), row, threadIdx.x); return; }
+    }
     Q3_STAMP(a, 0);
     int pos, slot;
     q3_row_map(row, a.row_pos, a.row_slot, a.slot_mod, a.pos_const, &pos, &slot);
@@ -437,11 +476,22 @@
     const float* rowp = a.qkv + (size_t)row * a.ld;
     const float* csp = pr.cs + (size_t)pos * half + 4 * (lane & 15);
     const float* snp = pr.sn + (size_t)pos * half + 4 * (lane & 15);
+    unsigned long long kk[2] = {0ull, 0ull};
+    if constexpr (GATHER) att_keys_load(att_gather(tx...), row, lane, kk);
     if (wv == R) {
         const bool isk = lane < nl;
+        float4 w4 = (float4){0.f, 0.f, 0.f, 0.f}, c4 = (float4){1.f, 1.f, 1.f, 1.f}, s4 = (float4){0.f, 0.f, 0.f, 0.f};
+        if constexpr (GATHER) {
+            if (isk) { w4 = ((const float4*)pr.knw)[lane]; c4 = *(const float4*)csp; s4 = *(const float4*)snp; }
+            const Q3AttGather& t = att_gather(tx...);
+            __builtin_amdgcn_sched_barrier(0);
+            const int code = att_keys_code(t, row, lane, kk);
+            rowp = t.tab + (size_t)(att_code_ok(t, code) ? code : t.tab_rows) * a.ld;
+        }
         const float4 x4 = isk ? ((const float4*)(rowp + (size_t)(a.Hq + g) * hd))[lane] : ((const float4*)(rowp + (size_t)(a.Hq + a.Hkv + g) * hd))[lane - nl];
-        float4 w4 = (float4){0.f, 0.f, 0.f, 0.f}, c4 = (float4){1.f, 1.f, 1.f, 1.f}, s4 = (float4){0.f, 0.f, 0.f, 0.f};
-        if (isk) { w4 = ((const float4*)pr.knw)[lane]; c4 = *(const float4*)csp; s4 = *(const float4*)snp; }
+        if constexpr (!GATHER) {
+            if (isk) { w4 = ((const float4*)pr.knw)[lane]; c4 = *(const float4*)csp; s4 = *(const float4*)snp; }
+        }
         const float4 v = isk ? x4 : (float4){0.f, 0.f, 0.f, 0.f};
         float o[4];
         prep_arith(v, w4, c4, s4, pr.eps, lane, o);
@@ -467,7 +517,16 @@
 #pragma unroll
     for (int u = 0; u < 16; ++u) vv[u] = u < pos ? *(const uint32_t*)(vb + (size_t)u * hd + 2 * lane) : 0u;
     float4 x4 = (float4){0.f, 0.f, 0.f, 0.f}, w4 = x4, c4 = (float4){1.f, 1.f, 1.f, 1.f}, s4 = x4;
+    if constexpr (GATHER) {
+        if (lane < nl) { w4 = ((const float4*)pr.qnw)[lane]; c4 = *(const float4*)csp; s4 = *(const float4*)snp; }
+        const Q3AttGather& t = att_gather(tx...);
+        __builtin_amdgcn_sched_barrier(0);
+        const int code = att_keys_code(t, row, lane, kk);
+        rowp = t.tab + (size_t)(att_code_ok(t, code) ? code : t.tab_rows) * a.ld;
+        if (lane < nl) x4 = ((const float4*)(rowp + (size_t)hq * hd))[lane];
+    } else {
     if (lane < nl) { x4 = ((const float4*)(rowp + (size_t)hq * hd))[lane]; w4 = ((const float4*)pr.qnw)[lane]; c4 = *(const float4*)csp; s4 = *(const float4*)snp; }
+    }
     {
         float y[4];
         prep_norm(x4, prep_rinv(x4, pr.eps, hd), w4, y);
@@ -778,6 +837,17 @@
     return 0;
 }
 
+int q3_launch_attend_gather(const Q3Attend& a, const Q3AttGather& t, hipStream_t s) {
+    if (q3_attend_pick(a) != Q3_ATT_SMALL2 || a.rows < 1) return 1;
+    if (!t.tab || t.tab_rows < 1 || !t.keys || t.n_key_parts < 1 || t.q < 1 || t.q >= t.ncb || !t.codec_q || !t.slots || !t.row_slot || !t.codes ||
+        t.max_steps_cap < 1 || !t.fb || !t.pproj_q || !t.proj_b || !t.px || t.d < 4 || (t.d & 3) || t.dp < 4 || (t.dp & 3)) return 1;
+#ifdef Q3_STAMPS
+    if (a.dbg) return 1;
+#endif
+    hipLaunchKernelGGL((k_attend_small<2, Q3AttGather>), dim3(a.Hkv + 1, a.rows), dim3(192), 0, s, a, t);
+    return 0;
+}
+
 __global__ __launch_bounds__(256) void k_kv_prefix(Q3KvPrefix a) {
     const int j = blockIdx.y, isv = blockIdx.x & 1, lg = blockIdx.x >> 1, l = lg / a.Hkv, g = lg - l * a.Hkv;
     const int P = a.P[j], np = (P + 63) & ~63;
diff --git a/qwen3-tts-rust_amd/csrc/q3_engine.h b/qwen3-tts-rust_amd/csrc/q3_engine.h
--- a/qwen3-tts-rust_amd/csrc/q3_engine.h
+++ b/qwen3-tts-rust_amd/csrc/q3_engine.h
@@ -75,6 +75,7 @@
     std::vector<float*> pproj;
     float* proj_w = nullptr;
     float* proj_b = nullptr;
+    float* qkv0 = nullptr;
     float* tts_pad = nullptr;
     float* marker_row = nullptr;
     int B = 0;
@@ -157,6 +158,10 @@
 };
 int q3_tfm_init(q3tts_engine* e, Q3Tfm& t, const Q3TfmShape& sh, const Q3Gguf* g, const char* file, int q8mode);
 int q3_assets_init(q3tts_engine* e, const std::string& wdir);
+int q3_pred_table_init(q3tts_engine* e);
+inline int q3_pred_table_rows(const q3tts_engine* e) { return e->cfg.model.codecq_rows; }
+inline const float* q3_pred_table_slice(const q3tts_engine* e, int q) { return e->qkv0 + (size_t)(q - 1) * (q3_pred_table_rows(e) + 1) * e->P.nqkv; }
+inline bool q3_pred_table_on(const q3tts_engine* e) { return e->qkv0 && !e->P.a8 && e->pred_variant == 0; }
 
 struct Q3LayerRun {
     int rows;
@@ -165,10 +170,12 @@
     hipEvent_t* probe;
     int slot_mod, pos_const;
     const int* seg; int n_seg, seg_max_n, seg_max_t;
+    const Q3AttGather* gather;
 };
 int q3_run_layers(q3tts_engine* e, Q3Tfm& t, const Q3Rows& r, const Q3LayerRun& a, Q3Scratch& sc, hipStream_t s);
 int q3_record_frame(q3tts_engine* e, Q3Lane& L, hipStream_t s, int B);
 int q3_capture_frames(q3tts_engine* e, std::vector<hipGraph_t>& graphs, std::vector<hipGraphExec_t>& execs);
+Q3BGemm q3_gemm_qkv(const Q3Tfm& t, int l, const Q3Rows& r, const Q3Scratch& sc, int rows, float eps, int once);
 Q3BGemm q3_gemm_head(const Q3Tfm& t, int q, int N, const Q3Rows& r, int row0, int rows, float eps, int once, float* y);
 int q3_launch_gemm(q3tts_engine* e, const Q3Tfm& t, const Q3BGemm& g, hipStream_t s, hipEvent_t* probe = nullptr, int kind = -1);
 
diff --git a/qwen3-tts-rust_amd/csrc/q3_engine.hip b/qwen3-tts-rust_amd/csrc/q3_engine.hip
--- a/qwen3-tts-rust_amd/csrc/q3_engine.hip
+++ b/qwen3-tts-rust_amd/csrc/q3_engine.hip
@@ -155,6 +155,7 @@
                                .head_n = (m.n_codebooks - 1) * m.codebook_size, .theta = m.p_rope_theta, .sections = nullptr, .n_ctx = 64, .n_slots = B},
                      wdir.empty() ? nullptr : &gp, "qwen3_tts_predictor.gguf", cfg->predictor_q8_0));
     TRYC(q3_assets_init(e, wdir));
+    TRYC(q3_pred_table_init(e));
     TRYC(q3_dalloc(e, &e->slots, (size_t)B));
     HIPC(hipHostMalloc((void**)&e->slots_host, sizeof(Q3Slot) * 2 * B, hipHostMallocDefault));
     memset(e->slots_host, 0, sizeof(Q3Slot) * 2 * B);
@@ -961,9 +962,14 @@
         const long long wp_layers = (long long)e->P.weight_bytes - (long long)(bpw_p * (double)((size_t)e->P.head_n * m.p_d_model));
         const long long head1 = (long long)(bpw_p * (double)((size_t)m.codebook_size * m.p_d_model)), pj = 2ll * m.p_d_model * m.d_embed;
         const long long kv_per_tok = 2ll * m.t_n_layer * 2 * m.t_n_kv_head * m.t_head_dim;
-        const long long fixed = wt + (m.n_codebooks - 1) * (wp_layers + head1) + pj;
-        e->tm.algo_bytes_per_step = fixed + (steps ? kv_per_tok * (ctx_tokens / steps) : 0);
+        long long fixed = wt + (m.n_codebooks - 1) * (wp_layers + head1) + pj;
         e->tm.mean_live_slots = steps ? (float)((double)live_slot_steps / (double)steps) : 0.0f;
+        long long gathered = 0;
+        if (q3_pred_table_on(e)) {
+            fixed -= (long long)(m.n_codebooks - 2) * (long long)(bpw_p * (double)((size_t)e->P.nqkv * m.p_d_model));
+            gathered = (long long)((double)(m.n_codebooks - 2) * (double)e->tm.mean_live_slots * (double)e->P.nqkv * 4.0);
+        }
+        e->tm.algo_bytes_per_step = fixed + gathered + (steps ? kv_per_tok * (ctx_tokens / steps) : 0);
         e->tm.algo_flops_per_step = (long long)((double)fixed * (double)e->tm.mean_live_slots);
         e->tm.mean_rows = steps ? (float)((double)e->row_steps / (double)steps) : 0.0f;
         e->tm.mean_ctx_tokens = steps ? (float)((double)ctx_tokens / (double)steps) : 0.0f;
diff --git a/qwen3-tts-rust_amd/csrc/q3_hooks.hip b/qwen3-tts-rust_amd/csrc/q3_hooks.hip
--- a/qwen3-tts-rust_amd/csrc/q3_hooks.hip
+++ b/qwen3-tts-rust_amd/csrc/q3_hooks.hip
@@ -392,6 +392,104 @@
     if (n_seg > 0) { a.seg = (const int*)16; a.n_seg = n_seg; a.seg_max_n = seg_max_n; a.seg_max_t = seg_max_t; }
     *kernel = q3_attend_pick(a);
     return Q3TTS_OK;
+}
+
+extern "C" int q3tts_k_pred_table_row(q3tts_engine* e, int32_t q, int32_t code, float* out) {
+    if (!e || !out) return q3_set_err(e, Q3TTS_ERR_INVALID, "pred table row: null argument");
+    Q3_NOT_IN_SESSION(e);
+    if (!e->qkv0) return q3_set_err(e, Q3TTS_ERR_STATE, "pred table row: this engine has no layer-0 QKV table");
+    if (q < 1 || q > e->cfg.model.n_codebooks - 2) return q3_set_err(e, Q3TTS_ERR_INVALID, "pred table row: q outside 1 .. n_codebooks - 2");
+    const int rows = q3_pred_table_rows(e), r = (code >= 0 && code < rows) ? code : rows;
+    Q3_HIP(e, hipSetDevice(e->cfg.device));
+    Q3_HIP(e, hipStreamSynchronize(e->stream));
+    Q3_HIP(e, hipMemcpy(out, q3_pred_table_slice(e, q) + (size_t)r * e->P.nqkv, (size_t)e->P.nqkv * 4, hipMemcpyDeviceToHost));
+    return Q3TTS_OK;
+}
+
+struct PredStepHook {
+    DevBuf keys, slots, row_slot, codec, pproj, bias, fb, px, codes;
+    static const char* check(const q3tts_k_pred_step* st) {
+        if (!st || !st->keys || !st->active || !st->n_frames || !st->codec_q || !st->pproj_q || !st->proj_b || !st->fb || !st->px || !st->codes) return "a null argument";
+        if (st->n_rows < 1 || st->n_rows > 4096 || st->n_key_parts < 1 || st->n_key_parts > 4096 || st->rows_q < 1) return "1 .. 4096 rows and key parts, rows_q >= 1";
+        if (st->n_codebooks < 3 || st->q < 1 || st->q > st->n_codebooks - 2) return "q in 1 .. n_codebooks - 2";
+        if (st->d_embed < 256 || st->d_embed % 256 || st->d_proj < 32 || st->d_proj % 32) return "d_embed % 256 == 0, d_proj % 32 == 0";
+        if (st->max_steps_cap < 1) return "max_steps_cap >= 1";
+        for (int b = 0; b < st->n_rows; ++b) if (st->n_frames[b] < 0 || st->n_frames[b] >= st->max_steps_cap) return "n_frames in [0, max_steps_cap)";
+        return nullptr;
+    }
+    int init(const q3tts_k_pred_step* st) {
+        const size_t B = st->n_rows;
+        std::vector<Q3Slot> sl(B); std::vector<int> id(B);
+        memset(sl.data(), 0, B * sizeof(Q3Slot));
+        for (size_t b = 0; b < B; ++b) { sl[b].active = st->active[b] ? 1 : 0; sl[b].n_frames = st->n_frames[b]; id[b] = (int)b; }
+        TRY(keys.put(st->keys, B * st->n_key_parts * 8)); TRY(slots.put(sl.data(), B * sizeof(Q3Slot))); TRY(row_slot.put(id.data(), B * 4));
+        TRY(codec.put(st->codec_q, (size_t)st->rows_q * st->d_embed * 4)); TRY(pproj.put(st->pproj_q, (size_t)st->rows_q * st->d_proj * 4));
+        TRY(bias.put(st->proj_b, (size_t)st->d_proj * 4)); TRY(fb.put(st->fb, B * st->d_embed * 4)); TRY(px.put(st->px, B * st->d_proj * 4));
+        return codes.put(st->codes, B * st->max_steps_cap * st->n_codebooks * 4);
+    }
+    int read(q3tts_k_pred_step* st) const {
+        const size_t B = st->n_rows;
+        TRY(fb.get(st->fb, B * st->d_embed * 4)); TRY(px.get(st->px, B * st->d_proj * 4));
+        return codes.get(st->codes, B * st->max_steps_cap * st->n_codebooks * 4);
+    }
+};
+
+extern "C" int q3tts_k_pred_next(int32_t device, q3tts_k_pred_step* st, const float* norm_w, uint16_t* xb, float* ssp) {
+    if (const char* why = PredStepHook::check(st)) return q3_set_err(nullptr, Q3TTS_ERR_INVALID, std::string("pred next hook: ") + why);
+    if (!norm_w || !xb || !ssp) return q3_set_err(nullptr, Q3TTS_ERR_INVALID, "pred next hook: a null argument");
+    HK(hipSetDevice(device));
+    PredStepHook h;
+    TRY(h.init(st));
+    const int B = st->n_rows, dp = st->d_proj;
+    DevBuf dnw, dxb, dssp;
+    TRY(dnw.put(norm_w, (size_t)dp * 4)); TRY(dxb.alloc(pad16(B) * dp * 2)); TRY(dssp.alloc((size_t)B * (dp / 16) * 4));
+    Q3PredNext pn{}; pn.keys = h.keys; pn.n_key_parts = st->n_key_parts; pn.q = st->q; pn.ncb = st->n_codebooks; pn.codec_q = h.codec; pn.rows_q = st->rows_q;
+    pn.d = st->d_embed; pn.slots = h.slots; pn.row_slot = h.row_slot; pn.B = B; pn.codes = h.codes; pn.max_steps_cap = st->max_steps_cap; pn.fb = h.fb;
+    pn.pproj_q = h.pproj; pn.proj_b = h.bias; pn.dp = dp; pn.px = h.px; pn.nw = dnw; pn.xb = dxb; pn.ssp = dssp;
+    if (q3_launch_pred_next(pn, nullptr, false)) return q3_set_err(nullptr, Q3TTS_ERR_INVALID, "pred next hook: the launch was refused");
+    HK(hipGetLastError()); HK(hipDeviceSynchronize());
+    TRY(h.read(st)); TRY(untile_host(dxb, B, dp, xb));
+    return dssp.get(ssp, (size_t)B * (dp / 16) * 4);
+}
+
+extern "C" int q3tts_k_attention_gather(int32_t device, q3tts_k_pred_step* st, const float* table, const float* qkv, int32_t len, int32_t n_ctx, int32_t Hq,
+                                        int32_t Hkv, int32_t hd, const float* qnw, const float* knw, float eps, float theta, const int32_t* sections,
+                                        int32_t out_form, void* out, float* out_scale, uint16_t* k_cache, uint16_t* v_cache) {
+    if (const char* why = PredStepHook::check(st)) return q3_set_err(nullptr, Q3TTS_ERR_INVALID, std::string("attention gather hook: ") + why);
+    const int n_slots = st->n_rows;
+    if (const char* why = AttHook::check(qkv, n_slots, n_ctx, Hq, Hkv, hd, qnw, knw, out_form, out, out_scale))
+        return q3_set_err(nullptr, Q3TTS_ERR_INVALID, std::string("attention gather hook: ") + why);
+    if (!table || len < 1 || len > n_ctx) return q3_set_err(nullptr, Q3TTS_ERR_INVALID, "attention gather hook: table, 1 <= len <= n_ctx");
+    HK(hipSetDevice(device));
+    AttHook h;
+    TRY(h.init(n_slots, n_ctx, Hq, Hkv, qnw, knw, theta, sections, out_form, n_slots));
+    PredStepHook ps;
+    TRY(ps.init(st));
+    const int ld = h.ld, npre = n_slots * (len - 1);
+    std::vector<float> pre((size_t)std::max(npre, 1) * ld);
+    std::vector<int> pp, psl;
+    for (int s = 0, ip = 0; s < n_slots; ++s)
+        for (int r = 0; r < len - 1; ++r, ++ip) { memcpy(&pre[(size_t)ip * ld], qkv + ((size_t)s * len + r) * ld, (size_t)ld * 4); pp.push_back(r); psl.push_back(s); }
+    DevBuf dpre, dpp, dps, dtab;
+    TRY(dpre.put(pre.data(), pre.size() * 4)); TRY(dpp.put(pp.data(), pp.size() * 4)); TRY(dps.put(psl.data(), psl.size() * 4));
+    TRY(dtab.put(table, (size_t)(st->rows_q + 1) * ld * 4));
+    if (npre) {
+        Q3QkPrep qp = h.prep(dpre, npre, eps); qp.row_pos = dpp; qp.row_slot = dps;
+        if (q3_launch_qk_prep(qp, nullptr)) return q3_set_err(nullptr, Q3TTS_ERR_INVALID, "attention gather hook: the q/k prep launch was refused");
+    }
+    Q3QkPrep dq = h.prep(nullptr, n_slots, eps);
+    Q3Attend at = h.attend(nullptr, n_slots);
+    dq.slot_mod = at.slot_mod = n_slots; dq.pos_const = at.pos_const = len - 1;
+    at.fused = 1; at.prep = dq;
+    Q3AttGather gt{}; gt.tab = dtab; gt.tab_rows = st->rows_q; gt.keys = ps.keys; gt.n_key_parts = st->n_key_parts; gt.q = st->q; gt.ncb = st->n_codebooks;
+    gt.codec_q = ps.codec; gt.d = st->d_embed; gt.slots = ps.slots; gt.row_slot = ps.row_slot; gt.codes = ps.codes; gt.max_steps_cap = st->max_steps_cap;
+    gt.fb = ps.fb; gt.pproj_q = ps.pproj; gt.proj_b = ps.bias; gt.dp = st->d_proj; gt.px = ps.px;
+    if (q3_launch_attend_gather(at, gt, nullptr)) return q3_set_err(nullptr, Q3TTS_ERR_INVALID, "attention gather hook: the launch was refused (two query heads per KV head, n_ctx 64)");
+    hipError_t er = hipGetLastError();
+    if (er == hipSuccess) er = hipDeviceSynchronize();
+    if (er != hipSuccess) return q3_set_err(nullptr, Q3TTS_ERR_DEVICE, std::string("attention gather hook: ") + hipGetErrorString(er));
+    TRY(h.read_out(out, out_scale)); TRY(h.read_cache(k_cache, v_cache));
+    return ps.read(st);
 }
 
 extern "C" int q3tts_k_sample(int32_t device, const float* logits, int32_t n, int32_t ld, int32_t limit, float temperature, int32_t top_k,
diff --git a/qwen3-tts-rust_amd/csrc/q3_kernels.h b/qwen3-tts-rust_amd/csrc/q3_kernels.h
--- a/qwen3-tts-rust_amd/csrc/q3_kernels.h
+++ b/qwen3-tts-rust_amd/csrc/q3_kernels.h
@@ -193,6 +193,17 @@
     Q3_STAMP_FIELD
 };
 int q3_launch_attend(const Q3Attend& a, hipStream_t s);
+struct Q3AttGather {
+    const float* tab; int tab_rows;
+    const unsigned long long* keys; int n_key_parts;
+    int q, ncb;
+    const float* codec_q; int d;
+    const Q3Slot* slots; const int* row_slot;
+    int* codes; int max_steps_cap;
+    float* fb;
+    const float* pproj_q; const float* proj_b; int dp; float* px;
+};
+int q3_launch_attend_gather(const Q3Attend& a, const Q3AttGather& t, hipStream_t s);
 enum { Q3_ATT_REFUSED = -1, Q3_ATT_N1 = 0, Q3_ATT_N2 = 1, Q3_ATT_N4 = 2,
        Q3_ATT_F2 = 3, Q3_ATT_F4 = 4,
        Q3_ATT_GQA2 = 5, Q3_ATT_SMALL2 = 6, Q3_ATT_PAIR = 7, Q3_ATT_PREFILL = 8 };
@@ -243,6 +254,7 @@
     Q3_STAMP_FIELD
 };
 int q3_launch_pred_next(const Q3PredNext& a, hipStream_t s, bool sample = false);
+void q3_launch_pred_table_rows(const float* tab, int rows, const float* bias, int dp, const float* nw, uint16_t* xb, float* ssp, hipStream_t s);
 int q3_pred_next_prepare();
 struct Q3TextRows {
     const float* text; int text_vocab;
diff --git a/qwen3-tts-rust_amd/csrc/q3_kernels.hip b/qwen3-tts-rust_amd/csrc/q3_kernels.hip
--- a/qwen3-tts-rust_amd/csrc/q3_kernels.hip
+++ b/qwen3-tts-rust_amd/csrc/q3_kernels.hip
@@ -574,6 +574,15 @@
     if (a.cbs < 1 || a.cbs > SAMP_MAX || !a.plogits || !a.prng || a.q < 1) return -1;
     hipLaunchKernelGGL(k_pred_next<true>, dim3(a.B), dim3(256), (size_t)a.cbs * sizeof(float), s, a);
     return 0;
+}
+__global__ __launch_bounds__(256) void k_pred_table_rows(const float* tab, int rows, const float* bias, int dp, const float* nw, uint16_t* xb, float* ssp) {
+    const int c = blockIdx.x;
+    const float* pr = c < rows ? tab + (size_t)c * dp : bias;
+    for (int i = threadIdx.x; i < dp; i += 256)
+        q3_norm_out(pr[i], nw[i], xb + q3_atile_off(c, i, dp >> 5), ssp + (size_t)c * (dp >> 4) + (i >> 4), (i & 15) == 0);
+}
+void q3_launch_pred_table_rows(const float* tab, int rows, const float* bias, int dp, const float* nw, uint16_t* xb, float* ssp, hipStream_t s) {
+    hipLaunchKernelGGL(k_pred_table_rows, dim3(rows + 1), dim3(256), 0, s, tab, rows, bias, dp, nw, xb, ssp);
 }
 int q3_launch_pred_last_text(const Q3PredNext& a, const Q3TextRows& t, hipStream_t s, bool sample) {
     if (a.q != a.ncb - 1 || !t.ids || !t.cnt || !t.cur || t.cap < 1 || (t.text_vocab > 0 && !t.text)) return -1;
diff --git a/qwen3-tts-rust_amd/csrc/q3_layers.hip b/qwen3-tts-rust_amd/csrc/q3_layers.hip
--- a/qwen3-tts-rust_amd/csrc/q3_layers.hip
+++ b/qwen3-tts-rust_amd/csrc/q3_layers.hip
@@ -16,7 +16,7 @@
     g.epi = Q3_EPI_RESID; g.y = r.x; g.ldy = t.d; g.yb = r.xb; g.nw_next = nw_next; g.ssp_out = r.ssp; g.ld_ssp_out = t.d / 16;
     if (t.a8) { g.yscale = r.ascale; g.y_rt16 = r.rt16; }
 }
-static Q3BGemm gemm_qkv(const Q3Tfm& t, int l, const Q3Rows& r, const Q3Scratch& sc, int rows, float eps, int once) {
+Q3BGemm q3_gemm_qkv(const Q3Tfm& t, int l, const Q3Rows& r, const Q3Scratch& sc, int rows, float eps, int once) {
     Q3BGemm g = gemm_w(t.wqkv[l], t.q8 ? t.sqkv[l] : nullptr, t.d, t.nqkv, rows, once);
     a_rows(g, t, r, eps);
     g.epi = Q3_EPI_STORE; g.y = sc.qkv; g.ldy = t.nqkv;
@@ -67,7 +67,8 @@
     const int once = &t == &e->T ? 1 : 0;
     for (int l = 0; l < t.L; ++l) {
         hipEvent_t* pe = l == 0 ? a.probe : nullptr;
-        bad += q3_launch_gemm(e, t, gemm_qkv(t, l, r, sc, a.rows, eps, once), s, pe, 1);
+        const bool gather = a.gather && l == 0;
+        if (!gather) bad += q3_launch_gemm(e, t, q3_gemm_qkv(t, l, r, sc, a.rows, eps, once), s, l == (a.gather ? 1 : 0) ? a.probe : nullptr, 1);
         Q3QkPrep qp{}; qp.qkv = sc.qkv; qp.ld = t.nqkv; qp.rows = a.rows; qp.Hq = t.Hq; qp.Hkv = t.Hkv; qp.hd = t.hd;
         qp.qnw = t.qn[l]; qp.knw = t.kn[l]; qp.eps = eps; qp.cs = t.cs; qp.sn = t.sn;
         qp.kc = t.kc + l * t.layer_stride; qp.vc = t.vc + l * t.layer_stride; qp.n_ctx = t.n_ctx; qp.row_pos = a.row_pos; qp.row_slot = a.row_slot;
@@ -80,7 +81,7 @@
         at.fused = pair ? 2 : (fused ? 1 : 0); at.prep = qp; at.out_bf16 = 1; at.slot_mod = a.slot_mod; at.pos_const = a.pos_const;
         if (t.a8) { at.out_bf16 = 2; at.out_scale = sc.asc_att; at.out_rt16 = sc.rt16; }
         if (!fused && !pair && a.n_seg > 0) { at.seg = a.seg; at.n_seg = a.n_seg; at.seg_max_n = a.seg_max_n; at.seg_max_t = a.seg_max_t; }
-        bad += probed(e, pe, 2, s, [&] { return q3_launch_attend(at, s) != 0; });
+        bad += probed(e, pe, 2, s, [&] { return (gather ? q3_launch_attend_gather(at, *a.gather, s) : q3_launch_attend(at, s)) != 0; });
         bad += q3_launch_gemm(e, t, gemm_o(t, l, r, sc, a.rows, once), s, pe, 3);
         bad += q3_launch_gemm(e, t, gemm_gate_up(t, l, r, sc, a.rows, eps, once), s, pe, 0);
         bad += q3_launch_gemm(e, t, gemm_down(t, l, r, sc, a.rows, once), s, pe, 4);
@@ -122,12 +123,19 @@
             bad += q3_launch_pred_last_text(pn, tr, s, smp) != 0;
         } else bad += q3_launch_pred_next(pn, s, smp) != 0;
     };
+    const bool tab = q3_pred_table_on(e);
     for (int q = 0; q < ncb - 1; ++q) {
         const int rows = q == 0 ? 2 * B : B;
-        if (q > 0) pred_next(q);
+        const bool gq = tab && q > 0;
+        Q3AttGather gt{};
+        if (gq) {
+            gt.tab = q3_pred_table_slice(e, q); gt.tab_rows = q3_pred_table_rows(e); gt.keys = L.keys; gt.n_key_parts = cbs / 16; gt.q = q; gt.ncb = ncb;
+            gt.codec_q = e->codec[q]; gt.d = de; gt.slots = slots; gt.row_slot = L.slot_id; gt.codes = codes; gt.max_steps_cap = cap; gt.fb = L.fb;
+            gt.pproj_q = e->pproj[q]; gt.proj_b = e->proj_b; gt.dp = dp; gt.px = L.P.x;
+        } else if (q > 0) pred_next(q);
         hipEvent_t* pe = nullptr;
         if (e->probe == 1 && q == 1 && B == L.nb && e->probe_i + 2 <= 8) { pe = &e->probe_ev[e->probe_i]; e->probe_i += 2; }
-        bad += q3_run_layers(e, e->P, L.P, {.rows = rows, .one_row_per_slot = q > 0, .probe = pe, .slot_mod = B, .pos_const = q == 0 ? 0 : q + 1}, L.sc, s);
+        bad += q3_run_layers(e, e->P, L.P, {.rows = rows, .one_row_per_slot = q > 0, .probe = pe, .slot_mod = B, .pos_const = q == 0 ? 0 : q + 1, .gather = gq ? &gt : nullptr}, L.sc, s);
         Q3BGemm g = q3_gemm_head(e->P, q, cbs, L.P, q == 0 ? B : 0, B, eps, 0, smp ? L.plogits : nullptr);
         if (!smp) { g.epi = Q3_EPI_ARGMAX; g.keys = L.keys; g.key_stride = cbs / 16; }
         bad += q3_launch_gemm(e, e->P, g, s);
diff --git a/qwen3-tts-rust_amd/csrc/q3_weights.hip b/qwen3-tts-rust_amd/csrc/q3_weights.hip
--- a/qwen3-tts-rust_amd/csrc/q3_weights.hip
+++ b/qwen3-tts-rust_amd/csrc/q3_weights.hip
@@ -278,3 +278,36 @@
     Q3_HIP(e, hipStreamSynchronize(s));
     return Q3TTS_OK;
 }
+
+int q3_pred_table_init(q3tts_engine* e) {
+    const q3tts_model_config& m = e->cfg.model;
+    const Q3Tfm& P = e->P;
+    const int nq = m.n_codebooks - 2, rows = m.codecq_rows, R = rows + 1, dp = m.p_d_model;
+    if (const char* ev = getenv("Q3TTS_PRED_TABLE")) if (!atoi(ev)) return Q3TTS_OK;
+    if (P.a8 || nq < 1 || rows < 1) return Q3TTS_OK;
+    {
+        Q3Attend at{}; at.hd = P.hd; at.Hq = P.Hq; at.Hkv = P.Hkv; at.fused = 1; at.n_ctx = P.n_ctx;
+        if (q3_attend_pick(at) != Q3_ATT_SMALL2 || (m.d_embed & 3) || (dp & 3)) return Q3TTS_OK;
+    }
+    long long max_mb = 1024;
+    if (const char* ev = getenv("Q3TTS_PRED_TABLE_MAX_MB")) max_mb = atoll(ev);
+    const size_t n = (size_t)nq * R * P.nqkv;
+    if ((double)n * 4.0 > (double)max_mb * 1048576.0) return Q3TTS_OK;
+    TRY(q3_dalloc(e, &e->qkv0, n));
+    const size_t r16 = ((size_t)R + 15) & ~(size_t)15;
+    struct Stage { void* p = nullptr; ~Stage() { if (p) hipFree(p); } } xb, ssp;
+    if (hipMalloc(&xb.p, r16 * dp * 2) != hipSuccess || hipMalloc(&ssp.p, (size_t)R * (dp / 16) * 4) != hipSuccess)
+        return q3_set_err(e, Q3TTS_ERR_OOM, "hipMalloc (Predictor QKV table staging)");
+    hipStream_t s = e->stream;
+    Q3_HIP(e, hipMemsetAsync(xb.p, 0, r16 * dp * 2, s));
+    Q3Rows r{}; r.xb = (uint16_t*)xb.p; r.ssp = (float*)ssp.p;
+    for (int q = 1; q <= nq; ++q) {
+        q3_launch_pred_table_rows(e->pproj[q], rows, e->proj_b, dp, P.attn_norm[0], r.xb, r.ssp, s);
+        Q3Scratch sc{}; sc.qkv = e->qkv0 + (size_t)(q - 1) * R * P.nqkv;
+        if (q3_launch_gemm(e, P, q3_gemm_qkv(P, 0, r, sc, R, m.rms_eps, 0), s))
+            return q3_set_err(e, Q3TTS_ERR_INVALID, "Predictor QKV table: the GEMM launch was refused for this model shape");
+    }
+    Q3_HIP(e, hipGetLastError());
+    Q3_HIP(e, hipStreamSynchronize(s));
+    return Q3TTS_OK;
+}
diff --git a/qwen3-tts-rust_amd/q3tts/_abi.py b/qwen3-tts-rust_amd/q3tts/_abi.py
--- a/qwen3-tts-rust_amd/q3tts/_abi.py
+++ b/qwen3-tts-rust_amd/q3tts/_abi.py
@@ -151,7 +151,17 @@
     "q3tts_set_output_rate", "q3tts_get_output_rate", "q3tts_resample", "q3tts_k_resample_table", "q3tts_k_pcm_resample",
     "q3tts_session_append_text", "q3tts_k_text_ready",
     "q3tts_k_attention_runs", "q3tts_k_attention_decode_ex", "q3tts_k_attention_pair", "q3tts_k_attend_pick",
+    "q3tts_k_pred_table_row", "q3tts_k_pred_next", "q3tts_k_attention_gather",
 ]
+
+
+class PredStep(C.Structure):
+    _fields_ = [
+        ("n_rows", C.c_int32), ("q", C.c_int32), ("n_codebooks", C.c_int32), ("n_key_parts", C.c_int32), ("rows_q", C.c_int32),
+        ("d_embed", C.c_int32), ("d_proj", C.c_int32), ("max_steps_cap", C.c_int32),
+        ("keys", C.c_void_p), ("active", C.c_void_p), ("n_frames", C.c_void_p), ("codec_q", C.c_void_p), ("pproj_q", C.c_void_p),
+        ("proj_b", C.c_void_p), ("fb", C.c_void_p), ("px", C.c_void_p), ("codes", C.c_void_p),
+    ]
 
 
 class Q3Error(RuntimeError):
@@ -228,6 +238,10 @@
     lib.q3tts_k_attention_pair.argtypes = [C.c_int32, f32p, C.c_int32, C.c_int32, C.c_int32, C.c_int32, C.c_int32, f32p, f32p, C.c_float, C.c_float,
                                            i32p, C.c_int32, C.c_void_p, C.c_void_p, C.c_void_p, C.c_void_p]
     lib.q3tts_k_attend_pick.argtypes = [C.c_int32, C.c_int32, C.c_int32, C.c_int32, C.c_int32, C.c_int32, C.c_int32, i32p]
+    lib.q3tts_k_pred_table_row.argtypes = [vp, C.c_int32, C.c_int32, f32p]
+    lib.q3tts_k_pred_next.argtypes = [C.c_int32, C.POINTER(PredStep), C.c_void_p, C.c_void_p, C.c_void_p]
+    lib.q3tts_k_attention_gather.argtypes = [C.c_int32, C.POINTER(PredStep), C.c_void_p, C.c_void_p, C.c_int32, C.c_int32, C.c_int32, C.c_int32, C.c_int32,
+                                             f32p, f32p, C.c_float, C.c_float, i32p, C.c_int32, C.c_void_p, C.c_void_p, C.c_void_p, C.c_void_p]
     lib.q3tts_k_sample.argtypes = [C.c_int32, f32p, C.c_int32, C.c_int32, C.c_int32, C.c_float, C.c_int32, C.c_float,
                                    f32p, i32p]
     lib.q3tts_k_talker_prefill.argtypes = [vp, f32p, C.c_int32, f32p, f32p]
diff --git a/qwen3-tts-rust_amd/q3tts/native.py b/qwen3-tts-rust_amd/q3tts/native.py
--- a/qwen3-tts-rust_amd/q3tts/native.py
+++ b/qwen3-tts-rust_amd/q3tts/native.py
@@ -120,6 +120,12 @@
     def k_pred_variant(self, force):
         self._check(self.lib.q3tts_k_pred_variant(self.h, int(force)), "q3tts_k_pred_variant")
 
+    def pred_table_row(self, q, code):
+        m = self.cfg.model
+        out = np.zeros((m.p_n_head + 2 * m.p_n_kv_head) * m.p_head_dim, dtype=np.float32)
+        self._check(self.lib.q3tts_k_pred_table_row(self.h, int(q), int(code), _ptr(out, f32p)), "q3tts_k_pred_table_row")
+        return out
+
     def build_prompt(self, desc):
         out, n = f32p(), C.c_int32()
         self._check(self.lib.q3tts_build_prompt(self.h, C.byref(desc), C.byref(out), C.byref(n)), "q3tts_build_prompt")
@@ -775,6 +781,56 @@
     return _att_hook_ret(out, sc, kc, vc)
 
 
+class PredStepState:
+
+    def __init__(self, q, n_codebooks, keys, active, n_frames, codec_q, pproj_q, proj_b, fb, px, codes):
+        c = np.ascontiguousarray
+        self.keys = c(keys, dtype=np.uint64); self.active = c(active, dtype=np.int32); self.n_frames = c(n_frames, dtype=np.int32)
+        self.codec_q = c(codec_q, dtype=np.float32); self.pproj_q = c(pproj_q, dtype=np.float32); self.proj_b = c(proj_b, dtype=np.float32)
+        self.fb = np.array(fb, dtype=np.float32, order="C"); self.px = np.array(px, dtype=np.float32, order="C")
+        self.codes = np.array(codes, dtype=np.int32, order="C")
+        n = self.keys.shape[0]
+        assert self.active.shape == (n,) and self.n_frames.shape == (n,) and self.fb.shape == (n, self.codec_q.shape[1])
+        assert self.px.shape == (n, self.pproj_q.shape[1]) and self.codes.shape[0] == n and self.codes.shape[2] == n_codebooks
+        st = _abi.PredStep()
+        st.n_rows, st.q, st.n_codebooks, st.n_key_parts, st.rows_q = n, q, n_codebooks, self.keys.shape[1], self.codec_q.shape[0]
+        st.d_embed, st.d_proj, st.max_steps_cap = self.codec_q.shape[1], self.pproj_q.shape[1], self.codes.shape[1]
+        for name in ("keys", "active", "n_frames", "codec_q", "pproj_q", "proj_b", "fb", "px", "codes"):
+            setattr(st, name, getattr(self, name).ctypes.data)
+        self.st = st
+
+
+def k_pred_next(state, norm_w, device=0):
+    lib = _abi.load_library()
+    nw = np.ascontiguousarray(norm_w, dtype=np.float32)
+    n, dp = state.px.shape
+    xb = np.zeros((n, dp), dtype=np.uint16); ssp = np.zeros((n, dp // 16), dtype=np.float32)
+    rc = lib.q3tts_k_pred_next(device, C.byref(state.st), nw.ctypes.data, xb.ctypes.data, ssp.ctypes.data)
+    if rc != 0:
+        raise _abi.Q3Error(f"q3tts_k_pred_next failed ({rc}): {lib.q3tts_last_error(None).decode()}")
+    return xb, ssp
+
+
+def k_attention_gather(state, table, qkv, length, n_ctx, n_head, n_kv_head, head_dim, q_norm_w, k_norm_w, eps, rope_theta, sections, out_form=0,
+                       want_cache=True, device=0):
+    lib = _abi.load_library()
+    tab = np.ascontiguousarray(table, dtype=np.float32)
+    qkv = np.ascontiguousarray(qkv, dtype=np.float32)
+    n = state.px.shape[0]
+    ld = (n_head + 2 * n_kv_head) * head_dim
+    assert qkv.shape == (n * length, ld) and tab.shape == (state.codec_q.shape[0] + 1, ld)
+    qn = np.ascontiguousarray(q_norm_w, dtype=np.float32)
+    kn = np.ascontiguousarray(k_norm_w, dtype=np.float32)
+    sec = None if sections is None else np.ascontiguousarray(sections, dtype=np.int32)
+    out, sc, kc, vc = _att_hook_out(n, n_head * head_dim, out_form, n, n_kv_head, n_ctx, head_dim, want_cache)
+    rc = lib.q3tts_k_attention_gather(device, C.byref(state.st), tab.ctypes.data, qkv.ctypes.data, length, n_ctx, n_head, n_kv_head, head_dim,
+                                      _ptr(qn, f32p), _ptr(kn, f32p), eps, rope_theta, None if sec is None else _ptr(sec, i32p), out_form,
+                                      _dp(out), _dp(sc), _dp(kc), _dp(vc))
+    if rc != 0:
+        raise _abi.Q3Error(f"q3tts_k_attention_gather failed ({rc}): {lib.q3tts_last_error(None).decode()}")
+    return _att_hook_ret(out, sc, kc, vc)
+
+
 def k_sample(logits, limit, temperature, top_k, top_p, r=None, device=0):
     lib = _abi.load_library()
     lg = np.ascontiguousarray(logits, dtype=np.float32)
```

After: 691.4, median of 6. 1.05x the previous value.
